# groupeLIAMG/ttcr

Hardware: AMD Instinct MI355X
Metric: Mnodes/s per sweep-iteration (512^3 fp32 grid, first-order FSM) (higher is better)
Workload: dtype f32

## Files before the change

include/ttcr_amd.h:

```cpp
#ifndef TTCR_AMD_H
#define TTCR_AMD_H

#include <stddef.h>
#include <stdint.h>

#ifdef __cplusplus
extern "C" {
#endif

typedef struct ttcr_fsm_grid ttcr_fsm_grid;

enum { TTCR_F32 = 0, TTCR_F64 = 1 };

enum {
    TTCR_OK = 0,
    TTCR_ERR_VALUE = 1,
    TTCR_ERR_RUNTIME = 2,
    TTCR_ERR_DEVICE = 3,
    TTCR_ERR_UNSUPPORTED = 4
};

int ttcr_fsm_device_count(void);

const char* ttcr_fsm_last_error(void);
// ... 97 lines not shown
int ttcr_fsm_adjoint_vjp_source(const ttcr_fsm_adjoint* t, const void* w, int w_on_device, const void* field_cot, int fc_on_device, void* grad,
                                int grad_on_device, void* gsrc, int gsrc_on_device, int schedule, int* passes);
int ttcr_fsm_adjoint_hold(ttcr_fsm_adjoint* t, const void* w, int w_on_device, const void* field_cot, int fc_on_device, void* grad,
                          int grad_on_device, int schedule, int* passes);
int ttcr_fsm_adjoint_release(ttcr_fsm_adjoint* t);
int ttcr_fsm_adjoint_hvp(ttcr_fsm_adjoint* t, const void* v, int v_on_device, void* out, int out_on_device, int schedule, int* passes_jvp,
                         int* passes_vjp);
int ttcr_fsm_adjoint_newton(ttcr_fsm_adjoint* t, const void* v, int v_on_device, const void* row_weight, int rw_on_device, void* out,
                            int out_on_device, int schedule, int* passes_jvp, int* passes_vjp);
int ttcr_fsm_adjoint_jvp_block(const ttcr_fsm_adjoint* t, int n_cols, const void* ds, int ds_on_device, void* dtt, int dtt_on_device,
                               void* dfields, int df_on_device, int schedule, int* passes);
int ttcr_fsm_adjoint_vjp_block(const ttcr_fsm_adjoint* t, int n_cols, const void* w, int w_on_device, void* grad, int grad_on_device,
                               int schedule, int* passes);
int ttcr_fsm_adjoint_gn_block(const ttcr_fsm_adjoint* t, int n_cols, const void* v, int v_on_device, const void* row_weight,
                              int rw_cols, int rw_on_device, void* out, int out_on_device, int schedule, int* passes_jvp, int* passes_vjp);
int ttcr_fsm_adjoint_block_release(ttcr_fsm_adjoint* t);
int ttcr_fsm_adjoint_free(ttcr_fsm_adjoint* t);

int ttcr_fsm_normal_tile_edge(int dtype);
int ttcr_fsm_normal_smooth(ttcr_fsm_adjoint* t, const void* v, int v_on_device, const double* weights, void* out, int out_on_device);
int ttcr_fsm_normal_dot(ttcr_fsm_adjoint* t, const void* a, int a_on_device, const void* b, int b_on_device, double* result);
int ttcr_fsm_normal_solve(ttcr_fsm_adjoint* t, const void* rhs, int rhs_on_device, const void* row_weight, int rw_on_device, double smooth,
                          const double* smooth_weights, double damp, const void* x0, int x0_on_device, int maxiter, double rtol,
                          int newton, int schedule, void* x, int x_on_device, int* status, int* iterations, double* rho, double* pq,
                          int* passes);
int ttcr_fsm_normal_release(ttcr_fsm_adjoint* t);

int ttcr_fsm_joint_jvp(const ttcr_fsm_adjoint* t, const void* ds, int ds_on_device, const void* dsrc, int dsrc_on_device, void* dtt,
                       int dtt_on_device, void* dfields, int df_on_device, int schedule, int* passes);
int ttcr_fsm_joint_gn(const ttcr_fsm_adjoint* t, const void* v, int v_on_device, const void* v_src, int vs_on_device, const void* row_weight,
                      int rw_on_device, const double* source_scale, void* out, int out_on_device, void* out_src, int os_on_device,
                      int schedule, int* passes_jvp, int* passes_vjp);
int ttcr_fsm_joint_solve(ttcr_fsm_adjoint* t, const void* rhs, int rhs_on_device, const void* rhs_src, int rs_on_device,
                         const void* row_weight, int rw_on_device, double smooth, const double* smooth_weights, double damp,
                         const double* source_damp, const double* source_scale, int maxiter, double rtol, int schedule, void* x,
                         int x_on_device, void* x_src, int xs_on_device, int* status, int* iterations, double* rho, double* pq, int* passes);
int ttcr_fsm_joint_release(ttcr_fsm_adjoint* t);

int ttcr_fsm_rcv_eval(const ttcr_fsm_adjoint* t, size_t n_pts, const void* pts, int pts_on_device, const int* event_of_pt, void* tt,
                              int tt_on_device, void* grad, int grad_on_device);
int ttcr_fsm_rcv_points(ttcr_fsm_adjoint* t, const int* set_point_of_row, size_t set_n_points, size_t* n_points, int* point_of_row,
                        int* differing_rows);
int ttcr_fsm_rcv_jvp(const ttcr_fsm_adjoint* t, const void* drcv, int drcv_on_device, void* dtt, int dtt_on_device);
int ttcr_fsm_rcv_vjp(const ttcr_fsm_adjoint* t, const void* w, int w_on_device, void* grcv, int grcv_on_device);
int ttcr_fsm_rjoint_jvp(const ttcr_fsm_adjoint* t, const void* ds, int ds_on_device, const void* drcv, int drcv_on_device, void* dtt,
                        int dtt_on_device, void* dfields, int df_on_device, int schedule, int* passes);
int ttcr_fsm_rjoint_gn(const ttcr_fsm_adjoint* t, const void* v, int v_on_device, const void* v_rcv, int vr_on_device, const void* row_weight,
                       int rw_on_device, const double* rcv_scale, void* out, int out_on_device, void* out_rcv, int or_on_device,
                       int schedule, int* passes_jvp, int* passes_vjp);
int ttcr_fsm_rjoint_solve(ttcr_fsm_adjoint* t, const void* rhs, int rhs_on_device, const void* rhs_rcv, int rr_on_device,
                          const void* row_weight, int rw_on_device, double smooth, const double* smooth_weights, double damp,
                          const double* rcv_damp, const double* rcv_scale, int maxiter, double rtol, int schedule, void* x,
                          int x_on_device, void* x_rcv, int xr_on_device, int* status, int* iterations, double* rho, double* pq, int* passes);
int ttcr_fsm_rcv_release(ttcr_fsm_adjoint* t);

int ttcr_fsm_loc_geometry(const ttcr_fsm_adjoint* t, int* nn, double* dx, double* origin);
int ttcr_fsm_loc_shape(const ttcr_fsm_adjoint* t, int* node_tile, int* hypo_chunk, int* staged);
int ttcr_fsm_loc_grid(const ttcr_fsm_adjoint* t, size_t n_hypo, const long long* hypo_off, const int* pick_field, const double* pick_time,
                      const double* pick_weight, const int* box, long long* node_out, double* t0_out, double* misfit_out,
                      void* volume_out, int volume_on_device);
int ttcr_fsm_loc_release(ttcr_fsm_adjoint* t);

int ttcr_fsm_raytrace_l(ttcr_fsm_grid* g, int slot, int n_tx, const void* tx, const void* t0, int n_rx,
                        const void* rx, void* tt_out, int with_rays);
int ttcr_fsm_slot_l_size(const ttcr_fsm_grid* g, int slot, size_t* n_rows, size_t* nnz);
int ttcr_fsm_get_slot_l(const ttcr_fsm_grid* g, int slot, long long* row_off, long long* cell, void* v);
int ttcr_fsm_raytrace_multi_l(ttcr_fsm_grid* g, int n_src, const int* tx_off, const void* tx, const void* t0, const int* rx_off,
                              const void* rx, void* tt_out, int with_rays);
int ttcr_fsm_multi_l_size(const ttcr_fsm_grid* g, size_t* n_rows, size_t* nnz);
int ttcr_fsm_get_multi_l(const ttcr_fsm_grid* g, long long* row_off, long long* cell, void* v);

typedef struct {
    double sweep_ms;
    double total_ms;
    long long kernel_launches;
    long long node_updates;
    long long evaluated_updates;
    int iterations;
    int n_sources;
} ttcr_fsm_timing;
int ttcr_fsm_last_timing(const ttcr_fsm_grid* g, ttcr_fsm_timing* out);
int ttcr_fsm_stopping_stats(const ttcr_fsm_grid* g, long long* reference_sums, long long* reference_sums_missed, long long* rounds);
int ttcr_fsm_prefill_swaps(const ttcr_fsm_grid* g, long long* swaps);
int ttcr_fsm_prefill_inline_fills(const ttcr_fsm_grid* g, long long* fills);
int ttcr_fsm_reference_change(ttcr_fsm_grid* g, const void* times, const void* field, int parallel, void* out);
int ttcr_fsm_last_kernel(const ttcr_fsm_grid* g, char* buf, size_t n);
int ttcr_fsm_unit_order(int dim, int dtype, int stage, int by_time, uint32_t nnx, uint32_t nny, uint32_t nnz, uint32_t* out,
                        size_t capacity, size_t* n_units);
int ttcr_fsm_prefill_slice(int dtype, uint64_t n_el, uint32_t n_tickets, uint32_t ticket, uint64_t* slice_len, uint64_t* begin, uint64_t* end);
const char* ttcr_fsm_build_id(void);

#ifdef __cplusplus
}
#endif
#endif
```

ttcr_amd/_lib.py:

```python
import ctypes as C
import os

HERE = os.path.dirname(os.path.abspath(__file__))
LIB_PATH = os.environ.get("TTCR_AMD_LIB") or os.path.join(HERE, "libttcr_amd.so")

TTCR_F32, TTCR_F64 = 0, 1
OK, ERR_VALUE, ERR_RUNTIME, ERR_DEVICE, ERR_UNSUPPORTED = 0, 1, 2, 3, 4

_P = C.c_void_p
_U32 = C.c_uint32
_D = C.c_double
_I = C.c_int


class Timing(C.Structure):
    _fields_ = [("sweep_ms", C.c_double), ("total_ms", C.c_double), ("kernel_launches", C.c_longlong),
                ("node_updates", C.c_longlong), ("evaluated_updates", C.c_longlong), ("iterations", C.c_int),
                ("n_sources", C.c_int)]


SYMBOLS = {
    "ttcr_fsm_device_count": (_I, []),
    "ttcr_fsm_last_error": (C.c_char_p, []),
    "ttcr_fsm3d_create": (_I, [C.POINTER(_P), _I, _I, _U32, _U32, _U32, _D, _D, _D, _D, _D, _I, _I, _I, _I, _I]),
    "ttcr_fsm2d_create": (_I, [C.POINTER(_P), _I, _I, _U32, _U32, _D, _D, _D, _D, _D, _I, _I, _I, _I, _I]),
    "ttcr_fsm3d_create_multi": (_I, [C.POINTER(_P), _I, _I, _U32, _U32, _U32, _D, _D, _D, _D, _D, _I, _I, _I, _I, C.POINTER(_I), _I]),
    "ttcr_fsm2d_create_multi": (_I, [C.POINTER(_P), _I, _I, _U32, _U32, _D, _D, _D, _D, _D, _I, _I, _I, _I, C.POINTER(_I), _I]),
    "ttcr_fsm_n_devices": (_I, [_P]),
    "ttcr_fsm_destroy": (None, [_P]),
    "ttcr_fsm_set_slowness": (_I, [_P, _P, C.c_size_t]),
    "ttcr_fsm_set_slowness_device": (_I, [_P, _P, C.c_size_t]),
    "ttcr_fsm_set_slowness_c_order": (_I, [_P, _P, C.c_size_t]),
    "ttcr_fsm_get_slowness": (_I, [_P, _P, C.c_size_t]),
    "ttcr_fsm_raytrace": (_I, [_P, _I, _I, _P, _P, _I, _P, _P]),
    "ttcr_fsm_raytrace_multi": (_I, [_P, _I, _P, _P, _P, _P, _P, _P]),
    "ttcr_fsm_get_tt": (_I, [_P, _I, _P, C.c_size_t]),
    "ttcr_fsm_get_tt_device": (_I, [_P, _I, C.POINTER(_P)]),
    "ttcr_fsm_get_tt_device_view": (_I, [_P, _I, C.POINTER(_P), C.POINTER(C.c_size_t)]),
    "ttcr_fsm_interp": (_I, [_P, _I, _I, _P, _P]),
    "ttcr_fsm_compute_slowness": (_I, [_P, _I, _P, _I, _P]),
    "ttcr_fsm_get_niter": (_I, [_P, _I, C.POINTER(_I), C.POINTER(_I)]),
    "ttcr_fsm_get_changes": (_I, [_P, _I, C.POINTER(_D), _I, C.POINTER(_D), _I]),
    "ttcr_fsm_get_reference_changes": (_I, [_P, _I, C.POINTER(_D), _I, C.POINTER(_D), _I]),
    "ttcr_fsm_n_slots": (_I, [_P]),
    "ttcr_fsm_n_nodes": (C.c_size_t, [_P]),
    "ttcr_fsm_n_cells": (C.c_size_t, [_P]),
    "ttcr_fsm_set_option": (_I, [_P, C.c_char_p, _D]),
    "ttcr_fsm_last_timing": (_I, [_P, C.POINTER(Timing)]),
    "ttcr_fsm_last_kernel": (_I, [_P, C.c_char_p, C.c_size_t]),
    "ttcr_fsm_build_id": (C.c_char_p, []),
    "ttcr_fsm_unit_order": (_I, [_I, _I, _I, _I, _U32, _U32, _U32, C.POINTER(_U32), C.c_size_t, C.POINTER(C.c_size_t)]),
    "ttcr_fsm_stopping_stats": (_I, [_P, C.POINTER(C.c_longlong), C.POINTER(C.c_longlong), C.POINTER(C.c_longlong)]),
    "ttcr_fsm_prefill_swaps": (_I, [_P, C.POINTER(C.c_longlong)]),
    "ttcr_fsm_prefill_inline_fills": (_I, [_P, C.POINTER(C.c_longlong)]),
    "ttcr_fsm_prefill_slice": (_I, [_I, C.c_uint64, _U32, _U32, C.POINTER(C.c_uint64), C.POINTER(C.c_uint64), C.POINTER(C.c_uint64)]),
    "ttcr_fsm_reference_change": (_I, [_P, C.c_void_p, C.c_void_p, C.c_int, C.c_void_p]),
    "ttcr_fsm_rays_size": (_I, [_P, C.POINTER(C.c_size_t), C.POINTER(C.c_size_t)]),
    "ttcr_fsm_get_rays": (_I, [_P, _P, _P]),
    "ttcr_fsm_raytrace_rays": (_I, [_P, _I, _I, _P, _P, _I, _P, _P]),
    "ttcr_fsm_slot_rays_size": (_I, [_P, _I, C.POINTER(C.c_size_t), C.POINTER(C.c_size_t)]),
    "ttcr_fsm_get_slot_rays": (_I, [_P, _I, _P, _P]),
    "ttcr_fsm_raytrace_m": (_I, [_P, _I, _I, _P, _P, _I, _P, _P]),
    "ttcr_fsm_raytrace_rm": (_I, [_P, _I, _I, _P, _P, _I, _P, _P]),
    "ttcr_fsm_raytrace_multi_m": (_I, [_P, _I, _P, _P, _P, _P, _P, _P, _I]),
    "ttcr_fsm_multi_m_size": (_I, [_P, C.POINTER(C.c_size_t), C.POINTER(C.c_size_t)]),
    "ttcr_fsm_get_multi_m": (_I, [_P, _P, _P, _P]),
    "ttcr_fsm_raytrace_multi_tape": (_I, [_P, _I, _P, _P, _P, _P, _P, _P, C.POINTER(_P)]),
    "ttcr_fsm_tape_size": (_I, [_P, C.POINTER(C.c_size_t), C.POINTER(C.c_size_t), C.POINTER(C.c_size_t)]),
    "ttcr_fsm_tape_bytes": (_I, [_P, C.POINTER(C.c_size_t)]),
    "ttcr_fsm_tape_device": (_I, [_P, C.POINTER(_I)]),
    "ttcr_fsm_tape_get_csr": (_I, [_P, _P, _P, _P]),
    "ttcr_fsm_tape_vjp": (_I, [_P, _P, _I, _P, _I]),
    "ttcr_fsm_tape_free": (_I, [_P]),
    "ttcr_fsm_raytrace_multi_adjoint": (_I, [_P, _I, _P, _P, _P, _P, _P, _P, C.POINTER(_P)]),
    "ttcr_fsm_raytrace_multi_adjoint_cells": (_I, [_P, _I, _P, _P, _P, _P, _P, _P, C.POINTER(_P)]),
    "ttcr_fsm_adjoint_model": (_I, [_P, C.POINTER(_I), C.POINTER(C.c_size_t), C.POINTER(C.c_size_t)]),
    "ttcr_fsm_adjoint_size": (_I, [_P, C.POINTER(C.c_size_t), C.POINTER(C.c_size_t), C.POINTER(C.c_size_t)]),
    "ttcr_fsm_adjoint_bytes": (_I, [_P, C.POINTER(C.c_size_t)]),
    "ttcr_fsm_adjoint_device": (_I, [_P, C.POINTER(_I)]),
    "ttcr_fsm_adjoint_get_field": (_I, [_P, C.c_size_t, _P]),
    "ttcr_fsm_adjoint_vjp": (_I, [_P, _P, _I, _P, _I, _P, _I, _I, C.POINTER(_I)]),
    "ttcr_fsm_adjoint_jvp": (_I, [_P, _P, _I, _P, _I, _P, _I, _I, C.POINTER(_I)]),
    "ttcr_fsm_adjoint_gn": (_I, [_P, _P, _I, _P, _I, _P, _I, _I, C.POINTER(_I), C.POINTER(_I)]),
    "ttcr_fsm_adjoint_points": (_I, [_P, C.POINTER(C.c_size_t), _P]),
    "ttcr_fsm_adjoint_jvp_source": (_I, [_P, _P, _I, _I, _P, _I, _P, _I, _I, C.POINTER(_I)]),
    "ttcr_fsm_adjoint_vjp_source": (_I, [_P, _P, _I, _P, _I, _P, _I, _P, _I, _I, C.POINTER(_I)]),
    "ttcr_fsm_adjoint_hold": (_I, [_P, _P, _I, _P, _I, _P, _I, _I, C.POINTER(_I)]),
    "ttcr_fsm_adjoint_release": (_I, [_P]),
    "ttcr_fsm_adjoint_hvp": (_I, [_P, _P, _I, _P, _I, _I, C.POINTER(_I), C.POINTER(_I)]),
    "ttcr_fsm_adjoint_newton": (_I, [_P, _P, _I, _P, _I, _P, _I, _I, C.POINTER(_I), C.POINTER(_I)]),
    "ttcr_fsm_adjoint_jvp_block": (_I, [_P, _I, _P, _I, _P, _I, _P, _I, _I, C.POINTER(_I)]),
    "ttcr_fsm_adjoint_vjp_block": (_I, [_P, _I, _P, _I, _P, _I, _I, C.POINTER(_I)]),
    "ttcr_fsm_adjoint_gn_block": (_I, [_P, _I, _P, _I, _P, _I, _I, _P, _I, _I, C.POINTER(_I), C.POINTER(_I)]),
    "ttcr_fsm_adjoint_block_release": (_I, [_P]),
    "ttcr_fsm_adjoint_free": (_I, [_P]),
    "ttcr_fsm_normal_tile_edge": (_I, [_I]),
    "ttcr_fsm_normal_smooth": (_I, [_P, _P, _I, C.POINTER(_D), _P, _I]),
    "ttcr_fsm_normal_dot": (_I, [_P, _P, _I, _P, _I, C.POINTER(_D)]),
    "ttcr_fsm_normal_solve": (_I, [_P, _P, _I, _P, _I, _D, C.POINTER(_D), _D, _P, _I, _I, _D, _I, _I, _P, _I, C.POINTER(_I),
                                   C.POINTER(_I), C.POINTER(_D), C.POINTER(_D), C.POINTER(_I)]),
    "ttcr_fsm_normal_release": (_I, [_P]),
    "ttcr_fsm_joint_jvp": (_I, [_P, _P, _I, _P, _I, _P, _I, _P, _I, _I, C.POINTER(_I)]),
    "ttcr_fsm_joint_gn": (_I, [_P, _P, _I, _P, _I, _P, _I, C.POINTER(_D), _P, _I, _P, _I, _I, C.POINTER(_I), C.POINTER(_I)]),
    "ttcr_fsm_joint_solve": (_I, [_P, _P, _I, _P, _I, _P, _I, _D, C.POINTER(_D), _D, C.POINTER(_D), C.POINTER(_D), _I, _D, _I, _P, _I, _P, _I,
                                  C.POINTER(_I), C.POINTER(_I), C.POINTER(_D), C.POINTER(_D), C.POINTER(_I)]),
    "ttcr_fsm_joint_release": (_I, [_P]),
    "ttcr_fsm_rcv_eval": (_I, [_P, C.c_size_t, _P, _I, C.POINTER(_I), _P, _I, _P, _I]),
    "ttcr_fsm_rcv_points": (_I, [_P, C.POINTER(_I), C.c_size_t, C.POINTER(C.c_size_t), C.POINTER(_I), C.POINTER(_I)]),
    "ttcr_fsm_rcv_jvp": (_I, [_P, _P, _I, _P, _I]),
    "ttcr_fsm_rcv_vjp": (_I, [_P, _P, _I, _P, _I]),
    "ttcr_fsm_rjoint_jvp": (_I, [_P, _P, _I, _P, _I, _P, _I, _P, _I, _I, C.POINTER(_I)]),
    "ttcr_fsm_rjoint_gn": (_I, [_P, _P, _I, _P, _I, _P, _I, C.POINTER(_D), _P, _I, _P, _I, _I, C.POINTER(_I), C.POINTER(_I)]),
    "ttcr_fsm_rjoint_solve": (_I, [_P, _P, _I, _P, _I, _P, _I, _D, C.POINTER(_D), _D, C.POINTER(_D), C.POINTER(_D), _I, _D, _I, _P, _I, _P, _I,
                                   C.POINTER(_I), C.POINTER(_I), C.POINTER(_D), C.POINTER(_D), C.POINTER(_I)]),
    "ttcr_fsm_rcv_release": (_I, [_P]),
    "ttcr_fsm_loc_geometry": (_I, [_P, C.POINTER(_I), C.POINTER(_D), C.POINTER(_D)]),
    "ttcr_fsm_loc_shape": (_I, [_P, C.POINTER(_I), C.POINTER(_I), C.POINTER(_I)]),
    "ttcr_fsm_loc_grid": (_I, [_P, C.c_size_t, C.POINTER(C.c_longlong), C.POINTER(_I), C.POINTER(_D), C.POINTER(_D), C.POINTER(_I),
                               C.POINTER(C.c_longlong), C.POINTER(_D), C.POINTER(_D), _P, _I]),
    "ttcr_fsm_loc_release": (_I, [_P]),
    "ttcr_fsm_raytrace_multi_l": (_I, [_P, _I, _P, _P, _P, _P, _P, _P, _I]),
    "ttcr_fsm_multi_l_size": (_I, [_P, C.POINTER(C.c_size_t), C.POINTER(C.c_size_t)]),
    "ttcr_fsm_get_multi_l": (_I, [_P, _P, _P, _P]),
    "ttcr_fsm_slot_m_size": (_I, [_P, _I, C.POINTER(C.c_size_t), C.POINTER(C.c_size_t)]),
    "ttcr_fsm_get_slot_m": (_I, [_P, _I, _P, _P, _P]),
    "ttcr_fsm_raytrace_l": (_I, [_P, _I, _I, _P, _P, _I, _P, _P, _I]),
    "ttcr_fsm_slot_l_size": (_I, [_P, _I, C.POINTER(C.c_size_t), C.POINTER(C.c_size_t)]),
    "ttcr_fsm_get_slot_l": (_I, [_P, _I, _P, _P, _P]),
}

_lib = None


def load():
# ... 50 lines not shown
```

ttcr_amd/build.py:

```python
import os
import shutil
import subprocess

HERE = os.path.dirname(os.path.abspath(__file__))
CSRC = os.path.join(HERE, "csrc")
OBJ = os.path.join(CSRC, "_obj")
LIB = os.path.join(HERE, "libttcr_amd.so")
INC = os.path.join("..", "..", "include", "ttcr_amd.h")
UNITS = {
    "fsm_capi.hip": ([], ["fsm_capi.hip", "fsm_kernels.h", "fsm_fast_api.h", "fsm_march_levels.inc", "fsm_fast.hip", "fsm_tape_api.h",
                          "fsm_tape.hip", "fsm_adjoint_api.h", "fsm_adjoint.hip", "fsm_normal.hip", "fsm_locate.hip", "fsm_unit_order.h", "fsm_prefill_slices.h", INC]),
    "fsm_fast.hip": ([], ["fsm_fast.hip", "fsm_fast_api.h", "fsm_kernels.h", "fsm_march_levels.inc", "fsm_prefill_slices.h"]),
    "fsm_tape.hip": ([], ["fsm_tape.hip", "fsm_tape_api.h"]),
    "fsm_adjoint.hip": ([], ["fsm_adjoint.hip", "fsm_adjoint_api.h", "fsm_kernels.h", "fsm_march_levels.inc", "fsm_prefill_slices.h"]),
    "fsm_normal.hip": ([], ["fsm_normal.hip", "fsm_adjoint_api.h"]),
    "fsm_locate.hip": ([], ["fsm_locate.hip", "fsm_adjoint_api.h"]),
}
SOURCES = list(UNITS)
DEPS = sorted({d for _, ds in UNITS.values() for d in ds})
FLAGS = ["--offload-arch=gfx950", "-O3", "-std=c++17", "-fPIC", "-ffp-contract=off",
         "-fno-fast-math", "-Wall", "-Wno-unused-result"]


def _hipcc():
    for c in (os.environ.get("HIPCC"), shutil.which("hipcc"), "/opt/rocm/bin/hipcc"):
        if c and os.path.exists(c):
            return c
    raise RuntimeError("hipcc not found")


def source_hash():
    import hashlib

    h = hashlib.sha256(" ".join(FLAGS).encode())
    for src in SOURCES:
        h.update(" ".join(UNITS[src][0]).encode())
    for d in DEPS:
        with open(os.path.join(CSRC, d), "rb") as f:
            h.update(f.read())
    return h.hexdigest()[:16]


def _obj(src):
    return os.path.join(OBJ, os.path.splitext(src)[0] + ".o")


def _stale(target, deps):
    if not os.path.exists(target):
        return True
    t = os.path.getmtime(target)
    return any(os.path.getmtime(os.path.join(CSRC, d)) > t for d in deps)


def needs_build():
    return _stale(LIB, DEPS)


def build(force=False, verbose=False):
    if not force and not needs_build():
        return LIB
    os.makedirs(OBJ, exist_ok=True)
    procs = []
    for src, (extra, deps) in UNITS.items():
        if force or _stale(_obj(src), deps):
            cmd = [_hipcc()] + FLAGS + extra + ['-DTTCR_BUILD_ID="%s"' % source_hash(), "-c", os.path.join(CSRC, src), "-o", _obj(src)]
            if verbose:
                print(" ".join(cmd), flush=True)
            procs.append((cmd, subprocess.Popen(cmd, cwd=CSRC)))
    for cmd, p in procs:
        if p.wait() != 0:
            raise subprocess.CalledProcessError(p.returncode, cmd)
    cmd = [_hipcc(), "--offload-arch=gfx950", "-shared", "-fPIC"] + [_obj(s) for s in SOURCES] + ["-o", LIB]
    if verbose:
        print(" ".join(cmd), flush=True)
    subprocess.check_call(cmd, cwd=CSRC)
    return LIB


if __name__ == "__main__":
    print(build(force=True, verbose=True))
```

ttcr_amd/csrc/fsm_capi.hip:

```cpp
#include <hip/hip_runtime.h>

#include <algorithm>
#include <atomic>
#include <chrono>
#include <condition_variable>
#include <cmath>
#include <cstdio>
#include <cstdlib>
#include <cstring>
#include <limits>
#include <map>
#include <memory>
#include <mutex>
#include <sstream>
#include <stdexcept>
#include <string>
#include <thread>
#include <vector>

#include "../../include/ttcr_amd.h"
#include "fsm_kernels.h"
#include "fsm_fast_api.h"
#include "fsm_tape_api.h"
#include "fsm_adjoint_api.h"
// ... 50 lines not shown
    ~DevBuf() { release(); }
};

struct Timing {
    double sweep_ms = 0, total_ms = 0;
    long long launches = 0, node_updates = 0, evaluated_updates = 0;
    int iterations = 0, n_sources = 0;
};

class GridBase {
   public:
    virtual ~GridBase() {}
    virtual void set_slowness(const void* s, size_t n, bool on_device, bool c_order = false) = 0;
    virtual void get_slowness(void* out, size_t n) = 0;
    virtual void raytrace_multi(int n_src, const int* tx_off, const void* tx, const void* t0, const int* rx_off,
                                const void* rx, void* tt_out, int forced_slot, const int* explicit_slots = nullptr,
                                bool force_rays = false) = 0;
    virtual void raytrace_rays(int slot, int n_tx, const void* tx, const void* t0, int n_rx, const void* rx, void* tt_out) = 0;
    virtual void slot_rays_size(int slot, size_t* n_rays, size_t* n_points) const = 0;
    virtual void get_slot_rays(int slot, long long* offsets, void* pts) const = 0;
    virtual void raytrace_m(int slot, int n_tx, const void* tx, const void* t0, int n_rx, const void* rx, void* tt_out, bool both) = 0;
    virtual void slot_m_size(int slot, size_t* n_rows, size_t* nnz) const = 0;
    virtual void get_slot_m(int slot, long long* row_off, long long* j, void* v) const = 0;
    virtual void raytrace_multi_m(int n_src, const int* tx_off, const void* tx, const void* t0, const int* rx_off, const void* rx,
                                  void* tt_out, bool both) = 0;
    virtual void multi_m_size(size_t* n_rows, size_t* nnz) const = 0;
    virtual void get_multi_m(long long* row_off, long long* j, void* v) const = 0;
    virtual void raytrace_multi_tape(int n_src, const int* tx_off, const void* tx, const void* t0, const int* rx_off, const void* rx,
                                     void* tt_out, TapeRows& out) = 0;
    virtual void raytrace_multi_adjoint(int n_src, const int* tx_off, const void* tx, const void* t0, const int* rx_off, const void* rx,
                                        void* tt_out, AdjSink& sink) = 0;
    virtual void adjoint_geometry(int* nn3, double* spacing, bool wrt_cells) const = 0;
    AdjSink* adj_sink = nullptr;
    std::vector<int> adj_src, adj_row;
    virtual void raytrace_l(int slot, int n_tx, const void* tx, const void* t0, int n_rx, const void* rx, void* tt_out, bool with_rays) = 0;
    virtual void slot_l_size(int slot, size_t* n_rows, size_t* nnz) const = 0;
    virtual void get_slot_l(int slot, long long* row_off, long long* cell, void* v) const = 0;
    virtual void raytrace_multi_l(int n_src, const int* tx_off, const void* tx, const void* t0, const int* rx_off, const void* rx,
                                  void* tt_out, bool with_rays) = 0;
    virtual void multi_l_size(size_t* n_rows, size_t* nnz) const = 0;
    virtual void get_multi_l(long long* row_off, long long* cell, void* v) const = 0;
    virtual void validate_points(int n_tx, const void* tx, int n_rx, const void* rx) = 0;
    struct Request {
        int slot, n_tx, n_rx;
        const void *tx, *t0, *rx;
        void* tt;
        int status = TTCR_OK;
        std::string err;
        bool done = false;
    };
    std::mutex q_mu;
    std::condition_variable q_cv;
    std::vector<Request*> queue;
    bool leader_active = false;
    bool had_company = false;
    std::atomic<int> combine_window_us{200};
    size_t elem_size = 4;
    virtual void get_tt(int slot, void* out, size_t n) = 0;
    virtual void* tt_device(int slot) = 0;
    virtual void* tt_device_view(int slot, size_t* stride) = 0;
    std::mutex mu;
    virtual void interp(int slot, int n, const void* pts, void* out) = 0;
    virtual void compute_slowness(int n, const void* pts, bool translated, void* out) = 0;
    virtual void rays_size(size_t* n_rays, size_t* n_points) const = 0;
    virtual void get_rays(long long* offsets, void* pts) const = 0;
    int dim = 3, dtype = 0, n_slots = 1, device = 0;
    size_t n_nodes = 0, n_cells = 0;
    std::vector<int> niter, niterw;
    std::vector<int> phys;
    int P(int slot) const { return phys.empty() ? slot : phys[slot]; }
    int stopping_shortcuts = 3;
    int stopping_rule = 1;
    long long reference_sums = 0, reference_sums_missed = 0;
    long long refsum_rounds = 0;
    virtual void stopping_stats(long long* sums, long long* missed, long long* rounds) const {
        if (sums) *sums = reference_sums;
        if (missed) *missed = reference_sums_missed;
        if (rounds) *rounds = refsum_rounds;
    }
    virtual void reference_change_host(const void* times, const void* field, bool parallel, void* out) = 0;
    int pair_by_distance = 1;
    virtual void set_pair_layout(int) {}
    virtual long long prefill_inline_count() const { return 0; }
    virtual long long prefill_swap_count() const { return 0; }
    int lone_chunk = 16;
    int arith = 0;
    int prefill = -1;
    int prefill_inline = -1;
    std::vector<std::vector<double>> change_hist, change_histw;
    std::vector<std::vector<double>> ref_hist, ref_histw;
    virtual void get_reference_changes(int slot, double* first, int n_first, double* wen, int n_weno) const {
        if (slot < 0 || slot >= n_slots) throw ValueError("Thread number is larger than number of threads");
        slot = P(slot);
        for (int q = 0; q < n_first; ++q) first[q] = (!ref_hist.empty() && q < (int)ref_hist[slot].size()) ? ref_hist[slot][q] : std::nan("");
        for (int q = 0; q < n_weno; ++q) wen[q] = (!ref_histw.empty() && q < (int)ref_histw[slot].size()) ? ref_histw[slot][q] : std::nan("");
    }
    virtual void get_changes(int slot, double* first, int n_first, double* wen, int n_weno) const {
        if (slot < 0 || slot >= n_slots) throw ValueError("Thread number is larger than number of threads");
        slot = P(slot);
        for (int q = 0; q < n_first; ++q) first[q] = (!change_hist.empty() && q < (int)change_hist[slot].size()) ? change_hist[slot][q] : 0.0;
        for (int q = 0; q < n_weno; ++q) wen[q] = (!change_histw.empty() && q < (int)change_histw[slot].size()) ? change_histw[slot][q] : 0.0;
    }
    bool weno = false;
    bool sweep45_strips = false;
    bool rotated = false;
    int ttrp = 0, interp_vel = 0;
    std::atomic<int> return_rays{0};
    int fixed_iters = 0, max_batch = 0, use_graph = 1;
    int skip = -1;
    int mode = 2;
    Timing timing;
    std::string last_kernel;
    virtual std::string kernel_name() const { return last_kernel; }
    long walk_step_limit = 1000000;
    long walk_records = 0;
    long walk_room(long extent) const { return std::min<long>(walk_step_limit, walk_records > 0 ? walk_records : extent); }
    virtual void apply_option(const std::string& k, double value) {
        if (k == "fixed_iters") fixed_iters = (int)value;
        else if (k == "max_batch") max_batch = (int)value;
        else if (k == "use_graph") use_graph = (int)value;
        else if (k == "combine_window_us") combine_window_us = (int)value;
        else if (k == "mode") mode = (int)value;
        else if (k == "skip") skip = (int)value;
        else if (k == "tt_from_rp") ttrp = value != 0;
        else if (k == "interp_vel") interp_vel = value != 0;
        else if (k == "return_rays") return_rays = value != 0;
        else if (k == "pair_sources") pair_by_distance = value != 0;
        else if (k == "pair_layout") {
            if (value != -1 && value != 0 && value != 1) throw ValueError("option 'pair_layout': -1 (default), 0 or 1");
            set_pair_layout((int)value);
        }
        else if (k == "stopping_rule") stopping_rule = (int)value;
        else if (k == "stopping_shortcuts") { if (value < 0 || value > 3 || value != (double)(int)value) throw ValueError("option stopping_shortcuts: 0 ... 3"); stopping_shortcuts = (int)value; }
        else if (k == "prefill") {
            if (value != -1 && value != 0 && value != 1) throw ValueError("option 'prefill': -1 (default), 0 or 1");
            prefill = (int)value;
        } else if (k == "prefill_inline") {
            if (value != -1 && value != 0 && value != 1) throw ValueError("option 'prefill_inline': -1 (default), 0 or 1");
            prefill_inline = (int)value;
        } else if (k == "lone_chunk") {
            if (value != 8 && value != 16) throw ValueError("option 'lone_chunk': 8 or 16");
            lone_chunk = (int)value;
        }
        else if (k == "arith") {
            if (value != 0 && value != 1 && value != 2)
                throw ValueError("option 'arith': 0 (the reference's arithmetic), 1 (tolerance-grade fp32 where it stays within 1e-5 s RMS) or 2 (the WENO stage as well)");
            arith = (int)value;
        }
        else if (k == "walk_records") {
            if (value != 0 && !(value >= 1 && value <= (double)walk_step_limit && value == (double)(long)value))
                throw ValueError("option 'walk_records': 0 (default) or a whole number from 1 to the step limit of a walk");
            walk_records = (long)value;
        }
        else throw ValueError("unknown option '" + k + "'");
    }
    virtual void get_niter(int slot, int* it, int* itw) const {
        if (slot < 0 || slot >= n_slots) throw ValueError("Thread number is larger than number of threads");
        if (it) *it = niter[P(slot)];
        if (itw) *itw = niterw[P(slot)];
    }
};

template <typename T, int DIM> struct TileCfg;
#ifndef FSM_PJ3
#define FSM_PJ3 16
#endif
#ifndef FSM_PK3
#define FSM_PK3 16
#endif
template <> struct TileCfg<float, 3> { static constexpr int PJ = FSM_PJ3, PK = FSM_PK3, BL = 16; };
template <> struct TileCfg<double, 3> { static constexpr int PJ = 16, PK = 8, BL = 16; };
#ifndef FSM_PJ2
#define FSM_PJ2 64
#endif
#ifndef FSM_CHUNK2
#define FSM_CHUNK2 16
#endif
template <> struct TileCfg<float, 2> { static constexpr int PJ = FSM_PJ2, PK = 1, BL = 32; };
template <> struct TileCfg<double, 2> { static constexpr int PJ = FSM_PJ2, PK = 1, BL = 32; };
template <typename T, int DIM> struct ChunkCfg { static constexpr int C = DIM == 3 ? FSM_CHUNK3 : FSM_CHUNK2; };

template <typename T>
class GridT : public GridBase {
   public:
    uint32_t ncx, ncy, ncz;
    T dx, dz, xmin, ymin, zmin, xmax, ymax, zmax, ox = 0, oy = 0, oz = 0;
    T epsilon;
    int nitermax;
    bool cell, translate;
    bool have_slowness = false;

    hipStream_t stream = nullptr;
    hipEvent_t ev0 = nullptr, ev1 = nullptr;
    DevBuf<T> d_s, d_cells, d_tt, d_rx, d_out;
    DevBuf<T> d_tt_alt;
    bool alt_filled = false;
    hipStream_t fill_stream = nullptr;
    hipEvent_t ev_fill = nullptr;
    long long prefill_swaps = 0;
    long long prefill_swap_count() const override { return prefill_swaps; }
    long long prefill_inline_fills = 0;
    long long prefill_inline_count() const override { return prefill_inline_fills; }
    void set_pair_layout(int v) override { pair_layout = v; }
    DevBuf<int> d_rslot;
    DevBuf<RaySrc> d_rdesc;
    int weno_ch4_min = 8;
    int weno_c16_below = 3;
    int f64_c16_below = 5;
    int pre_min = 2;
    size_t xs_lds_bytes = 40000;
    int xs_lds_below = 2;
    size_t xs_dyn_lds(int batch) const { return (dim == 3 && stage == 0 && batch < xs_lds_below) ? xs_lds_bytes : 0; }
    int time_order_below = 1 << 30;
    DevBuf<T> d_gather;
    DevBuf<T> d_rsrc, d_rt0;
    DevBuf<int> d_rstat;
    DevBuf<T> d_ssh;
    size_t ssh_stride = 0;
    DevBuf<uint32_t> d_mask;
    DevBuf<int> d_bbox, d_slots, d_lmask;
    int* h_lmask = nullptr;
    DevBuf<uint32_t> d_tiles;
    std::vector<int> tile_off, tile_cnt;
    DevBuf<double> d_change;
    DevBuf<unsigned long long> d_prof;
    size_t prof_words = 0;
    DevBuf<uint32_t> d_order;
    DevBuf<uint32_t> d_order_xs[2][2];
    DevBuf<int> d_sync;
    int n_patches = 0;
    int* h_abort = nullptr;
    DevBuf<int> d_stamp;
    DevBuf<unsigned long long> d_cmap;
    int cmap_words = 1;
    DevBuf<unsigned long long> d_sw;
    int sw_sweeps = 0;
    DevBuf<int> d_iter;
    DevBuf<unsigned long long> d_evals;
    int* h_iter = nullptr;
    unsigned launch_epoch = 1;
    bool sync_clean = true;
    size_t sync_words = 0;
    unsigned long long* h_evals = nullptr;
    int nbf = 0, nbj = 0, nbk = 0;
    size_t n_bricks = 0;
    DevBuf<InitPoint<T>> d_pts;
    double* h_change = nullptr;
    int* h_slots = nullptr;
    size_t mask_words = 0;
    SweepGeom geom;
    int n_launch = 0;
    hipGraph_t graphs[2] = {nullptr, nullptr};
    hipGraphExec_t graph_execs[2] = {nullptr, nullptr};
    int graph_batches[2] = {0, 0}, graph_modes[2] = {-1, -1};

    GridT(int dim_, bool cell_, uint32_t nx, uint32_t ny, uint32_t nz, double ddx, double ddz, double minx,
          double miny, double minz, double eps, int maxit, int nslots, bool translate_, int dev, bool weno_) {
        dim = dim_;
        weno = weno_;
        dtype = sizeof(T) == 4 ? TTCR_F32 : TTCR_F64;
        elem_size = sizeof(T);
        cell = cell_;
        translate = translate_;
        ncx = nx; ncy = ny; ncz = nz;
        dx = (T)ddx;
        dz = (T)ddz;
        xmin = (T)minx; ymin = (T)miny; zmin = (T)minz;
        xmax = xmin + (T)nx * dx;
        if (dim == 3) {
            ymax = ymin + (T)ny * dx;
            zmax = zmin + (T)nz * dx;
        } else {
            ymax = ymin;
            zmax = zmin + (T)nz * dz;
        }
        if (translate) {
            ox = xmin; oy = ymin; oz = zmin;
            xmax -= xmin; ymax -= ymin; zmax -= zmin;
            xmin = 0; ymin = 0; zmin = 0;
        }
        n_nodes = dim == 3 ? (size_t)(nx + 1) * (ny + 1) * (nz + 1) : (size_t)(nx + 1) * (nz + 1);
        n_cells = dim == 3 ? (size_t)nx * ny * nz : (size_t)nx * nz;
        if (n_nodes >= (1ull << 32)) throw ValueError("grid too large: node index must fit uint32 (reference T2)");
        epsilon = (T)eps;
        epsilon *= (T)n_nodes;
        nitermax = maxit;
        n_slots = nslots;
        niter.assign(n_slots, 0);
        niterw.assign(n_slots, 0);
        phys.resize(n_slots);
        for (int q = 0; q < n_slots; ++q) phys[q] = q;
        max_batch = n_slots;
        device = dev;
        HIP_CHECK(hipSetDevice(device));
        {
            int cus = 0;
            HIP_CHECK(hipDeviceGetAttribute(&cus, hipDeviceAttributeMultiprocessorCount, device));
            persist_wgs = 8 * std::max(cus, 1);
        }
        HIP_CHECK(hipStreamCreateWithFlags(&stream, hipStreamNonBlocking));
        HIP_CHECK(hipEventCreate(&ev0));
        HIP_CHECK(hipEventCreate(&ev1));
        d_s.reserve(n_nodes, 64);
        {
            long long pair_units_min = 6144;
            if (const char* e = std::getenv("TTCR_FSM_PAIR_UNITS")) pair_units_min = std::atoll(e);
            const long long patches = dim == 3 ? (long long)((ny + 1 + TileCfg<T, 3>::PJ - 1) / TileCfg<T, 3>::PJ) * ((nz + 1 + TileCfg<T, 3>::PK - 1) / TileCfg<T, 3>::PK) : 0;
            NS = (n_slots >= 2 && dim == 3 && !weno && (long long)n_slots * patches > pair_units_min) ? 2 : 1;
            ns_window = NS == 2 && (long long)n_slots * patches <= (5 * pair_units_min) / 2;
        }
        if (const char* e = std::getenv("TTCR_FSM_PAIR")) { NS = (std::atoi(e) != 0 && n_slots >= 2) ? 2 : 1; ns_window = false; }
        if (const char* e = std::getenv("TTCR_FSM_LAYOUT_LO")) layout_lo = std::atof(e);
        if (const char* e = std::getenv("TTCR_FSM_LAYOUT_HI")) layout_hi = std::atof(e);
        d_tt.reserve(n_nodes * tt_fields(), 64);
        mask_words = (n_nodes + 31) / 32;
        d_mask.reserve(mask_words * (size_t)n_slots);
        d_bbox.reserve(6 * (size_t)n_slots);
        d_slots.reserve(n_slots);
        d_lmask.reserve(n_slots);
        HIP_CHECK(hipHostMalloc((void**)&h_lmask, sizeof(int) * n_slots));
        d_change.reserve(n_slots);
        if (std::getenv("TTCR_FSM_PROF")) {
            prof_words = 8 + 4 * (size_t)(1 << 20);
            d_prof.reserve(prof_words);
            HIP_CHECK(hipMemset(d_prof.p, 0, prof_words * sizeof(unsigned long long)));
        }
        HIP_CHECK(hipHostMalloc((void**)&h_change, sizeof(double) * n_slots));
        HIP_CHECK(hipHostMalloc((void**)&h_slots, sizeof(int) * n_slots));
        HIP_CHECK(hipHostMalloc((void**)&h_abort, sizeof(int)));
        *h_abort = 0;
        HIP_CHECK(hipHostMalloc((void**)&h_iter, 2 * sizeof(int)));
        HIP_CHECK(hipHostMalloc((void**)&h_evals, sizeof(unsigned long long) * n_slots));
        HIP_CHECK(hipMemsetAsync(d_tt.p, 0, n_nodes * tt_fields() * sizeof(T), stream));

        if (dim == 3) {
            using C = TileCfg<T, 3>;
            geom.NF = nx + 1; geom.NJ = ny + 1; geom.NK = nz + 1;
            geom.npj = (geom.NJ + C::PJ - 1) / C::PJ;
            geom.npk = (geom.NK + C::PK - 1) / C::PK;
            n_launch = count_launches(C::BL);
        } else {
            using C = TileCfg<T, 2>;
            geom.NF = nz + 1; geom.NJ = nx + 1; geom.NK = 1;
            geom.npj = (geom.NJ + C::PJ - 1) / C::PJ;
            geom.npk = 1;
            n_launch = count_launches(C::BL);
        }
        geom.n_nodes = (uint32_t)n_nodes;
        geom.M = (std::max(geom.NF, geom.NJ) + 1) & ~1;
        geom.MP = geom.M + FSM_XPAD;
        geom.SR = dim == 3 ? ((geom.NJ + 15) / 16) * 32 : 0;
        ssh_stride = (size_t)geom.NK * shear_plane(geom);
        if ((double)(dim == 3 ? 16 : 1) * (double)shear_plane(geom) * sizeof(T) >= 4294967296.0)
            throw ValueError("grid too large for the slowness offsets of the sweep kernel (16 planes of max(nx, ny) x ny nodes must stay below 4 GiB)");
        d_ssh.reserve(ssh_stride * (dim == 3 ? 4 : 2));
        HIP_CHECK(hipMemsetAsync(d_ssh.p, 0, ssh_stride * (dim == 3 ? 4 : 2) * sizeof(T), stream));
        if (dim == 3) build_tile_lists(TileCfg<T, 3>::PJ, TileCfg<T, 3>::PK, TileCfg<T, 3>::BL);
        else build_tile_lists(TileCfg<T, 2>::PJ, TileCfg<T, 2>::PK, TileCfg<T, 2>::BL);
        build_persistent_lists();
        nbf = (geom.NF + FSM_BRICK - 1) / FSM_BRICK;
        nbj = (geom.NJ + FSM_BRICK - 1) / FSM_BRICK;
        nbk = (geom.NK + FSM_BRICK - 1) / FSM_BRICK;
        n_bricks = (size_t)nbf * nbj * nbk;
        d_stamp.reserve(n_bricks * n_slots);
        {
            const int PJ = dim == 3 ? TileCfg<T, 3>::PJ : TileCfg<T, 2>::PJ, PK = dim == 3 ? TileCfg<T, 3>::PK : 1;
            const int max_chunks = (geom.NF + 2 * (PJ + PK)) / 4 + 4;
            cmap_words = max_chunks / 32 + 1;
            d_cmap.reserve((size_t)n_patches * n_slots * (dim == 3 ? 8 : 4) * 2 * cmap_words);
            HIP_CHECK(hipMemset(d_cmap.p, 0, (size_t)n_patches * n_slots * (dim == 3 ? 8 : 4) * 2 * cmap_words * sizeof(unsigned long long)));
            sw_sweeps = (dim == 3 ? 8 : 4) * (2 * std::min(nitermax, 256) + 2);
            d_sw.reserve((size_t)sw_sweeps * n_slots);
        }
        d_iter.reserve(2);
        d_evals.reserve(n_slots);
        if (dim == 2)
            HIP_CHECK(hipFuncSetAttribute(reinterpret_cast<const void*>(&fsm_sweep45_rows<T>),
                                          hipFuncAttributeMaxDynamicSharedMemorySize, 156 * 1024));
        if (const char* e = std::getenv("TTCR_FSM_SWEEP45")) sweep45_strips = std::string(e) == "strips";
        if (const char* e = std::getenv("TTCR_FSM_WENO_CH4_MIN")) weno_ch4_min = std::atoi(e);
        if (const char* e = std::getenv("TTCR_FSM_WENO_C16_BELOW")) weno_c16_below = std::atoi(e);
        if (const char* e = std::getenv("TTCR_FSM_F64_C16_BELOW")) f64_c16_below = std::atoi(e);
        if (const char* e = std::getenv("TTCR_FSM_TIME_ORDER_BELOW")) time_order_below = std::atoi(e);
        if (const char* e = std::getenv("TTCR_FSM_PRE_MIN")) pre_min = std::atoi(e);
        if (const char* e = std::getenv("TTCR_FSM_SKIP")) skip = std::atoi(e);
        if (const char* e = std::getenv("TTCR_FSM_SKIP_UNITS")) skip_units_min = std::atoi(e);
        if (const char* e = std::getenv("TTCR_FSM_SKIP_PROBE_UNITS")) skip_probe_min = std::atoi(e);
        if (const char* e = std::getenv("TTCR_FSM_RS_FIELDS")) rs_fields_max = (size_t)std::max(0, std::atoi(e));
        if (const char* e = std::getenv("TTCR_FSM_WGS")) persist_wgs = std::atoi(e);
        if (const char* e = std::getenv("TTCR_FSM_XS_LDS")) xs_lds_bytes = (size_t)std::atol(e);
        if (const char* e = std::getenv("TTCR_FSM_XS_LDS_BELOW")) xs_lds_below = std::atoi(e);
        if (const char* e = std::getenv("TTCR_FSM_MODE")) mode = std::atoi(e);
        if (const char* e = std::getenv("TTCR_FSM_PREFILL")) prefill = std::atoi(e);
        if (const char* e = std::getenv("TTCR_FSM_LONE_CHUNK")) lone_chunk = std::atoi(e) == 8 ? 8 : 16;
        if (const char* e = std::getenv("TTCR_FSM_ARITH")) arith = std::max(0, std::min(2, std::atoi(e)));
    }

    void build_persistent_lists() {
        const std::vector<uint32_t> order = fsm_diag_order(geom.npj, geom.npk);
        n_patches = (int)order.size();
        d_order.reserve(order.size());
        HIP_CHECK(hipMemcpy(d_order.p, order.data(), order.size() * sizeof(uint32_t), hipMemcpyHostToDevice));
        sync_words = 8 + (size_t)n_patches * n_slots * (dim == 3 ? 8 : 4);
        d_sync.reserve(sync_words);
        HIP_CHECK(hipMemset(d_sync.p, 0, sync_words * sizeof(int)));
        if (geom.npj >= (1 << 14) || geom.npk >= (1 << 14)) throw ValueError("grid too large for the patch index of the sweep kernel");
        for (int st = 0; st < 2; ++st)
            for (int tm = 0; tm < 2; ++tm) {
                const std::vector<uint32_t> xs = xs_order(order, tm != 0, st == 0 ? 1 : 2);
                d_order_xs[st][tm].reserve(xs.size());
                HIP_CHECK(hipMemcpy(d_order_xs[st][tm].p, xs.data(), xs.size() * sizeof(uint32_t), hipMemcpyHostToDevice));
            }
    }

    std::vector<uint32_t> xs_order(const std::vector<uint32_t>& diag_order, bool by_time, int H) const {
        const int PJ = dim == 3 ? TileCfg<T, 3>::PJ : TileCfg<T, 2>::PJ, PK = dim == 3 ? TileCfg<T, 3>::PK : 1;
        const int C = dim == 3 ? ChunkCfg<T, 3>::C : ChunkCfg<T, 2>::C;
        return fsm_xs_order(dim, geom.NF, geom.NJ, geom.NK, PJ, PK, C, H, by_time, diag_order);
    }

    template <int DIM, int H>
    void launch_sweeps_persistent(int batch) {
        constexpr int C0 = ChunkCfg<T, DIM>::C;
        if constexpr (DIM == 3 && C0 == 8) {
            const int below = H == 2 ? weno_c16_below : sizeof(T) == 4 ? std::numeric_limits<int>::max() : f64_c16_below;
            if (NS == 1 && mode == 2 && (lone_chunk == 16 || fast_now<H>()) && batch < below) {
                launch_sweeps_persistent_ns<DIM, H, 1, 16, true>(batch);
                return;
            }
        }
        if (H == 2 && DIM == 3 && NS == 2 && batch >= weno_ch4_min && C0 == 8) {
            if (NS == 2) launch_sweeps_persistent_ns<DIM, H, 2, (H == 2 && DIM == 3) ? 4 : C0>(batch);
            else launch_sweeps_persistent_ns<DIM, H, 1, (H == 2 && DIM == 3) ? 4 : C0>(batch);
        } else {
            if (NS == 2) launch_sweeps_persistent_ns<DIM, H, 2, C0>(batch); else launch_sweeps_persistent_ns<DIM, H, 1, C0>(batch);
        }
    }

    template <int DIM, int H, int NSV, int CH, bool XS_ONLY = false>
    void launch_sweeps_persistent_ns(int batch) {
        using C = TileCfg<T, DIM>;
        PersistArgs<T> pa;
        SweepArgs<T>& a = pa.s;
        constexpr bool NO_PRE = CH == 16 && H == 1 && DIM == 3;
        const size_t dyn_lds = NO_PRE ? 0 : xs_dyn_lds(batch);
        a.tt = d_tt.p;
        a.ts = NS;
        a.lmask = d_lmask.p;
        a.frozen = d_mask.p;
        a.bbox = d_bbox.p;
        a.change = d_change.p;
        a.slots = d_slots.p;
        a.tiles = nullptr;
        a.g = geom;
        a.prof = d_prof.p;
        a.mask_words = (uint32_t)mask_words;
        a.dx = dx;
        a.dz = dz;
        a.w = 0;
        a.variant = DIM == 3 ? 0 : (dx == dz ? 1 : 2);
        pa.order = d_order.p;
        pa.sync = d_sync.p;
        pa.n_patches = n_patches;
        pa.batch = batch;
        pa.timeout_ticks = 300000000ull;
        pa.stamp = d_stamp.p;
        pa.iter_ptr = d_iter.p;
        pa.evals = d_evals.p;
        pa.nbf = nbf; pa.nbj = nbj; pa.nbk = nbk;
        pa.ndir = DIM == 3 ? 8 : 4;
        pa.skip = skip_now(batch) ? (std::getenv("TTCR_FSM_SKIP_ALL_DIRTY") ? 2 : 1) : 0;
        pa.cmap = d_cmap.p;
        pa.cw = cmap_words;
        pa.sw = std::getenv("TTCR_FSM_NO_SW") ? nullptr : d_sw.p;
        pa.n_sw_groups = n_groups();
        pa.n_sw_sweeps = sw_sweeps;
        pa.fill_dst = nullptr;
        pa.fill_slice = 0;
        pa.fill_n = 0;

        const size_t wg_cap = (fsm_looped(DIM == 3, H) && persist_wgs > 0) ? (size_t)persist_wgs : ~(size_t)0;
        const dim3 block(C::PJ * C::PK), grid((unsigned)std::min<size_t>((size_t)n_patches * batch, wg_cap));
        const int ndir = DIM == 3 ? 8 : 4;
        {
            const bool pre_ = mode == 2 && !NO_PRE && (DIM == 2 || batch >= pre_min || dyn_lds > 0);
            char nm[160];
            std::snprintf(nm, sizeof nm, "fsm_sweep_persistent<%s,%d,%d,%d,%s,%s,%d,%d,%s,%s>", sizeof(T) == 4 ? "float" : "double", C::PJ, C::PK, CH,
                          DIM == 3 ? "true" : "false", skip_now(batch) ? "true" : "false", H, NSV, mode == 2 ? "true" : "false", pre_ ? "true" : "false");
            last_kernel = nm;
        }
        if (mode == 2) {
            pa.ssh = d_ssh.p;
            pa.ssh_stride = ssh_stride;
            pa.dir = 0;
            a.rf = a.rj = a.rk = a.rev = 0;
            a.s_sheared = nullptr;
            pa.timeout_ticks = 1000000000ull;
            const dim3 gridx((unsigned)std::min<size_t>((size_t)n_patches * batch * ndir, wg_cap));
            pa.order = d_order_xs[H == 2 ? 1 : 0][batch < time_order_below ? 1 : 0].p;
            const bool pre = DIM == 2 || batch >= pre_min || dyn_lds > 0;
            if (fill_arm) {
                pa.fill_dst = d_tt_alt.p;
                pa.fill_n = n_nodes * tt_fields();
                pa.fill_slice = fsm_fill_slice_len(pa.fill_n, (size_t)n_patches * batch * ndir, 16 / sizeof(T));
                fill_arm = false;
                fill_in_flight = true;
            }
            if constexpr (std::is_same<T, float>::value) {
                if (fast_now<H>() && (H == 1 || NSV == 1)) {
                    const FastCfg fc{H, DIM, NSV, CH, skip_now(batch), NO_PRE ? false : pre};
                    last_kernel.insert(last_kernel.size() - 1, ",1");
                    const hipError_t e = fsm_fast_launch(pa, fc, gridx.x, dyn_lds, stream);
                    if (e == hipErrorInvalidValue) throw std::logic_error("arith = 1: no such kernel (" + last_kernel + ")");
                    HIP_CHECK(e);
                    return;
                }
            }
            if constexpr (NO_PRE) {
                (void)pre;
                if (skip_now(batch))
                    fsm_sweep_persistent<T, C::PJ, C::PK, CH, DIM == 3, true, H, NSV, true><<<gridx, block, dyn_lds, stream>>>(pa);
                else
                    fsm_sweep_persistent<T, C::PJ, C::PK, CH, DIM == 3, false, H, NSV, true><<<gridx, block, dyn_lds, stream>>>(pa);
            } else {
                if (skip_now(batch) && pre)
                    fsm_sweep_persistent<T, C::PJ, C::PK, CH, DIM == 3, true, H, NSV, true, true><<<gridx, block, dyn_lds, stream>>>(pa);
                else if (skip_now(batch))
                    fsm_sweep_persistent<T, C::PJ, C::PK, CH, DIM == 3, true, H, NSV, true><<<gridx, block, dyn_lds, stream>>>(pa);
                else if (pre)
                    fsm_sweep_persistent<T, C::PJ, C::PK, CH, DIM == 3, false, H, NSV, true, true><<<gridx, block, dyn_lds, stream>>>(pa);
                else
                    fsm_sweep_persistent<T, C::PJ, C::PK, CH, DIM == 3, false, H, NSV, true><<<gridx, block, dyn_lds, stream>>>(pa);
            }
            HIP_CHECK(hipGetLastError());
            return;
        }
        if (fast_now<H>() && H == 1) throw ValueError("option 'arith' = 1 needs whole-iteration launches (option 'mode' = 2)");
        if constexpr (XS_ONLY) throw std::logic_error("launch_sweeps_persistent_ns: whole-iteration launches only");
        else {
        pa.ssh = nullptr;
        pa.ssh_stride = 0;
        static const int RX2[4] = {0, 1, 1, 0}, RZ2[4] = {0, 0, 1, 1};
        for (int d = 0; d < ndir; ++d) {
            int fam;
            if (DIM == 3) {
                a.rf = d & 1; a.rj = (d >> 1) & 1; a.rk = (d >> 2) & 1;
                a.rev = a.rk;
                fam = (a.rf ^ a.rk) | ((a.rj ^ a.rk) << 1);
            } else {
                a.rj = RX2[d]; a.rf = RZ2[d]; a.rk = 0;
                a.rev = a.rj;
                fam = a.rf ^ a.rj;
            }
            a.s_sheared = d_ssh.p + (size_t)fam * ssh_stride;
            pa.dir = d;
            if (skip_now(batch))
                fsm_sweep_persistent<T, C::PJ, C::PK, CH, DIM == 3, true, H, NSV, false><<<grid, block, 0, stream>>>(pa);
            else
                fsm_sweep_persistent<T, C::PJ, C::PK, CH, DIM == 3, false, H, NSV, false><<<grid, block, 0, stream>>>(pa);
        }
        HIP_CHECK(hipGetLastError());
        }
    }

    void build_tile_lists(int PJ, int PK, int BL) {
        std::vector<uint32_t> all;
        tile_off.assign(n_launch, 0);
        tile_cnt.assign(n_launch, 0);
        for (int w = 0; w < n_launch; ++w) {
            tile_off[w] = (int)all.size();
            for (int m = 0; m <= geom.npj + geom.npk - 2; ++m) {
                const int L0 = BL * w - m * (BL - 1);
                for (int TK = std::max(0, m - geom.npj + 1); TK <= std::min(m, geom.npk - 1); ++TK) {
                    const int TJ = m - TK;
                    const int j0 = TJ * PJ, k0 = TK * PK;
                    const int jmaxp = std::min(j0 + PJ, geom.NJ) - 1, kmaxp = std::min(k0 + PK, geom.NK) - 1;
                    if (L0 + BL - 1 < j0 + k0 || L0 > jmaxp + kmaxp + geom.NF - 1) continue;
                    all.push_back((uint32_t)TJ | ((uint32_t)TK << 16));
                }
            }
            tile_cnt[w] = (int)all.size() - tile_off[w];
        }
        d_tiles.reserve(std::max<size_t>(all.size(), 1));
        HIP_CHECK(hipMemcpy(d_tiles.p, all.data(), all.size() * sizeof(uint32_t), hipMemcpyHostToDevice));
    }

    ~GridT() override {
        (void)hipSetDevice(device);
        for (int i = 0; i < 2; ++i) {
            if (graph_execs[i]) (void)hipGraphExecDestroy(graph_execs[i]);
            if (graphs[i]) (void)hipGraphDestroy(graphs[i]);
        }
        if (h_change) (void)hipHostFree(h_change);
        if (h_slots) (void)hipHostFree(h_slots);
        if (h_lmask) (void)hipHostFree(h_lmask);
        if (h_abort) (void)hipHostFree(h_abort);
        if (h_iter) (void)hipHostFree(h_iter);
// ... 200 lines not shown
        a.dz = dz;
        a.variant = DIM == 3 ? 0 : (dx == dz ? 1 : 2);
        const dim3 block(C::PJ * C::PK);
        const int ndir = DIM == 3 ? 8 : 4;
        static const int RX2[4] = {0, 1, 1, 0}, RZ2[4] = {0, 0, 1, 1};
        for (int d = 0; d < ndir; ++d) {
            int fam;
            if (DIM == 3) {
                a.rf = d & 1; a.rj = (d >> 1) & 1; a.rk = (d >> 2) & 1;
                a.rev = a.rk;
                fam = (a.rf ^ a.rk) | ((a.rj ^ a.rk) << 1);
            } else {
                a.rj = RX2[d]; a.rf = RZ2[d]; a.rk = 0;
                a.rev = a.rj;
                fam = a.rf ^ a.rj;
            }
            a.s_sheared = d_ssh.p + (size_t)fam * ssh_stride;
            for (int w = 0; w < n_launch; ++w) {
                if (tile_cnt[w] == 0) continue;
                a.w = w;
                a.tiles = d_tiles.p + tile_off[w];
                const dim3 grid(tile_cnt[w], 1, batch);
                fsm_sweep_tile<T, C::PJ, C::PK, C::BL, DIM == 3><<<grid, block, 0, stream>>>(a);
            }
        }
        last_kernel = std::string("fsm_sweep_tile<") + (sizeof(T) == 4 ? "float" : "double") + "," + std::to_string(C::PJ) + "," + std::to_string(C::PK) + "," + std::to_string(C::BL) + "," + (DIM == 3 ? "true" : "false") + ">";
        HIP_CHECK(hipGetLastError());
    }

    int NS = 1;
    bool ns_window = false;
    int pair_layout = -1;
    double last_eval_frac = -1;
    double layout_lo = 0.55, layout_hi = 0.70;
    void choose_layout() {
        if (!ns_window) return;
        int want = NS;
        if (pair_layout >= 0) want = pair_layout ? 2 : 1;
        else if (last_eval_frac >= 0) want = NS == 2 ? (last_eval_frac < layout_lo ? 1 : 2) : (last_eval_frac > layout_hi ? 2 : 1);
        if (want == NS) return;
        NS = want;
        graph_batches[0] = graph_batches[1] = -1;
        for (int q = 0; q < n_slots; ++q) phys[q] = q;
    }
    int n_groups() const { return (n_slots + NS - 1) / NS; }
    size_t tt_fields() const { return (size_t)n_slots + ((ns_window || NS == 2) ? (size_t)(n_slots & 1) : 0); }
    T* tt_ptr(int slot) const { return d_tt.p + (size_t)(slot / NS) * n_nodes * NS + slot % NS; }
    template <int H>
    bool fast_now() const { return sizeof(T) == 4 && (arith == 2 || (arith == 1 && !weno)); }
    bool prefill_on() const {
        if (prefill >= 0) return prefill != 0;
        const size_t bytes = n_nodes * tt_fields() * sizeof(T);
        if (bytes < ((size_t)64 << 20)) return false;
        size_t free_b = 0, total_b = 0;
        if (hipMemGetInfo(&free_b, &total_b) != hipSuccess) return false;
        return d_tt_alt.p || (2 * bytes <= total_b / 2 && bytes + ((size_t)1 << 30) <= free_b);
    }
    bool fill_arm = false;
    bool fill_in_flight = false;
    bool inline_fill_now(int entries) const {
        if (prefill_inline == 0 || !d_tt_alt.p || d_tt_alt.n < n_nodes * tt_fields()) return false;
        if (mode != 2 || stage != 0 || use_graph >= 2) return false;
        if (prefill_inline == 1) return true;
        return dim == 3 && !fast_now<1>() && (long long)n_patches * entries >= skip_units_min;
    }

    int stage = 0;
    int skip_units_min = 2048;
    int skip_probe_min = 1024;
    bool probe_skip = true;
    int probe_off_calls = 0;
    int persist_wgs = 2048;
    bool in_probe_window(int entries) const {
        const long long u = (long long)n_patches * entries;
        return dim == 3 && sizeof(T) == 4 && u >= skip_probe_min && u < skip_units_min;
    }
    int skip_default(int entries) const {
        if (dim != 3) return 1;
        if (stage == 1) return 1;
        if (in_probe_window(entries)) return probe_skip ? 1 : 0;
        return (long long)n_patches * entries >= skip_units_min ? 1 : 0;
    }
    bool persistent_now() const { return mode >= 1 || stage == 1; }
    bool skip_now(int entries) const {
        const int on = skip < 0 ? skip_default(entries) : skip;
        const bool fits = (long long)geom.NF + geom.NJ + geom.NK < (1ll << 22) && nbf <= 32 * FSM_SLAB_WORDS;
        return on != 0 && fits && !(dim == 2 && rotated && !weno && dx == dz);
    }

    void launch_sweep45(int batch) {
        Sweep45Args<T> a;
        a.tt = d_tt.p;
        a.s = d_s.p;
        a.frozen = d_mask.p;
        a.change = d_change.p;
        a.slots = d_slots.p;
        a.lmask = d_lmask.p;
        a.ts = NS;
        a.by_group = persistent_now() ? 1 : 0;
        a.nnx = (int)ncx + 1;
        a.nnz = (int)ncz + 1;
        a.n_nodes = n_nodes;
        a.mask_words = (uint32_t)mask_words;
        a.dx = dx;
        const int blocks = a.by_group ? batch * NS : batch;
        const size_t smem = 4 * ((size_t)a.nnz + 2) * sizeof(T);
        if (smem <= 156 * 1024 && !sweep45_strips) {
            const int threads = (int)std::min<size_t>(1024, (((size_t)a.nnz + 63) / 64) * 64);
            fsm_sweep45_rows<T><<<blocks, threads, smem, stream>>>(a);
        } else {
            constexpr int NTMAX = sizeof(T) == 4 ? 1024 : 512;
            if (a.nnx + 2 <= 256) fsm_sweep45<T, 256><<<blocks, 256, 0, stream>>>(a);
            else fsm_sweep45<T, NTMAX><<<blocks, NTMAX, 0, stream>>>(a);
        }
        HIP_CHECK(hipGetLastError());
    }

    void issue_sweeps(int batch) {
        issue_sweeps_axis(batch);
        if (dim == 2 && rotated && !weno && dx == dz) launch_sweep45(batch);
    }

    void issue_sweeps_axis(int batch) {
        if (stage == 1) {
            if (dim == 3) launch_sweeps_persistent<3, 2>(batch); else launch_sweeps_persistent<2, 2>(batch);
        } else if (mode >= 1) {
            if (dim == 3) launch_sweeps_persistent<3, 1>(batch); else launch_sweeps_persistent<2, 1>(batch);
        } else {
            if (dim == 3) launch_sweeps<3>(batch); else launch_sweeps<2>(batch);
        }
    }

    void run_iteration(int batch) {
        const int ndir = dim == 3 ? 8 : 4;
        if (use_graph >= 2 || (use_graph == 1 && !persistent_now())) {
            hipGraph_t& graph = graphs[stage];
            hipGraphExec_t& graph_exec = graph_execs[stage];
            const int key = mode * 2 + (skip_now(batch) ? 1 : 0);
            if (!graph_exec || graph_batches[stage] != batch || graph_modes[stage] != key) {
                if (graph_exec) { (void)hipGraphExecDestroy(graph_exec); graph_exec = nullptr; }
                if (graph) { (void)hipGraphDestroy(graph); graph = nullptr; }
                HIP_CHECK(hipStreamBeginCapture(stream, hipStreamCaptureModeThreadLocal));
                try {
                    issue_sweeps(batch);
                } catch (...) {
                    hipGraph_t junk = nullptr;
                    (void)hipStreamEndCapture(stream, &junk);
                    if (junk) (void)hipGraphDestroy(junk);
                    throw;
                }
                HIP_CHECK(hipStreamEndCapture(stream, &graph));
                HIP_CHECK(hipGraphInstantiate(&graph_exec, graph, nullptr, nullptr, 0));
                graph_batches[stage] = batch;
                graph_modes[stage] = key;
            }
            HIP_CHECK(hipGraphLaunch(graph_exec, stream));
        } else {
            issue_sweeps(batch);
        }
        timing.launches += mode == 2 ? 1 : persistent_now() ? (long long)ndir : (long long)ndir * n_launch;
    }

    std::map<int, DevBuf<T>> snap;
    std::vector<int> snap_iter;
    std::vector<double> prev_change;
    std::vector<double> prev2_change;
    bool snap_always = false;
    std::vector<int> snap_T;
    bool stamps_ok = false;
    int iter_T = 0;
    bool stamps_live_for(int entries) const { return (stopping_shortcuts & 1) && dim == 3 && !weno && persistent_now() && skip_now(entries) && n_nodes * (size_t)NS < ((size_t)1 << 31); }
    void terms_pass(int gi, T* x0, T* x1, unsigned* c0, unsigned* c1, int since_T) {
        RefTermsArgs<T> ta;
        ta.cur = d_tt.p + (size_t)gi * n_nodes * NS;
        ta.old = snap[gi].p;
        ta.x[0] = x0; ta.x[1] = x1;
        ta.cnt[0] = c0; ta.cnt[1] = c1;
        ta.n_nodes = (uint32_t)n_nodes;
        ta.ns = NS;
        constexpr int V = 16 / (int)sizeof(T);
        const size_t n_el = n_nodes * (size_t)NS;
        const bool vec = n_el % V == 0 && ((uintptr_t)ta.cur | (uintptr_t)ta.old) % 16 == 0;
        const int nodes_per_vec = vec ? std::max(1, V / NS) : 1;
        const bool bricks = since_T >= 0 && geom.NF % nodes_per_vec == 0;
        ta.stamp = bricks ? d_stamp.p + (size_t)gi * n_bricks : nullptr;
        ta.thr = (dim == 3 ? 8 : 4) * since_T + 1;
        ta.NF = geom.NF; ta.NJ = geom.NJ; ta.nbf = nbf; ta.nbj = nbj;
        const unsigned nblk = (unsigned)((n_nodes + FSM_REFSUM_CB - 1) / FSM_REFSUM_CB);
        const unsigned blocks = std::min(nblk, 8192u);
        if (vec) fsm_refsum_terms<T, V><<<blocks, 256, 0, stream>>>(ta);
        else fsm_refsum_terms<T, 1><<<blocks, 256, 0, stream>>>(ta);
        HIP_CHECK(hipGetLastError());
    }
    DevBuf<size_t> d_ref_off;
    DevBuf<T> d_ref_out;
    double window_lo() const { return sizeof(T) == 4 ? 0.5 : 1.0 - 1e-6; }
    double window_hi() const { return sizeof(T) == 4 ? 16.0 : 1.0 + 1e-6; }
    void snapshots_before_iteration(const std::vector<int>& active, int it_next) {
        if (!stopping_rule || fixed_iters > 0) return;
        if ((int)snap_iter.size() != n_groups()) snap_iter.assign(n_groups(), 0);
        const bool cheap = n_nodes * (size_t)NS <= ((size_t)1 << 24);
        std::vector<char> done(n_groups(), 0);
        for (int s2 : active) {
            const int gi = s2 / NS;
            if (done[gi]) continue;
            bool may = prev_change[s2] < 1e3 * window_hi() * (double)epsilon;
            if (may && (int)prev2_change.size() == n_slots && std::isfinite(prev2_change[s2]) && prev2_change[s2] > 0) {
                const double r = std::min(1.0, prev_change[s2] / prev2_change[s2]);
                may = prev_change[s2] * r / 8.0 <= window_hi() * (double)epsilon;
            }
            if (!(cheap || (stage == 1 && it_next == 1) || may || snap_always)) continue;
            if (it_next == 1 && stage == 0) continue;
            done[gi] = 1;
            if (snap_iter[gi] == it_next) continue;
            DevBuf<T>& b = snap[gi];
            b.reserve(n_nodes * (size_t)NS);
            if ((int)snap_T.size() != n_groups()) snap_T.assign(n_groups(), -1);
            if (stamps_ok && snap_T[gi] >= 0 && n_nodes * (size_t)NS < ((size_t)1 << 32)) terms_pass(gi, nullptr, nullptr, nullptr, nullptr, snap_T[gi]);
            else HIP_CHECK(hipMemcpyAsync(b.p, d_tt.p + (size_t)gi * n_nodes * NS, n_nodes * (size_t)NS * sizeof(T), hipMemcpyDeviceToDevice, stream));
            snap_iter[gi] = it_next;
            snap_T[gi] = iter_T;
// ... 172 lines not shown
                    const int gi = active[ask[a]] / NS;
                    if (a > a0 && active[ask[a - 1]] / NS == gi) continue;
                    T* xp[2] = {nullptr, nullptr};
                    unsigned* cp[2] = {nullptr, nullptr};
                    for (size_t b = a; b < a1 && active[ask[b]] / NS == gi; ++b) {
                        xp[active[ask[b]] % NS] = d_rs_x.p + (b - a0) * pitch;
                        cp[active[ask[b]] % NS] = d_rs_cnt.p + (b - a0) * (size_t)nblk;
                    }
                    const bool bricks = stamps_ok && (int)snap_T.size() == n_groups() && snap_T[gi] == iter_T;
                    terms_pass(gi, xp[0], xp[1], cp[0], cp[1], bricks ? iter_T : -1);
                    snap_iter[gi] = it + 1;
                    if ((int)snap_T.size() != n_groups()) snap_T.assign(n_groups(), -1);
                    snap_T[gi] = iter_T + 1;
                }
                const dim3 cgrid(std::min(nblk, 4096u), (unsigned)nf);
                fsm_refsum_scan<0><<<(unsigned)nf, 1024, 0, stream>>>(d_rs_cnt.p, d_rs_off.p, nblk, d_rs_n.p);
                HIP_CHECK(hipGetLastError());
                std::vector<unsigned long long> h_m(nf);
                HIP_CHECK(hipMemcpyAsync(h_m.data(), d_rs_n.p, nf * sizeof(unsigned long long), hipMemcpyDeviceToHost, stream));
                HIP_CHECK(hipStreamSynchronize(stream));
                std::vector<size_t> need;
                for (size_t f = 0; f < nf; ++f) {
                    const double u = 0.5 * (double)std::numeric_limits<T>::epsilon(), mu = (double)h_m[f] * u;
                    const double c = h_change[active[ask[a0 + f]]], e = (double)epsilon;
                    if (host_prof) std::fprintf(stderr, "[host]   ask: slot %d iteration %d  fp64 change / (eps N) %.4f  non-zero terms %llu (M u = %.4f)\n", active[ask[a0 + f]], it, c / e, h_m[f], mu);
                    if (h_m[f] == 0ull) { res[a0 + f] = (T)0; res_known[a0 + f] = 1; continue; }
                    if ((stopping_shortcuts & 2) && stage == 0 && mu < 0.25) {
                        const double g = mu / (1.0 - mu), m = 2.0 * (double)(geom.NF + geom.NJ + geom.NK + 64) * u + 1e-6;
                        if (c * (1.0 - m) * (1.0 - g) >= e) { res_go[a0 + f] = 1; continue; }
                        if (c * (1.0 + m) * (1.0 + g) < e) { res_go[a0 + f] = 0; continue; }
                    }
                    need.push_back(f);
                }
                if (!need.empty()) {
                    fsm_refsum_compact<T><<<cgrid, 256, 0, stream>>>(d_rs_x.p, d_rs_xc.p, pitch, n_nodes, d_rs_cnt.p, d_rs_off.p, nblk);
                    HIP_CHECK(hipGetLastError());
                    std::vector<const T*> c2(need.size()), o2(need.size(), nullptr);
                    std::vector<unsigned long long> m2(need.size());
                    for (size_t q = 0; q < need.size(); ++q) { c2[q] = curs[need[q]]; m2[q] = h_m[need[q]]; }
                    d_rs_n2.reserve(std::max<size_t>(need.size(), 64));
                    HIP_CHECK(hipMemcpyAsync(d_rs_n2.p, m2.data(), need.size() * sizeof(unsigned long long), hipMemcpyHostToDevice, stream));
                    const std::vector<T> r = reference_changes(c2, o2, 1, false, epsilon, d_rs_n2.p, &m2);
                    for (size_t q = 0; q < need.size(); ++q) { res[a0 + need[q]] = r[q]; res_known[a0 + need[q]] = 1; }
                }
                a0 = a1;
            }
        }
        for (size_t a = 0; a < ask.size(); ++a) {
            go[ask[a]] = res_known[a] ? res[a] >= epsilon : res_go[a] != 0;
            if (res_known[a]) ref_change_last[active[ask[a]]] = (double)res[a];
            ++reference_sums;
        }
        return go;
    }
    std::vector<double> ref_change_last;

    bool host_prof = std::getenv("TTCR_FSM_HOST_PROF") != nullptr;
    std::chrono::steady_clock::time_point hp_t = std::chrono::steady_clock::now();
    void hp_mark(const char* what) {
        if (!host_prof) return;
        const auto now = std::chrono::steady_clock::now();
        std::fprintf(stderr, "[host] %-28s %8.3f ms\n", what, std::chrono::duration<double, std::milli>(now - hp_t).count());
        hp_t = now;
    }
    void solve_batch(const std::vector<int>& slot_ids, const std::vector<int>& src_ids, const int* tx_off,
                     const T* tx, const T* t0) {
        const int nb = (int)slot_ids.size();
        hp_mark("(before solve_batch)");
        const int nc = ncoord();
        const long long node_updates_before = timing.node_updates;
        size_t tot_pts = 0;
        for (int b = 0; b < nb; ++b) tot_pts += tx_off[src_ids[b] + 1] - tx_off[src_ids[b]];
        std::vector<InitPoint<T>> pts;
        pts.reserve(tot_pts);
        std::vector<size_t> first(nb);
        for (int b = 0; b < nb; ++b) {
            first[b] = pts.size();
            for (int n = tx_off[src_ids[b]]; n < tx_off[src_ids[b] + 1]; ++n) pts.push_back(locate(tx + (size_t)nc * n, t0[n]));
        }
        d_pts.reserve(std::max<size_t>(tot_pts, 1));
        HIP_CHECK(hipMemcpyAsync(d_pts.p, pts.data(), pts.size() * sizeof(InitPoint<T>), hipMemcpyHostToDevice, stream));
        for (int b = 0; b < nb; ++b)
            HIP_CHECK(hipMemsetAsync(d_stamp.p + (size_t)(slot_ids[b] / NS) * n_bricks, 0xFF, n_bricks * sizeof(int), stream));
        std::vector<char> group_filled(n_groups(), 0);
        const bool all_slots = nb == n_slots && prefill_on();
        fill_arm = fill_in_flight = false;
        bool inline_filled = false;
        if (all_slots && alt_filled) {
            HIP_CHECK(hipStreamWaitEvent(stream, ev_fill, 0));
            std::swap(d_tt.p, d_tt_alt.p);
            std::swap(d_tt.n, d_tt_alt.n);
            std::swap(d_tt.guard, d_tt_alt.guard);
            alt_filled = false;
            ++prefill_swaps;
            graph_batches[0] = graph_batches[1] = -1;
            std::fill(group_filled.begin(), group_filled.end(), 1);
        }
        if (NS > 1) {
            std::vector<int> cnt(n_groups(), 0);
            for (int b = 0; b < nb; ++b) cnt[slot_ids[b] / NS] += 1;
            for (int gi = 0; gi < n_groups(); ++gi) {
                if (cnt[gi] != NS || group_filled[gi]) continue;
                const size_t n_el = n_nodes * (size_t)NS;
                const int blocks = (int)std::min<size_t>((n_el + 255) / 256, 16384);
                fsm_fill<T><<<blocks, 256, 0, stream>>>(d_tt.p + (size_t)gi * n_el, n_el, real_traits<T>::max(), 1);
                group_filled[gi] = 1;
            }
        }
        for (int b = 0; b < nb; ++b) {
            const int slot = slot_ids[b];
            T* tt = tt_ptr(slot);
            const int blocks = (int)std::min<size_t>((n_nodes + 255) / 256, 8192);
            if (!group_filled[slot / NS]) fsm_fill<T><<<blocks, 256, 0, stream>>>(tt, n_nodes, real_traits<T>::max(), NS);
            HIP_CHECK(hipMemsetAsync(d_mask.p + (size_t)slot * mask_words, 0, mask_words * sizeof(uint32_t), stream));
            InitArgs<T> ia;
            ia.tt = tt;
            ia.ts = NS;
            ia.slowness = d_s.p;
            ia.frozen = d_mask.p + (size_t)slot * mask_words;
            ia.bbox = d_bbox.p + 6 * (size_t)slot;
            ia.pts = d_pts.p + first[b];
            ia.n_pts = tx_off[src_ids[b] + 1] - tx_off[src_ids[b]];
            ia.npts = weno ? 2 : 1;
            ia.nnx = ncx + 1;
            ia.nny = dim == 3 ? ncy + 1 : 1;
            ia.nnz = ncz + 1;
            ia.dx = dx; ia.dz = dz; ia.xmin = xmin; ia.ymin = ymin; ia.zmin = zmin;
            ia.dim = dim;
            ia.stamp = d_stamp.p + (size_t)(slot / NS) * n_bricks;
            ia.nbf = nbf; ia.nbj = nbj; ia.nbk = nbk;
            fsm_init_source<T><<<1, 128, 0, stream>>>(ia);
            niter[slot] = 0;
            niterw[slot] = 0;
            if (change_hist.empty()) { change_hist.resize(n_slots); change_histw.resize(n_slots); }
            if (ref_hist.empty()) { ref_hist.resize(n_slots); ref_histw.resize(n_slots); }
            change_hist[slot].clear();
            change_histw[slot].clear();
            ref_hist[slot].clear();
            ref_histw[slot].clear();
        }
        HIP_CHECK(hipGetLastError());
        hp_mark("reinit + initFSM issued");
        HIP_CHECK(hipStreamSynchronize(stream));
        hp_mark("reinit + initFSM done");

        const int maxit = fixed_iters > 0 ? fixed_iters : nitermax;
        const int ndir = dim == 3 ? 8 : 4;
        if (!sync_clean || launch_epoch > 0xfffff000u) {
            HIP_CHECK(hipMemsetAsync(d_sync.p, 0, sync_words * sizeof(int), stream));
            HIP_CHECK(hipMemsetAsync(d_cmap.p, 0, (size_t)n_patches * n_slots * ndir * 2 * cmap_words * sizeof(unsigned long long), stream));
            HIP_CHECK(hipStreamSynchronize(stream));
            launch_epoch = 1;
        }
        sync_clean = false;
        snap_always = false;
        if (persistent_now() || weno) HIP_CHECK(hipMemsetAsync(d_sync.p + 8, 0, (sync_words - 8) * sizeof(int), stream));
        if (persistent_now() || weno) HIP_CHECK(hipMemsetAsync(d_sync.p + 4, 0, sizeof(int), stream));
        HIP_CHECK(hipMemsetAsync(d_evals.p, 0, sizeof(unsigned long long) * n_slots, stream));
        HIP_CHECK(hipMemsetAsync(d_sw.p, 0, sizeof(unsigned long long) * (size_t)sw_sweeps * n_groups(), stream));
        HIP_CHECK(hipEventRecord(ev0, stream));
        int it_total = 0;
        for (stage = 0; stage < (weno ? 2 : 1); ++stage) {
            std::vector<int> active(slot_ids);
            int it = 0;
            prev_change.assign(n_slots, std::numeric_limits<double>::infinity());
            prev2_change.assign(n_slots, std::numeric_limits<double>::infinity());
            snap_iter.assign(n_groups(), 0);
            snap_T.assign(n_groups(), -1);
            stamps_ok = false;
            if ((int)ref_change_last.size() != n_slots) ref_change_last.assign(n_slots, std::nan(""));
            std::vector<int> groups;
            for (int s2 : slot_ids)
                if (groups.empty() || groups.back() != s2 / NS) groups.push_back(s2 / NS);
            while (!active.empty() && it < maxit) {
                int n_entries;
                if (persistent_now()) {
                    n_entries = (int)groups.size();
                    for (int b = 0; b < n_entries; ++b) {
                        int m2 = 0;
                        for (int s2 : active)
                            if (s2 / NS == groups[b]) m2 |= 1 << (s2 % NS);
                        h_slots[b] = m2 ? groups[b] : -1;
                        h_lmask[b] = m2;
                    }
                } else {
                    n_entries = nb;
                    for (int b = 0; b < nb; ++b) { h_slots[b] = b < (int)active.size() ? active[b] : -1; h_lmask[b] = 1; }
                }
                HIP_CHECK(hipMemcpyAsync(d_slots.p, h_slots, sizeof(int) * n_entries, hipMemcpyHostToDevice, stream));
                HIP_CHECK(hipMemcpyAsync(d_lmask.p, h_lmask, sizeof(int) * n_entries, hipMemcpyHostToDevice, stream));
                HIP_CHECK(hipMemsetAsync(d_change.p, 0, sizeof(double) * n_slots, stream));
                iter_T = it_total;
                snapshots_before_iteration(active, it + 1);
                if (host_prof) { HIP_CHECK(hipStreamSynchronize(stream)); hp_mark("snapshots"); }
                stamps_ok = (it == 0 ? true : stamps_ok) && stamps_live_for(n_entries);
                h_iter[0] = it_total;
                h_iter[1] = (int)launch_epoch;
                launch_epoch += (persistent_now() && mode == 2) ? 1u : (unsigned)ndir;
                HIP_CHECK(hipMemcpyAsync(d_iter.p, h_iter, 2 * sizeof(int), hipMemcpyHostToDevice, stream));
                fill_arm = it_total == 0 && all_slots && !alt_filled && inline_fill_now(n_entries);
                run_iteration(n_entries);
                fill_arm = false;
                HIP_CHECK(hipMemcpyAsync(h_change, d_change.p, sizeof(double) * n_slots, hipMemcpyDeviceToHost, stream));
                if (persistent_now()) HIP_CHECK(hipMemcpyAsync(h_abort, d_sync.p + 4, sizeof(int), hipMemcpyDeviceToHost, stream));
                HIP_CHECK(hipStreamSynchronize(stream));
                hp_mark("sweep-iteration");
                if (persistent_now() && *h_abort) {
                    HIP_CHECK(hipMemsetAsync(d_sync.p + 4, 0, sizeof(int), stream));
                    stage = 0;
                    throw DeviceError("persistent sweep kernel: a patch timed out waiting for its upwind neighbour");
                }
                if (fill_in_flight) { inline_filled = true; fill_in_flight = false; }
                ++it;
                ++it_total;
                std::vector<int> next;
                if (fixed_iters > 0) ref_change_last.assign(n_slots, std::nan(""));
                const std::vector<char> go = fixed_iters > 0 ? std::vector<char>(active.size(), 1) : decide_go_on(active, it);
                hp_mark("stopping rule");
                for (size_t q = 0; q < active.size(); ++q) {
                    const int s2 = active[q];
                    (stage == 0 ? niter : niterw)[s2] = it;
                    (stage == 0 ? change_hist : change_histw)[s2].push_back(h_change[s2]);
                    (stage == 0 ? ref_hist : ref_histw)[s2].push_back((int)ref_change_last.size() == n_slots ? ref_change_last[s2] : std::nan(""));
                    timing.node_updates += (long long)n_nodes * ndir;
                    prev2_change[s2] = prev_change[s2];
                    prev_change[s2] = h_change[s2];
                    if (go[q]) next.push_back(s2);
                }
                active.swap(next);
            }
            timing.iterations = std::max(timing.iterations, it_total);
            if (stage == 0 && weno) {
                HIP_CHECK(hipMemsetAsync(d_sw.p, 0, sizeof(unsigned long long) * (size_t)sw_sweeps * n_groups(), stream));
                for (int s2 : slot_ids)
                    HIP_CHECK(hipMemsetD32Async((hipDeviceptr_t)(d_stamp.p + (size_t)(s2 / NS) * n_bricks), it_total * (dim == 3 ? 8 : 4),
                                                n_bricks, stream));
            }
        }
        if (std::getenv("TTCR_FSM_DEBUG_SW")) {
            std::vector<unsigned long long> h((size_t)std::min(sw_sweeps, 40) * n_groups());
            HIP_CHECK(hipMemcpy(h.data(), d_sw.p, h.size() * sizeof(unsigned long long), hipMemcpyDeviceToHost));
            for (size_t q = 0; q < h.size(); ++q) std::fprintf(stderr, "%s%u/%u", q % n_groups() == 0 ? "\n[sw] " : " ", (unsigned)h[q], (unsigned)(h[q] >> 32));
            std::fprintf(stderr, "\n");
        }
        const bool was_persistent = mode >= 1 || weno;
        stage = 0;
        sync_clean = true;
        HIP_CHECK(hipEventRecord(ev1, stream));
        if (all_slots && inline_filled) {
            alt_filled = true;
            ++prefill_inline_fills;
        } else if (all_slots) {
            const size_t n_el = n_nodes * tt_fields();
            if (!fill_stream) {
                int lo = 0, hi = 0;
                HIP_CHECK(hipDeviceGetStreamPriorityRange(&lo, &hi));
                HIP_CHECK(hipStreamCreateWithPriority(&fill_stream, hipStreamNonBlocking, lo));
                HIP_CHECK(hipEventCreateWithFlags(&ev_fill, hipEventDisableTiming));
            }
            bool have_alt = true;
            try {
                d_tt_alt.reserve(n_el, 64);
            } catch (const DeviceError&) {
                (void)hipGetLastError();
                have_alt = false;
                prefill = 0;
            }
            if (have_alt) {
            HIP_CHECK(hipStreamWaitEvent(fill_stream, ev1, 0));
            const int blocks = (int)std::min<size_t>((n_el + 255) / 256, 16384);
            fsm_fill<T><<<blocks, 256, 0, fill_stream>>>(d_tt_alt.p, n_el, real_traits<T>::max(), 1);
            HIP_CHECK(hipEventRecord(ev_fill, fill_stream));
            alt_filled = true;
            }
        }
        HIP_CHECK(hipEventSynchronize(ev1));
        if (d_prof.p) {
            unsigned long long h[8];
            HIP_CHECK(hipMemcpy(h, d_prof.p, sizeof(h), hipMemcpyDeviceToHost));
            if (const char* tp = std::getenv("TTCR_FSM_PROF_TRACE")) {
                std::vector<unsigned long long> tr(prof_words);
                HIP_CHECK(hipMemcpy(tr.data(), d_prof.p, prof_words * sizeof(unsigned long long), hipMemcpyDeviceToHost));
                if (FILE* f = std::fopen(tp, "wb")) { std::fwrite(tr.data() + 8, sizeof(unsigned long long), prof_words - 8, f); std::fclose(f); }
            }
            HIP_CHECK(hipMemset(d_prof.p, 0, sizeof(h)));
            if (mode >= 1) {
                const double nb_ = (double)std::max<unsigned long long>(h[7], 1), nu_ = (double)std::max<unsigned long long>(h[6], 1);
                std::fprintf(stderr, "[ttcr_amd prof] units %llu chunks %llu  per unit (us): start %.2f total %.2f | per chunk (us): top %.3f  wait %.3f  stage %.3f  march %.3f  writeback %.3f\n",
                             h[6], h[7], h[5] * 0.01 / nu_, (h[0] + h[1] + h[2] + h[3] + h[4] + h[5]) * 0.01 / nu_, h[0] * 0.01 / nb_,
                             h[1] * 0.01 / nb_, h[2] * 0.01 / nb_, h[3] * 0.01 / nb_, h[4] * 0.01 / nb_);
            } else {
                const double nb_ = (double)std::max<unsigned long long>(h[4], 1);
                std::fprintf(stderr, "[ttcr_amd prof] tiles %llu  per tile (us): setup %.2f  stage %.2f  march %.2f  writeback %.2f\n",
                             h[4], h[0] * 0.01 / nb_, h[1] * 0.01 / nb_, h[2] * 0.01 / nb_, h[3] * 0.01 / nb_);
            }
        }
        hp_mark("after the iterations");
        float ms = 0;
        HIP_CHECK(hipEventElapsedTime(&ms, ev0, ev1));
        timing.sweep_ms += ms;
        const long long evaluated_before = timing.evaluated_updates;
        if (was_persistent) {
            HIP_CHECK(hipMemcpy(h_evals, d_evals.p, sizeof(unsigned long long) * n_slots, hipMemcpyDeviceToHost));
            for (int s2 : slot_ids) timing.evaluated_updates += (long long)h_evals[s2];
        } else {
            timing.evaluated_updates += timing.node_updates - node_updates_before;
        }
        const bool skipped_now = skip_now(n_groups());
        if (nb == n_slots && timing.node_updates > node_updates_before && skipped_now)
            last_eval_frac = (double)(timing.evaluated_updates - evaluated_before) / (double)(timing.node_updates - node_updates_before);
        if (skip < 0 && !weno && in_probe_window((nb + NS - 1) / NS) && timing.node_updates > node_updates_before) {
            if (skipped_now) {
                probe_skip = (double)(timing.evaluated_updates - evaluated_before) / (double)(timing.node_updates - node_updates_before) < 0.6;
                probe_off_calls = 0;
            } else if (++probe_off_calls >= 8) {
                probe_skip = true;
                probe_off_calls = 0;
            }
        }
    }

    void interp(int slot, int n, const void* pts, void* out) override {
        HIP_CHECK(hipSetDevice(device));
        check_slot(slot);
        if (n <= 0) return;
        const int nc = ncoord();
        std::vector<T> p((const T*)pts, (const T*)pts + (size_t)nc * n);
        if (translate)
            for (int m = 0; m < n; ++m) { p[3 * m] -= ox; p[3 * m + 1] -= oy; p[3 * m + 2] -= oz; }
        check_pts(p.data(), n);
        interp_grid_coords(P(slot), n, p.data(), (T*)out);
    }

    void compute_slowness(int n, const void* pts, bool translated, void* out) override {
        HIP_CHECK(hipSetDevice(device));
        if (!have_slowness) throw std::runtime_error("Error: slowness has not been assigned.");
        if (n <= 0) return;
        const int nc = ncoord();
        std::vector<T> p((const T*)pts, (const T*)pts + (size_t)nc * n);
        if (translate && !translated)
            for (int m = 0; m < n; ++m) { p[3 * m] -= ox; p[3 * m + 1] -= oy; p[3 * m + 2] -= oz; }
        check_pts(p.data(), n);
        d_rx.reserve((size_t)nc * n);
        d_out.reserve(n);
        HIP_CHECK(hipMemcpyAsync(d_rx.p, p.data(), sizeof(T) * nc * n, hipMemcpyHostToDevice, stream));
        const int blocks = (n + 63) / 64;
        if (dim == 3) {
            RayGeom<T> rg;
            rg.nnx = ncx + 1; rg.nny = ncy + 1; rg.nnz = ncz + 1;
            rg.dx = dx; rg.xmin = xmin; rg.ymin = ymin; rg.zmin = zmin; rg.xmax = xmax; rg.ymax = ymax; rg.zmax = zmax;
            rg.interp_vel = interp_vel;
            fsm_compute_slowness3d<T><<<blocks, 64, 0, stream>>>(rg, d_s.p, d_rx.p, n, d_out.p);
        } else {
            RayGeom2<T> rg2;
            rg2.nnx = ncx + 1; rg2.nnz = ncz + 1;
            rg2.dx = dx; rg2.dz = dz; rg2.xmin = xmin; rg2.zmin = zmin; rg2.xmax = xmax; rg2.zmax = zmax;
            fsm_compute_slowness2d<T><<<blocks, 64, 0, stream>>>(rg2, d_s.p, d_rx.p, n, d_out.p);
        }
        HIP_CHECK(hipGetLastError());
        HIP_CHECK(hipMemcpyAsync(out, d_out.p, sizeof(T) * n, hipMemcpyDeviceToHost, stream));
        HIP_CHECK(hipStreamSynchronize(stream));
    }

    void interp_grid_coords(int slot, int n, const T* p, T* out) {
        if (n <= 0) return;
        const int nc = ncoord();
        d_rx.reserve((size_t)nc * n);
        d_out.reserve(n);
        HIP_CHECK(hipMemcpyAsync(d_rx.p, p, sizeof(T) * nc * n, hipMemcpyHostToDevice, stream));
        const T* tt = tt_ptr(slot);
        const int blocks = (n + 127) / 128;
        if (dim == 3)
            fsm_interp3d<T><<<blocks, 128, 0, stream>>>(tt, NS, d_rx.p, d_out.p, n, (int)ncx + 1, (int)ncy + 1, (int)ncz + 1, dx, xmin, ymin, zmin);
        else
            fsm_interp2d<T><<<blocks, 128, 0, stream>>>(tt, NS, d_rx.p, d_out.p, n, (int)ncx + 1, (int)ncz + 1, dx, dz, xmin, zmin);
        HIP_CHECK(hipGetLastError());
        HIP_CHECK(hipMemcpyAsync(out, d_out.p, sizeof(T) * n, hipMemcpyDeviceToHost, stream));
        HIP_CHECK(hipStreamSynchronize(stream));
    }

    void interp_batch(const std::vector<int>& sl, const std::vector<int>& sr, const int* rx_off, const T* rx, T* tt_out) {
        const int nc = ncoord();
        size_t n = 0;
        for (int s2 : sr) n += (size_t)(rx_off[s2 + 1] - rx_off[s2]);
        if (n == 0) return;
        std::vector<T> p(nc * n), o(n);
        std::vector<int> so(n);
        size_t k = 0;
        for (size_t b = 0; b < sl.size(); ++b) {
            const int m = rx_off[sr[b] + 1] - rx_off[sr[b]];
            std::memcpy(p.data() + nc * k, rx + (size_t)nc * rx_off[sr[b]], sizeof(T) * nc * m);
// ... 2557 lines not shown
}
int ttcr_fsm_slot_rays_size(const ttcr_fsm_grid* g, int slot, size_t* n_rays, size_t* n_points) {
    return guarded_on(g, [&] {
        if (!n_rays || !n_points) throw ValueError("null output pointer");
        g->impl->slot_rays_size(slot, n_rays, n_points);
    });
}
int ttcr_fsm_get_slot_rays(const ttcr_fsm_grid* g, int slot, long long* offsets, void* pts) {
    return guarded_on(g, [&] { g->impl->get_slot_rays(slot, offsets, pts); });
}

int ttcr_fsm_raytrace_multi(ttcr_fsm_grid* g, int n_src, const int* tx_off, const void* tx, const void* t0,
                            const int* rx_off, const void* rx, void* tt_out) {
    return guarded_on(g, [&] { g->impl->raytrace_multi(n_src, tx_off, tx, t0, rx_off, rx, tt_out, -1); });
}

int ttcr_fsm_get_tt(ttcr_fsm_grid* g, int slot, void* out, size_t n) {
    return guarded_on(g, [&] { g->impl->get_tt(slot, out, n); });
}
int ttcr_fsm_get_tt_device(ttcr_fsm_grid* g, int slot, void** d_ptr) {
    return guarded_on(g, [&] {
        if (!d_ptr) throw ValueError("null output pointer");
        *d_ptr = g->impl->tt_device(slot);
    });
}
int ttcr_fsm_get_tt_device_view(ttcr_fsm_grid* g, int slot, void** d_ptr, size_t* stride) {
    return guarded_on(g, [&] {
        if (!d_ptr || !stride) throw ValueError("null output pointer");
        *d_ptr = g->impl->tt_device_view(slot, stride);
    });
}
int ttcr_fsm_interp(ttcr_fsm_grid* g, int slot, int n_pts, const void* pts, void* tt_out) {
    return guarded_on(g, [&] { g->impl->interp(slot, n_pts, pts, tt_out); });
}
int ttcr_fsm_compute_slowness(ttcr_fsm_grid* g, int n_pts, const void* pts, int translated, void* out) {
    return guarded_on(g, [&] { g->impl->compute_slowness(n_pts, pts, translated != 0, out); });
}
int ttcr_fsm_get_niter(ttcr_fsm_grid* g, int slot, int* niter, int* niterw) {
    return guarded_on(g, [&] { g->impl->get_niter(slot, niter, niterw); });
}
int ttcr_fsm_get_changes(ttcr_fsm_grid* g, int slot, double* first_order, int n_first, double* weno, int n_weno) {
    return guarded_on(g, [&] {
        if ((n_first > 0 && !first_order) || (n_weno > 0 && !weno) || n_first < 0 || n_weno < 0) throw ValueError("bad output buffers");
        g->impl->get_changes(slot, first_order, n_first, weno, n_weno);
    });
}
int ttcr_fsm_get_reference_changes(ttcr_fsm_grid* g, int slot, double* first_order, int n_first, double* weno, int n_weno) {
    return guarded_on(g, [&] {
        if ((n_first > 0 && !first_order) || (n_weno > 0 && !weno) || n_first < 0 || n_weno < 0) throw ValueError("bad output buffers");
        g->impl->get_reference_changes(slot, first_order, n_first, weno, n_weno);
    });
}
int ttcr_fsm_n_slots(const ttcr_fsm_grid* g) { return g->impl->n_slots; }
size_t ttcr_fsm_n_nodes(const ttcr_fsm_grid* g) { return g->impl->n_nodes; }
size_t ttcr_fsm_n_cells(const ttcr_fsm_grid* g) { return g->impl->n_cells; }

int ttcr_fsm_set_option(ttcr_fsm_grid* g, const char* key, double value) {
    return guarded_on(g, [&] { g->impl->apply_option(std::string(key ? key : ""), value); });
}

int ttcr_fsm_rays_size(const ttcr_fsm_grid* g, size_t* n_rays, size_t* n_points) {
    return guarded_on(g, [&] { g->impl->rays_size(n_rays, n_points); });
}
int ttcr_fsm_get_rays(const ttcr_fsm_grid* g, long long* offsets, void* pts) {
    return guarded_on(g, [&] { g->impl->get_rays(offsets, pts); });
}

int ttcr_fsm_last_timing(const ttcr_fsm_grid* g, ttcr_fsm_timing* out) {
    return guarded_on(g, [&] {
        const Timing& t = g->impl->timing;
        out->sweep_ms = t.sweep_ms;
        out->total_ms = t.total_ms;
        out->kernel_launches = t.launches;
        out->node_updates = t.node_updates;
        out->evaluated_updates = t.evaluated_updates;
        out->iterations = t.iterations;
        out->n_sources = t.n_sources;
    });
}

int ttcr_fsm_stopping_stats(const ttcr_fsm_grid* g, long long* reference_sums, long long* reference_sums_missed, long long* rounds) {
    return guarded_on(g, [&] { g->impl->stopping_stats(reference_sums, reference_sums_missed, rounds); });
}
int ttcr_fsm_prefill_swaps(const ttcr_fsm_grid* g, long long* swaps) {
    return guarded_on(g, [&] { if (swaps) *swaps = g->impl->prefill_swap_count(); });
}
int ttcr_fsm_prefill_inline_fills(const ttcr_fsm_grid* g, long long* fills) {
    return guarded_on(g, [&] { if (fills) *fills = g->impl->prefill_inline_count(); });
}
int ttcr_fsm_reference_change(ttcr_fsm_grid* g, const void* times, const void* field, int parallel, void* out) {
    return guarded_on(g, [&] {
        if (!times || !field || !out) throw ValueError("ttcr_fsm_reference_change: null argument");
        g->impl->reference_change_host(times, field, parallel != 0, out);
    });
}

int ttcr_fsm_last_kernel(const ttcr_fsm_grid* g, char* buf, size_t n) {
    return guarded_on(g, [&] {
        if (!buf || n == 0) throw ValueError("ttcr_fsm_last_kernel: no buffer");
        const std::string k = g->impl->kernel_name();
        std::snprintf(buf, n, "%s", k.c_str());
    });
}

#ifndef TTCR_BUILD_ID
#define TTCR_BUILD_ID "unknown"
#endif
int ttcr_fsm_unit_order(int dim, int dtype, int stage, int by_time, uint32_t nnx, uint32_t nny, uint32_t nnz, uint32_t* out,
                        size_t capacity, size_t* n_units) {
    return guarded([&] {
        if (dim != 2 && dim != 3) throw ValueError("dim must be 2 or 3");
        if (dtype != TTCR_F32 && dtype != TTCR_F64) throw ValueError("dtype must be TTCR_F32 or TTCR_F64");
        if (stage != 0 && stage != 1) throw ValueError("stage must be 0 (first order) or 1 (WENO)");
        if (nnx < 2 || nnz < 2 || (dim == 3 && nny < 2)) throw ValueError("grid needs at least two nodes per axis");
        if (!n_units) throw ValueError("null unit count");
        const uint32_t NF = dim == 3 ? nnx : nnz, NJ = dim == 3 ? nny : nnx, NK = dim == 3 ? nnz : 1;
        int PJ, PK, C;
        if (dtype == TTCR_F32) {
            PJ = dim == 3 ? TileCfg<float, 3>::PJ : TileCfg<float, 2>::PJ; PK = dim == 3 ? TileCfg<float, 3>::PK : 1;
            C = dim == 3 ? ChunkCfg<float, 3>::C : ChunkCfg<float, 2>::C;
        } else {
            PJ = dim == 3 ? TileCfg<double, 3>::PJ : TileCfg<double, 2>::PJ; PK = dim == 3 ? TileCfg<double, 3>::PK : 1;
            C = dim == 3 ? ChunkCfg<double, 3>::C : ChunkCfg<double, 2>::C;
        }
        const uint64_t npj = ((uint64_t)NJ + PJ - 1) / PJ, npk = ((uint64_t)NK + PK - 1) / PK;
        if (NF >= (1u << 30) || npj >= (1u << 14) || npk >= (1u << 14)) throw ValueError("grid too large for the patch index of the sweep kernel");
        *n_units = (size_t)(npj * npk) * (dim == 3 ? 8 : 4);
        if (!out) return;
        if (capacity < *n_units) throw ValueError("output buffer too small for the units of the launch");
        const std::vector<uint32_t> xs = fsm_xs_order(dim, (int)NF, (int)NJ, (int)NK, PJ, PK, C, stage == 0 ? 1 : 2, by_time != 0,
                                                      fsm_diag_order((int)npj, (int)npk));
        std::copy(xs.begin(), xs.end(), out);
    });
}

int ttcr_fsm_prefill_slice(int dtype, uint64_t n_el, uint32_t n_tickets, uint32_t ticket, uint64_t* slice_len, uint64_t* begin, uint64_t* end) {
    return guarded([&] {
        if (dtype != TTCR_F32 && dtype != TTCR_F64) throw ValueError("dtype must be TTCR_F32 or TTCR_F64");
        if (n_tickets == 0) throw ValueError("a launch has at least one ticket");
        const size_t slice = fsm_fill_slice_len((size_t)n_el, n_tickets, dtype == TTCR_F32 ? 4 : 2);
        size_t b = 0, e = 0;
        fsm_fill_slice_range((size_t)n_el, slice, ticket, &b, &e);
        if (slice_len) *slice_len = slice;
        if (begin) *begin = b;
        if (end) *end = e;
    });
}

const char* ttcr_fsm_build_id(void) { return TTCR_BUILD_ID; }

}
```

ttcr_amd/csrc/fsm_kernels.h:

```cpp
#pragma once
#include <hip/hip_runtime.h>
#include <stdint.h>
#include <type_traits>

#include "fsm_prefill_slices.h"

namespace ttcr_amd {

constexpr int FSM_BRICK = 16;

template <typename T> struct real_traits;
template <> struct real_traits<float> {
    static __host__ __device__ constexpr float max() { return 3.402823466e+38f; }
    static __device__ __forceinline__ float inf() { return __builtin_huge_valf(); }
};
template <> struct real_traits<double> {
    static __host__ __device__ constexpr double max() { return 1.7976931348623157e+308; }
    static __device__ __forceinline__ double inf() { return __builtin_huge_val(); }
};

__device__ __forceinline__ uint32_t idx_u32(double v) { return v < 0 ? 0u : (v >= 4294967295.0 ? 4294967295u : (uint32_t)v); }

__device__ __forceinline__ float rmin(float a, float b) { return a < b ? a : b; }
__device__ __forceinline__ double rmin(double a, double b) { return a < b ? a : b; }
__device__ __forceinline__ float rmax(float a, float b) { return a < b ? b : a; }
__device__ __forceinline__ double rmax(double a, double b) { return a < b ? b : a; }

__device__ __forceinline__ bool wave_any(bool p) { return __builtin_amdgcn_ballot_w64(p) != 0ull; }
__device__ __forceinline__ unsigned long long lanes_gt(float a, float b) { return __builtin_amdgcn_fcmpf(a, b, 2); }
__device__ __forceinline__ unsigned long long lanes_gt(double a, double b) { return __builtin_amdgcn_fcmp(a, b, 2); }

__device__ __forceinline__ double sqrt_disc(double x) {
    double y = __builtin_amdgcn_rsq(x);
    double g = x * y;
    double h = 0.5 * y;
    double e = __builtin_fma(-h, g, 0.5);
    g = __builtin_fma(g, e, g);
    h = __builtin_fma(h, e, h);
    double d = __builtin_fma(-g, g, x);
    g = __builtin_fma(d, h, g);
    d = __builtin_fma(-g, g, x);
    g = __builtin_fma(d, h, g);
    return x == 0.0 ? x : g;
}
__device__ __forceinline__ double sqrt_disc_pos(double x) {
    double y = __builtin_amdgcn_rsq(x);
    double g = x * y;
    double h = 0.5 * y;
    double e = __builtin_fma(-h, g, 0.5);
    g = __builtin_fma(g, e, g);
    h = __builtin_fma(h, e, h);
    double d = __builtin_fma(-g, g, x);
    g = __builtin_fma(d, h, g);
    d = __builtin_fma(-g, g, x);
    return __builtin_fma(d, h, g);
}

__device__ __forceinline__ float update3(float ax, float ay, float az, float s, float dx, unsigned long long live_lanes) {
    const float a1 = __builtin_fminf(__builtin_fminf(ax, ay), az);
    const float a3 = __builtin_fmaxf(__builtin_fmaxf(ax, ay), az);
    const float a2 = __builtin_amdgcn_fmed3f(ax, ay, az);
    const float fh = s * dx;
    const float t1 = a1 + fh;
    float t = t1;
    const unsigned long long beyond1d = lanes_gt(t1, a2) & live_lanes;
    if (beyond1d != 0ull) {
        const double d1 = a1, d2 = a2, d3 = a3, dfh = fh;
        double r = -d1 * d1;
        r = __builtin_fma(d1, d2, r);
        r = __builtin_fma(-d2, d2, r);
        r = __builtin_fma(d1, d3, r);
        r = __builtin_fma(d2, d3, r);
        r = __builtin_fma(-d3, d3, r);
        r = __builtin_fma(r, 2.0, (3.0 * dfh) * dfh);
        const float s12 = a1 + a2;
        const float s123 = s12 + a3;
        const float t3 = (float)((1. / 3.) * ((double)s123 + sqrt_disc_pos(r)));
        const float u = a3 - a1, v = a3 - a2;
        const float fh2 = fh * fh;
        const float slack = fh2 - (u * u + v * v);
        const float thr = __builtin_fmaf(4e-6f * fh, __builtin_fabsf(a1) + __builtin_fabsf(a3), __builtin_fmaf(4e-6f, fh2, 0x1p-120f));
        if ((beyond1d & ~lanes_gt(slack, thr)) != 0ull) {
            const float df = a1 - a2;
            const float df2 = df * df;
            const double disc2 = __builtin_fma(dfh * dfh, 2.0, -(double)df2);
            const float t2 = (float)(0.5 * ((double)s12 + sqrt_disc_pos(disc2)));
            t = t1 > a2 ? (t2 > a3 ? t3 : t2) : t1;
        } else {
// ... 278 lines not shown
    bool changed = false;

    __syncthreads();
    FSM_PROF_MARK(1)

    T own[NQ];
#pragma unroll
    for (int q = 0; q < NQ; ++q) own[q] = Tt[row * RS + q];

#pragma unroll
    for (int q = 1; q <= BL; ++q) {
        bool active = (q >= qa) & (q <= qb);
        if (near_src && active) {
            const int ip = L0 - 1 + q - jp - kp;
            const uint32_t n = colbase + (rf ? NF - 1 - ip : ip);
            active = !((Fz[n >> 5] >> (n & 31)) & 1u);
        }
        const T c = own[q];
        const T af = vmin(own[q - 1], own[q + 1]);
        const T aj = vmin(Tt[(row - 1) * RS + q - 1], Tt[(row + 1) * RS + q + 1]);
        const T s = sv[q - 1];
        T t;
        if (IS3D) {
            const T ak = vmin(Tt[(row - RJ) * RS + q - 1], Tt[(row + RJ) * RS + q + 1]);
            t = update3(ak, aj, af, s, dx, __builtin_amdgcn_ballot_w64(active));
        } else {
            t = variant == 1 ? update2(aj, af, s, dx) : update2_xz(aj, af, s, dx, dz);
        }
        const bool acc = active & (t < c);
        const T nv = acc ? t : c;
        dec += acc ? c - t : (T)0;
        changed |= acc;
        own[q] = nv;
        Tt[row * RS + q] = nv;
        __syncthreads();
    }

    FSM_PROF_MARK(2)
    if (FSM_ENABLE_PROF && a.prof && tid == 0) atomicAdd(a.prof + 4, 1ull);
    if (__syncthreads_or(changed)) {
        for (int f = tid; f < NT * BL; f += NT) {
            const int c = f / BL, q = f - c * BL;
            const int cj = c % PJ, ck = c / PJ;
            const int jq = j0 + cj, kq = k0 + ck;
            const int ip = L0 + q - jq - kq;
            if (jq < NJ && kq < NK && ip >= 0 && ip < NF) {
                const int i = rf ? NF - 1 - ip : ip;
                const int j = rj ? NJ - 1 - jq : jq;
                const int k = rk ? NK - 1 - kq : kq;
                const int r2 = IS3D ? (ck + 1) * RJ + cj + 1 : cj + 1;
                Tg[(size_t)(((uint32_t)k * NJ + j) * NF + i) * ts] = Tt[r2 * RS + q + 1];
            }
        }
        double accd = (double)dec;
#pragma unroll
        for (int off = 32; off > 0; off >>= 1) accd += __shfl_down(accd, off, 64);
        if ((tid & 63) == 0 && accd != 0.0) atomicAdd(a.change + slot, accd);
        FSM_PROF_MARK(3)
    }
}

template <typename T>
struct PersistArgs {
    SweepArgs<T> s;
    const uint32_t* order;
    int* sync;
    int n_patches, batch;
    unsigned long long timeout_ticks;
    int* stamp;
    const int* iter_ptr;
    unsigned long long* evals;
    int nbf, nbj, nbk;
    int dir, ndir;
    int skip;
    unsigned long long* cmap;
    int cw;
    unsigned long long* sw;
    int n_sw_groups, n_sw_sweeps;
    const T* ssh;
    size_t ssh_stride;
    T* fill_dst;
    size_t fill_slice;
    size_t fill_n;
};



__device__ __forceinline__ float ld_sc1(const float* p) {
    return __uint_as_float(__hip_atomic_load((const unsigned int*)p, __ATOMIC_RELAXED, __HIP_MEMORY_SCOPE_AGENT));
}
__device__ __forceinline__ double ld_sc1(const double* p) {
    return __longlong_as_double(__hip_atomic_load((const long long*)p, __ATOMIC_RELAXED, __HIP_MEMORY_SCOPE_AGENT));
}
__device__ __forceinline__ void st_sc1(float* p, float v) {
    __hip_atomic_store((unsigned int*)p, __float_as_uint(v), __ATOMIC_RELAXED, __HIP_MEMORY_SCOPE_AGENT);
}
__device__ __forceinline__ void st_sc1(double* p, double v) {
    __hip_atomic_store((long long*)p, __double_as_longlong(v), __ATOMIC_RELAXED, __HIP_MEMORY_SCOPE_AGENT);
}

__device__ __forceinline__ double div_h2(double x, double h2, double r2) {
    const double q0 = x * r2;
    return __builtin_fma(__builtin_fma(-q0, h2, x), r2, q0);
}

__device__ __forceinline__ float weno_fwd(float v1, float v2, float v3, float v4, float h, double r2) {
    const float eps = 1.1920928955078125e-07f;
    const float num = (float)(((double)v4 - 2.0 * (double)v3) + (double)v2);
    const float den = (float)(((double)v3 - 2.0 * (double)v2) + (double)v1);
    const float r = (eps + num * num) / (eps + den * den);
    const float w = (float)(1.0 / (1.0 + (2.0 * (double)r) * (double)r));
    const float d31 = v3 - v1;
    const double h2 = 2.0 * (double)h;
    const double ap = div_h2((1.0 - (double)w) * (double)d31, h2, r2) +
                      div_h2((double)w * ((-(double)v4 + 4.0 * (double)v3) - 3.0 * (double)v2), h2, r2);
    return v2 + h * (float)ap;
}
__device__ __forceinline__ float weno_bwd(float v0, float v1, float v2, float v3, float h, double r2) {
    const float eps = 1.1920928955078125e-07f;
    const float num = (float)(((double)v2 - 2.0 * (double)v1) + (double)v0);
    const float den = (float)(((double)v3 - 2.0 * (double)v2) + (double)v1);
    const float r = (eps + num * num) / (eps + den * den);
    const float w = (float)(1.0 / (1.0 + (2.0 * (double)r) * (double)r));
    const float d31 = v3 - v1;
    const double h2 = 2.0 * (double)h;
    const double am = div_h2((1.0 - (double)w) * (double)d31, h2, r2) +
                      div_h2((double)w * ((3.0 * (double)v2 - 4.0 * (double)v1) + (double)v0), h2, r2);
    return v2 - h * (float)am;
}
__device__ __forceinline__ double weno_fwd(double v1, double v2, double v3, double v4, double h, double) {
    const double eps = 2.220446049250313e-16;
    const double num = (v4 - 2.0 * v3 + v2);
    const double den = (v3 - 2.0 * v2 + v1);
    const double r = (eps + num * num) / (eps + den * den);
    const double w = 1.0 / (1.0 + 2.0 * r * r);
    const double ap = (1.0 - w) * (v3 - v1) / (2.0 * h) + w * (-v4 + 4.0 * v3 - 3.0 * v2) / (2.0 * h);
    return v2 + h * ap;
}
__device__ __forceinline__ double weno_bwd(double v0, double v1, double v2, double v3, double h, double) {
    const double eps = 2.220446049250313e-16;
    const double num = (v2 - 2.0 * v1 + v0);
    const double den = (v3 - 2.0 * v2 + v1);
    const double r = (eps + num * num) / (eps + den * den);
    const double w = 1.0 / (1.0 + 2.0 * r * r);
    const double am = (1.0 - w) * (v3 - v1) / (2.0 * h) + w * (3.0 * v2 - 4.0 * v1 + v0) / (2.0 * h);
    return v2 - h * am;
}

template <typename T>
__device__ __forceinline__ T weno_axis(T m2, T m1, T c, T p1, T p2, int idx, int n, T h, double r2) {
    const bool c0 = idx == 0;
    const bool c1 = !c0 && idx == 1;
    const bool cn = !c0 && !c1 && idx == n;
    const bool cm = !c0 && !c1 && !cn && idx == n - 1;
    const T F = weno_fwd(m1, c, p1, p2, h, r2);
    const T B = weno_bwd(m2, m1, c, p1, h, r2);
    T a = cm ? B : F;
    const T t = c1 ? m1 : (cm ? p1 : B);
    a = a < t ? a : t;
    return c0 ? p1 : (cn ? m1 : a);
}

#ifndef FSM_WENO_PLAIN
#define FSM_WENO_PLAIN 0
#endif
__device__ __forceinline__ float weno_quot_tame(float A, float B, float y) {
// ... 96 lines not shown

__device__ __forceinline__ float solve3_literal(float a1, float a2, float a3, float fh) {
    if (a1 > a2) { const float w = a1; a1 = a2; a2 = w; }
    if (a1 > a3) { const float w = a1; a1 = a3; a3 = w; }
    if (a2 > a3) { const float w = a2; a2 = a3; a3 = w; }
    float t = a1 + fh;
    if (t > a2) {
        const double d1 = a1, d2 = a2, dfh = fh;
        const float df = a1 - a2;
        const float df2 = df * df;
        t = (float)(0.5 * ((double)(a1 + a2) + __builtin_sqrt(__builtin_fma(dfh * dfh, 2.0, -(double)df2))));
        if (t > a3) {
            const double d3 = a3;
            double r = (-2.0 * d1) * d1;
            r = __builtin_fma(2.0 * d1, d2, r);
            r = __builtin_fma(-2.0 * d2, d2, r);
            r = __builtin_fma(2.0 * d1, d3, r);
            r = __builtin_fma(2.0 * d2, d3, r);
            r = __builtin_fma(-2.0 * d3, d3, r);
            r = __builtin_fma(3.0 * dfh, dfh, r);
            t = (float)((1. / 3.) * ((double)((a1 + a2) + a3) + __builtin_sqrt(r)));
        }
    }
    return t;
}
__device__ __forceinline__ double solve3_literal(double a1, double a2, double a3, double fh) {
    if (a1 > a2) { const double w = a1; a1 = a2; a2 = w; }
    if (a1 > a3) { const double w = a1; a1 = a3; a3 = w; }
    if (a2 > a3) { const double w = a2; a2 = a3; a3 = w; }
    double t = a1 + fh;
    if (t > a2) {
        t = 0.5 * (a1 + a2 + __builtin_sqrt(2. * fh * fh - (a1 - a2) * (a1 - a2)));
        if (t > a3) {
            t = 1. / 3. * ((a1 + a2 + a3) + __builtin_sqrt(-2. * a1 * a1 + 2. * a1 * a2 - 2. * a2 * a2 + 2. * a1 * a3 +
                                                            2. * a2 * a3 - 2. * a3 * a3 + 3. * fh * fh));
        }
    }
    return t;
}

__device__ __forceinline__ float weno_axis_fast(float m2, float m1, float c, float p1, float p2, int idx, int n) {
    const float eps = 1.1920928955078125e-07f;
    const float d0 = c - m1, d1 = p1 - c, d2 = p2 - p1, dm = m1 - m2;
    const float den = d1 - d0, nF = d2 - d1, nB = d0 - dm;
    const float y = __builtin_amdgcn_rcpf(__builtin_fmaf(den, den, eps));
    const float rF = __builtin_fmaf(nF, nF, eps) * y, rB = __builtin_fmaf(nB, nB, eps) * y;
    const float wF = __builtin_amdgcn_rcpf(__builtin_fmaf(2.0f * rF, rF, 1.0f));
    const float wB = __builtin_amdgcn_rcpf(__builtin_fmaf(2.0f * rB, rB, 1.0f));
    const float d31 = p1 - m1;
    const float F = __builtin_fmaf(0.5f, __builtin_fmaf(wF, __builtin_fmaf(3.0f, d1, -d2) - d31, d31), c);
    const float B = __builtin_fmaf(-0.5f, __builtin_fmaf(wB, __builtin_fmaf(3.0f, d0, -dm) - d31, d31), c);
    const bool c0 = idx == 0;
    const bool c1 = !c0 && idx == 1;
    const bool cn = !c0 && !c1 && idx == n;
    const bool cm = !c0 && !c1 && !cn && idx == n - 1;
    float a = cm ? B : F;
    const float t = c1 ? m1 : (cm ? p1 : B);
    a = a < t ? a : t;
    return c0 ? p1 : (cn ? m1 : a);
}
__device__ __forceinline__ float solve3_literal_fast(float a1, float a2, float a3, float fh) {
    if (a1 > a2) { const float w = a1; a1 = a2; a2 = w; }
    if (a1 > a3) { const float w = a1; a1 = a3; a3 = w; }
    if (a2 > a3) { const float w = a2; a2 = a3; a3 = w; }
    const float t1 = a1 + fh;
    const float df = a1 - a2, d3 = a3 - a1;
    const float df2 = df * df;
    const float t2 = 0.5f * ((a1 + a2) + __builtin_amdgcn_sqrtf(__builtin_fmaf(2.0f * fh, fh, -df2)));
    const float e = d3 + df;
    const float disc3 = __builtin_fmaf(3.0f * fh, fh, -(df2 + __builtin_fmaf(d3, d3, e * e)));
    const float t3 = __builtin_fmaf(1.0f / 3.0f, (d3 - df) + __builtin_amdgcn_sqrtf(disc3), a1);
    return t1 > a2 ? (t2 > a3 ? t3 : t2) : t1;
}

#ifndef FSM_POLL_SLEEP
#define FSM_POLL_SLEEP 2
#endif
#ifndef FSM_MINW
#define FSM_MINW 1
#endif
#ifndef FSM_SLAB_WORDS
#define FSM_SLAB_WORDS 32
#endif
#define FSM_FIN 0x3ffffff0
#ifndef FSM_SKIP_ABL
#define FSM_SKIP_ABL 0
#endif
#ifndef FSM_EARLY_PUB
#define FSM_EARLY_PUB 0
#endif
__device__ __forceinline__ float lane_below(float x, float edge) {
    return __uint_as_float((unsigned)__builtin_amdgcn_update_dpp((int)__float_as_uint(edge), (int)__float_as_uint(x), 0x138, 0xf, 0xf, false));
}
__device__ __forceinline__ float lane_above(float x, float edge) {
    return __uint_as_float((unsigned)__builtin_amdgcn_update_dpp((int)__float_as_uint(edge), (int)__float_as_uint(x), 0x130, 0xf, 0xf, false));
}
__device__ __forceinline__ double lane_below(double x, double edge) {
    const unsigned long long u = (unsigned long long)__double_as_longlong(x), e = (unsigned long long)__double_as_longlong(edge);
    const unsigned lo = (unsigned)__builtin_amdgcn_update_dpp((int)(unsigned)e, (int)(unsigned)u, 0x138, 0xf, 0xf, false);
    const unsigned hi = (unsigned)__builtin_amdgcn_update_dpp((int)(unsigned)(e >> 32), (int)(unsigned)(u >> 32), 0x138, 0xf, 0xf, false);
    return __longlong_as_double((long long)(((unsigned long long)hi << 32) | lo));
}
__device__ __forceinline__ double lane_above(double x, double edge) {
    const unsigned long long u = (unsigned long long)__double_as_longlong(x), e = (unsigned long long)__double_as_longlong(edge);
    const unsigned lo = (unsigned)__builtin_amdgcn_update_dpp((int)(unsigned)e, (int)(unsigned)u, 0x130, 0xf, 0xf, false);
    const unsigned hi = (unsigned)__builtin_amdgcn_update_dpp((int)(unsigned)(e >> 32), (int)(unsigned)(u >> 32), 0x130, 0xf, 0xf, false);
    return __longlong_as_double((long long)(((unsigned long long)hi << 32) | lo));
}

template <typename T, int NS> struct Pack;
template <typename T> struct Pack<T, 1> { T v[1]; };
template <typename T> struct alignas(2 * sizeof(T)) Pack<T, 2> { T v[2]; };

template <typename T, int NS>
__device__ __forceinline__ Pack<T, NS> pack_fill(T x) {
    Pack<T, NS> p;
#pragma unroll
    for (int l = 0; l < NS; ++l) p.v[l] = x;
    return p;
}
__device__ __forceinline__ Pack<float, 1> ld_sc1(const Pack<float, 1>* p) { Pack<float, 1> r; r.v[0] = ld_sc1(&p->v[0]); return r; }
__device__ __forceinline__ Pack<double, 1> ld_sc1(const Pack<double, 1>* p) { Pack<double, 1> r; r.v[0] = ld_sc1(&p->v[0]); return r; }
__device__ __forceinline__ Pack<float, 2> ld_sc1(const Pack<float, 2>* p) {
    const unsigned long long u = __hip_atomic_load((const unsigned long long*)p, __ATOMIC_RELAXED, __HIP_MEMORY_SCOPE_AGENT);
    Pack<float, 2> r;
    r.v[0] = __uint_as_float((unsigned)u);
    r.v[1] = __uint_as_float((unsigned)(u >> 32));
    return r;
}
__device__ __forceinline__ Pack<double, 2> ld_sc1(const Pack<double, 2>* p) {
    Pack<double, 2> r;
    r.v[0] = ld_sc1(&p->v[0]);
    r.v[1] = ld_sc1(&p->v[1]);
    return r;
}
__device__ __forceinline__ void st_sc1(Pack<float, 1>* p, Pack<float, 1> x) { st_sc1(&p->v[0], x.v[0]); }
__device__ __forceinline__ void st_sc1(Pack<double, 1>* p, Pack<double, 1> x) { st_sc1(&p->v[0], x.v[0]); }
__device__ __forceinline__ void st_sc1(Pack<float, 2>* p, Pack<float, 2> x) {
    const unsigned long long u = (unsigned long long)__float_as_uint(x.v[0]) | ((unsigned long long)__float_as_uint(x.v[1]) << 32);
    __hip_atomic_store((unsigned long long*)p, u, __ATOMIC_RELAXED, __HIP_MEMORY_SCOPE_AGENT);
}
__device__ __forceinline__ void st_sc1(Pack<double, 2>* p, Pack<double, 2> x) {
    st_sc1(&p->v[0], x.v[0]);
    st_sc1(&p->v[1], x.v[1]);
}

__host__ __device__ constexpr bool fsm_looped(bool is3d, int h) { return is3d && h == 1; }

__device__ __forceinline__ int kmaxp_of(int k0, int NK, int PK) { return (k0 + PK < NK ? k0 + PK : NK) - 1; }
template <typename T, int PJ, int PK, int C, bool IS3D, bool SKIP, int H, int NS, bool XS, bool PRE, int AR = 0>
__device__ __forceinline__ bool fsm_sweep_unit(const PersistArgs<T>& pa) {
    static_assert(AR == 0 || std::is_same<T, float>::value, "tolerance-grade arithmetic: fp32 kernels");
    constexpr bool LOOPED = fsm_looped(IS3D, H);
    using P = Pack<T, NS>;
    constexpr int NT = PJ * PK;
    constexpr int RJ = PJ + 2 * H;
    constexpr int NROWS = IS3D ? RJ * (PK + 2 * H) : RJ;
    constexpr int NQ = C + 2 * H;
    constexpr int RS = NQ | 1;
    constexpr int NUP = IS3D ? H * (PJ + PK) : H;
    constexpr int NDH = IS3D ? H * (PJ + PK) : H;
    constexpr int RPI = NT / C;
    constexpr int NOWN = C;
    constexpr int NHI = (NDH + RPI - 1) / RPI;
    constexpr int NUPI = (NUP + RPI - 1) / RPI;
    static_assert(NT % C == 0 && (IS3D || PK == 1) && C <= FSM_BRICK && (H == 1 || H == 2), "tile shape");
    static_assert(C - 1 <= FSM_XPAD, "the rows of a chunk are read from the sheared copies without a wrap");
    static_assert(!(SKIP && FSM_EARLY_PUB > 0), "FSM_EARLY_PUB is a tuning option of the kernels without exact skipping");
    const SweepArgs<T>& a = pa.s;
    const unsigned epoch = (unsigned)pa.iter_ptr[1] + (XS ? 0u : (unsigned)pa.dir);
    const int e2 = (int)(epoch % 3u) + 1;
    auto dec_prog = [&](int raw_) -> int { return (int)((unsigned)raw_ >> 30) == e2 ? (raw_ & 0x3fffffff) : 0; };
    auto ld_raw = [&](const int* p_) -> int { return __hip_atomic_load(p_, __ATOMIC_RELAXED, __HIP_MEMORY_SCOPE_AGENT); };
    auto ld_prog = [&](const int* p_) -> int { return dec_prog(ld_raw(p_)); };
    auto st_prog = [&](int* p_, int v_) {
        __hip_atomic_store(p_, (int)(((unsigned)e2 << 30) | (unsigned)v_), __ATOMIC_RELAXED, __HIP_MEMORY_SCOPE_AGENT);
    };
    auto ld_cmap = [&](const unsigned long long* p_) -> unsigned {
        const unsigned long long v_ = __hip_atomic_load(p_, __ATOMIC_RELAXED, __HIP_MEMORY_SCOPE_AGENT);
        return (unsigned)(v_ >> 32) == epoch ? (unsigned)v_ : 0u;
    };
    auto st_cmap = [&](unsigned long long* p_, unsigned v_) {
        __hip_atomic_store(p_, ((unsigned long long)epoch << 32) | v_, __ATOMIC_RELAXED, __HIP_MEMORY_SCOPE_AGENT);
    };

    __shared__ P Tt[NROWS * RS];
    __shared__ int s_ticket, s_abort;
    __shared__ int s_anychg;
    constexpr int SLABW = SKIP ? FSM_SLAB_WORDS : 1;
    __shared__ unsigned s_stamped[SKIP ? 9 : 1][SLABW];
    __shared__ unsigned s_slab[SLABW];
    __shared__ int s_next, s_act;
    __shared__ int s_cwi[2], s_cwl[2];
    __shared__ unsigned s_cwv[2];
    __shared__ int s_mywi;
    __shared__ unsigned s_mywv[2];
    enum { U_THR, U_RSJLO, U_RSKLO, U_RSNJ, U_RSNK, U_LCF, U_UPLCF0, U_UPLCF1, U_HIST, U_EVER, U_UCHG, U_PENDV, U_LCHG, U_N };
    __shared__ int s_u[U_N];

    int tid = threadIdx.x;
    if constexpr (LOOPED) asm volatile("" : "+v"(tid));
    unsigned long long prof_t = (FSM_ENABLE_PROF && a.prof) ? wall_clock64() : 0ull;
    unsigned long long pacc[6] = {0, 0, 0, 0, 0, 0};
    unsigned pchunks = 0;
    unsigned long long twait = 0;
    constexpr int FSM_TRACE_UNITS = FSM_ENABLE_PROF == 2 ? (1 << 20) : 65536;
    const unsigned long long trace_t0 = prof_t;
    unsigned long long* prec = nullptr;
    __shared__ unsigned long long s_pacc[FSM_ENABLE_PROF == 2 ? 8 : 1];
    if constexpr (FSM_ENABLE_PROF == 2) {
        if (tid == 0) {
            for (int q = 0; q < 6; ++q) s_pacc[q] = 0;
            s_pacc[6] = prof_t;
        }
    }
#define FSM_PMARK(slot_)                                                          \
    if constexpr (FSM_ENABLE_PROF == 2) {                                         \
        if (a.prof && tid == 0) {                                                 \
            const unsigned long long now_ = wall_clock64();                       \
            s_pacc[slot_] += now_ - s_pacc[6];                                    \
            s_pacc[6] = now_;                                                     \
        }                                                                         \
    }                                                                             \
    if (FSM_ENABLE_PROF == 1 && a.prof && tid == 0) {                             \
        const unsigned long long now_ = wall_clock64();                           \
        pacc[slot_] += now_ - prof_t;                                             \
        prof_t = now_;                                                            \
         \
        if ((slot_) < 5 && prec && pchunks < 80u) prec[pchunks * 5u + (slot_)] = now_; \
    }
    const int NF = a.g.NF, NJ = a.g.NJ, NK = a.g.NK;
    const int npj = a.g.npj;
    auto prev_sweep_counter = [&](int d, int TJ_, int TK_, int z_, int lane) -> const int* {
        const int pd = d - 1;
        int crj, crk, prj, prk;
        if (IS3D) { crj = (d >> 1) & 1; crk = (d >> 2) & 1; prj = (pd >> 1) & 1; prk = (pd >> 2) & 1; }
        else { crj = (d == 1) | (d == 2); crk = 0; prj = (pd == 1) | (pd == 2); prk = 0; }
        const int j0_ = TJ_ * PJ, k0_ = TK_ * PK;
        const int jm_ = (j0_ + PJ < NJ ? j0_ + PJ : NJ) - 1, km_ = (k0_ + PK < NK ? k0_ + PK : NK) - 1;
        int ja = j0_ - 2 * H, jb = jm_ + 2 * H, ka = k0_ - 2 * H, kb = km_ + 2 * H;
        ja = ja < 0 ? 0 : ja; jb = jb > NJ - 1 ? NJ - 1 : jb;
        ka = ka < 0 ? 0 : ka; kb = kb > NK - 1 ? NK - 1 : kb;
        const int ja2 = (crj != prj) ? NJ - 1 - jb : ja, jb2 = (crj != prj) ? NJ - 1 - ja : jb;
        const int ka2 = (crk != prk) ? NK - 1 - kb : ka, kb2 = (crk != prk) ? NK - 1 - ka : kb;
        const int tja = ja2 / PJ, ntj = jb2 / PJ - tja + 1;
        const int tka = IS3D ? ka2 / PK : 0, ntk = IS3D ? kb2 / PK - tka + 1 : 1;
        const int ia = lane & 3, ib = lane >> 2;
        if (ia >= ntj || ib >= ntk) return nullptr;
        return pa.sync + 8 + ((size_t)pd * pa.batch + z_) * pa.n_patches + ((tka + ib) * npj + tja + ia);
    };
    if constexpr (LOOPED) __syncthreads();
    if (tid == 0) {
        const int t_ = atomicAdd(pa.sync + (epoch & 3u), 1);
        if (t_ == 0) __hip_atomic_store(pa.sync + ((epoch + 2u) & 3u), 0, __ATOMIC_RELAXED, __HIP_MEMORY_SCOPE_AGENT);
        s_ticket = t_;
    }
    if (LOOPED && tid == 1) s_abort = __hip_atomic_load(pa.sync + 4, __ATOMIC_RELAXED, __HIP_MEMORY_SCOPE_AGENT);
    __syncthreads();
    if (LOOPED && s_abort) return false;
    const int ticket = __builtin_amdgcn_readfirstlane(s_ticket);
    if (pa.fill_slice) {
        constexpr int VE = 16 / (int)sizeof(T);
        typedef T FillV __attribute__((ext_vector_type(VE)));
        size_t fb, fe;
        fsm_fill_slice_range(pa.fill_n, pa.fill_slice, (size_t)(unsigned)ticket, &fb, &fe);
        T* __restrict__ fdst = pa.fill_dst;
        T fmax = real_traits<T>::max();
        asm volatile("" : "+v"(fmax));
        FillV fv;
#pragma unroll
        for (int q = 0; q < VE; ++q) fv[q] = fmax;
        for (size_t i = fb + (size_t)tid * VE; i + VE <= fe; i += (size_t)NT * VE) *reinterpret_cast<FillV*>(fdst + i) = fv;
        const size_t rem = (fe - fb) % VE;
        if ((size_t)tid < rem) fdst[fe - rem + tid] = fmax;
    }
    const int oidx = ticket / pa.batch, z = ticket - oidx * pa.batch;
    if (oidx >= (XS ? pa.n_patches * pa.ndir : pa.n_patches)) return false;
    if (FSM_ENABLE_PROF == 1 && a.prof && ticket < 8192) prec = a.prof + 8 + 4 * 65536 + (size_t)ticket * 400;
    const uint32_t tile = pa.order[oidx];
    const int dir = XS ? (int)(tile >> 28) : pa.dir;
    const int TJ = XS ? (int)(tile & 0x3fffu) : (int)(tile & 0xffffu), TK = XS ? (int)((tile >> 14) & 0x3fffu) : (int)(tile >> 16);
// ... 235 lines not shown
                    if (q & 1) rowp += SRB;
                }
            } else {
#pragma unroll
                for (int q = 0; q < C; ++q) {
                    if (!(q & 1)) { sv[q] = ld_row(1); rowp += SRB; } else sv[q] = ld_row(0);
                }
            }
        } else {
#pragma unroll
            for (int q = 0; q < C; ++q) {
                sv[q] = ld_row(0);
                rowp += SRB;
            }
        }
        x = rev ? x - C : x + C;
        if (x < 0 || x >= M) { x %= M; x = x < 0 ? x + M : x; }
        xs_next = x;
        xs_level = L + C;
        const int sL = sf * L;
#pragma unroll
        for (int it = 0; it < NOWN + NHI; ++it) {
            P v = PFILL;
            if ((unsigned)(L + ipb[it]) < (unsigned)NF) v = XS ? ld_sc1(Tg + (abase[it] + sL)) : Tg[abase[it] + sL];
            tv[it] = v;
        }
    };

    unsigned long long nevals = 0;

    T dec[NS];
#pragma unroll
    for (int l = 0; l < NS; ++l) dec[l] = 0;
    P carry[2 * H];
#pragma unroll
    for (int q = 0; q < 2 * H; ++q) carry[q] = PFILL;
    bool have_prev = false;
    int pref_for = -(1 << 30);
    int pending = 0;
    int n_done = 0;
    int pre_j = -1, pre_k = -1;
    int smp_j = 0, smp_k = 0;
    P uvn[NUPI];
    int uvn_for = -(1 << 30);
    int near_lo[NS], near_hi[NS];
    {
        const int jlo = rj ? NJ - 1 - jmaxp : j0, jhi = rj ? NJ - 1 - j0 : jmaxp;
        const int klo = rk ? NK - 1 - kmaxp : k0, khi = rk ? NK - 1 - k0 : kmaxp;
#pragma unroll
        for (int l = 0; l < NS; ++l) {
            const int* b6 = bb + 6 * l;
            const int b0 = rf ? NF - 1 - b6[1] : b6[0], b1 = rf ? NF - 1 - b6[0] : b6[1];
            const bool jk = !(jhi < b6[2] || jlo > b6[3] || khi < b6[4] || klo > b6[5]) && b0 <= NF - 1 && b1 >= 0;
            near_lo[l] = jk ? b0 - (C - 1) + j0 + k0 : 1;
            near_hi[l] = jk ? b1 + jmaxp + kmaxp : 0;
        }
    }
    if (!FSM_EXP_NOWAIT && XS && dir > 0 && !chase) {
        if (tid < 16) {
            const int* pp = prev_sweep_counter(dir, TJ, TK, z, tid);
            if (pp) {
                const unsigned long long t0 = wall_clock64();
                int spins = 0;
                while (ld_prog(pp) < (SKIP ? FSM_FIN : 0x3fffffff)) {
                    if ((++spins & 63) == 0) {
                        if (__hip_atomic_load(pa.sync + 4, __ATOMIC_RELAXED, __HIP_MEMORY_SCOPE_AGENT)) break;
                        if (wall_clock64() - t0 > pa.timeout_ticks) {
                            __hip_atomic_store(pa.sync + 4, 1, __ATOMIC_RELAXED, __HIP_MEMORY_SCOPE_AGENT);
                            break;
                        }
                    }
                    __builtin_amdgcn_s_sleep(8);
                }
            }
        }
        __syncthreads();
    }
    if (CHASE_OK && chase) chase_wait(Lc - C, -1, false);
    if (!SKIP) { issue_static(Lc); pref_for = Lc; }
    if constexpr (SKIP) {
        const int nsw = (pa.nbf + 31) >> 5;
        for (int w = tid; w < nsw; w += NT) s_slab[w] = 0u;
        for (int w = tid; w < 9 * SLABW; w += NT) s_stamped[w / SLABW][w % SLABW] = 0u;
        if (tid == 0) {
            s_cwi[0] = -1; s_cwi[1] = -1; s_mywi = -1;
            const int ja = j0 - H < 0 ? 0 : j0 - H, jb = jmaxp + H > NJ - 1 ? NJ - 1 : jmaxp + H;
            const int ka = k0 - H < 0 ? 0 : k0 - H, kb = kmaxp + H > NK - 1 ? NK - 1 : kmaxp + H;
            const int jlo = (rj ? NJ - 1 - jb : ja) / FSM_BRICK, jhi = (rj ? NJ - 1 - ja : jb) / FSM_BRICK;
            const int klo = (rk ? NK - 1 - kb : ka) / FSM_BRICK, khi = (rk ? NK - 1 - ka : kb) / FSM_BRICK;
            s_u[U_RSJLO] = jlo; s_u[U_RSNJ] = jhi - jlo + 1;
            s_u[U_RSKLO] = klo; s_u[U_RSNK] = khi - klo + 1;
            const int sg = pa.ndir * pa.iter_ptr[0] + dir + 1;
            s_u[U_THR] = pa.skip == 2 ? -(1 << 30) : (sg - 1 > 0 ? sg - 1 : 0);
            s_u[U_LCF] = Lc;
            const int lsj = Ls - PJ, lsk = Ls - PK, mu = TJ + TK - 1;
            s_u[U_UPLCF0] = lsj - (((lsj - mu) % C + C) % C);
            s_u[U_UPLCF1] = lsk - (((lsk - mu) % C + C) % C);
            s_u[U_HIST] = 0; s_u[U_EVER] = 0; s_u[U_UCHG] = 0; s_u[U_PENDV] = 0; s_u[U_LCHG] = 0;
        }
        __syncthreads();
        {
            const int jlo = s_u[U_RSJLO], nj = s_u[U_RSNJ], klo = s_u[U_RSKLO], nk = s_u[U_RSNK], thr = s_u[U_THR];
            const int* __restrict__ stamp = pa.stamp + (size_t)grp * pa.nbf * pa.nbj * pa.nbk;
            const int total = pa.nbf * nj * nk;
            for (int b = tid; b < total; b += NT) {
                const int bf = b % pa.nbf, jk = b / pa.nbf;
                const int bj = jlo + jk % nj, bk = klo + jk / nj;
                const int v = __hip_atomic_load(stamp + ((size_t)bk * pa.nbj + bj) * pa.nbf + bf, __ATOMIC_RELAXED, __HIP_MEMORY_SCOPE_AGENT);
                if (v >= thr) atomicOr(&s_slab[bf >> 5], 1u << (bf & 31));
            }
        }
        __syncthreads();
    }
    FSM_PMARK(5)
    const unsigned long long trace_t1 = (FSM_ENABLE_PROF && a.prof) ? wall_clock64() : 0ull;
    auto cmap_of = [&](int pidx, int e) -> unsigned long long* {
        return pa.cmap + ((((size_t)(XS ? dir : 0) * pa.batch + z) * pa.n_patches + (size_t)pidx) * 2 + e) * pa.cw;
    };
    auto slab_any = [&](int flo, int fhi) -> bool {
        const int b0 = flo / FSM_BRICK, b1 = fhi / FSM_BRICK;
        for (int w = b0 >> 5; w <= (b1 >> 5); ++w) {
            const int lo = w == (b0 >> 5) ? (b0 & 31) : 0, hi = w == (b1 >> 5) ? (b1 & 31) : 31;
            const unsigned msk = (hi == 31 ? 0xffffffffu : ((2u << hi) - 1u)) & ~((1u << lo) - 1u);
            if (s_slab[w] & msk) return true;
        }
        return false;
    };
    auto chunk_frange = [&](int L, int ext, int& flo, int& fhi) {
        int ia = L - ext - jmaxp - kmaxp, ib = L + C - 1 + ext - j0 - k0;
        ia = ia < 0 ? 0 : ia;
        ib = ib > NF - 1 ? NF - 1 : ib;
        flo = rf ? NF - 1 - ib : ia;
        fhi = rf ? NF - 1 - ia : ib;
    };
    auto up_dirty = [&](int v, int need, int e) -> bool {
        if (v >= FSM_FIN && !((v >> e) & 1)) return false;
        for (int p2 = 0; p2 < H; ++p2) {
            const int nd = need - p2 * C;
            const int ulcf = s_u[U_UPLCF0 + e];
            const int ciu = (nd - C - ulcf) / C;
            if (nd - C - ulcf < 0) continue;
            int bit;
            const int d = v >= FSM_FIN ? 4 : ((v >> 8) - nd) / C;
            if (d < 4) {
                bit = (v >> (2 * d + e)) & 1;
            } else {
                const int w = ciu >> 5;
                if (w >= pa.cw) continue;
                if (s_cwi[e] != w || s_cwl[e] < nd) {
                    s_cwl[e] = v >= FSM_FIN ? 0x7fffffff : (v >> 8);
                    const unsigned long long* um = cmap_of(e == 0 ? TK * npj + TJ - 1 : (TK - 1) * npj + TJ, e);
                    s_cwv[e] = ld_cmap(um + w);
                    s_cwi[e] = w;
                }
                bit = (s_cwv[e] >> (ciu & 31)) & 1u;
            }
            if (bit) return true;
        }
        return false;
    };
    auto poll_until = [&](const int* ptr, int want, bool& ok) -> int {
        unsigned long long t0 = 0;
        int spins = 0;
        for (;;) {
            const int v = ld_prog(ptr);
            if (v >= want) {
                if (FSM_ENABLE_PROF == 2 && spins) twait += wall_clock64() - t0;
                return v;
            }
            if (spins == 0) t0 = wall_clock64();
            if ((++spins & 63) == 0) {
                if (__hip_atomic_load(pa.sync + 4, __ATOMIC_RELAXED, __HIP_MEMORY_SCOPE_AGENT)) { ok = false; return v; }
                if (wall_clock64() - t0 > pa.timeout_ticks) {
                    __hip_atomic_store(pa.sync + 4, 1, __ATOMIC_RELAXED, __HIP_MEMORY_SCOPE_AGENT);
                    ok = false;
                    return v;
                }
            }
            __builtin_amdgcn_s_sleep(FSM_POLL_SLEEP);
        }
    };
    for (; Lc <= Le; Lc += C) {
        if constexpr (PRE) {
            pre_j = dec_prog(smp_j);
            pre_k = dec_prog(smp_k);
        }
        if constexpr (SKIP) {
            FSM_PMARK(0)
            if (tid == 0) {
                int L = Lc, act = 1, h = s_u[U_HIST];
                const int lcf = s_u[U_LCF];
                const bool follow = s_u[U_LCHG] != 0 && L <= Le;
                s_u[U_LCHG] = 0;
                for (;;) {
                    if (L > Le) { act = 0; break; }
                    if (follow) {
                        const int need8 = (L + C - 1) << 8;
                        bool ok = true;
                        if (up_j && pre_j < need8) pre_j = poll_until(up_j, need8, ok);
                        if (up_k && ok && pre_k < need8) pre_k = poll_until(up_k, need8, ok);
                        if (!ok) act = 0;
                        break;
                    }
                    const int need = L + C - 1, need8 = need << 8;
                    int vj = FSM_FIN, vk = FSM_FIN;
                    bool ok = true;
                    if (up_j) { vj = pre_j >= need8 ? pre_j : poll_until(up_j, need8, ok); pre_j = vj; }
                    if (up_k && ok) { vk = pre_k >= need8 ? pre_k : poll_until(up_k, need8, ok); pre_k = vk; }
                    if (!ok) { act = 0; break; }
                    if (L == lcf && vj >= FSM_FIN && !(vj & 1) && vk >= FSM_FIN && !(vk & 2)) {
                        bool any = false;
                        for (int w = 0; w < ((pa.nbf + 31) >> 5); ++w) any |= s_slab[w] != 0u;
                        if (!any) {
                            st_prog(my_prog, FSM_FIN);
                            L = Le + 1;
                            act = 0;
                            break;
                        }
                    }
                    int flo, fhi;
                    chunk_frange(L, H, flo, fhi);
                    bool dirty = slab_any(flo, fhi);
                    if (!dirty && up_j) dirty = up_dirty(vj, need, 0);
                    if (!dirty && up_k) dirty = up_dirty(vk, need, 1);
                    if (dirty) break;
                    if (pending) { act = 2; break; }
                    L += C;
                    h = (h << 2) & 0xff;
                    if (L > Le && s_u[U_UCHG]) {
                        s_u[U_PENDV] = FSM_FIN | s_u[U_EVER];
                    } else {
                        st_prog(my_prog, L > Le ? (FSM_FIN | s_u[U_EVER]) : ((L << 8) | h));
                    }
                }
                s_u[U_HIST] = h;
                s_next = L;
                s_act = act;
            }
            __syncthreads();
            const int act = __builtin_amdgcn_readfirstlane(s_act), Ln = __builtin_amdgcn_readfirstlane(s_next);
            if (Ln != Lc) {
                have_prev = false;
                Lc = Ln;
            }
            if (act == 2) {
                asm volatile("s_waitcnt vmcnt(0)" ::: "memory");
                __syncthreads();
                if (tid == 0) st_prog(my_prog, s_u[U_PENDV]);
                pending = 0;
                Lc -= C;
                continue;
            }
            if (act == 0) break;
        }
        const int L0 = Lc;
        const int eoff = jp + kp - L0;
        const int ea = col_ok ? (eoff > 0 ? eoff : 0) : C;
        const int eb = eoff + NF - 1 < C - 1 ? eoff + NF - 1 : C - 1;
        if constexpr (!SKIP) { FSM_PMARK(0) }

        if constexpr (!SKIP) {
        if (CHASE_OK && chase) {
            chase_wait(L0, pre_j, true);
        } else if (tid == 0 && (up_j || up_k) && !((up_j ? pre_j : 0x3fffffff) >= L0 + C - 1 && (up_k ? pre_k : 0x3fffffff) >= L0 + C - 1)) {
            const int need = L0 + C - 1;
            unsigned long long t0 = 0;
            int spins = 0;
            for (;;) {
                const int vj = up_j ? ld_prog(up_j) : need;
                const int vk = up_k ? ld_prog(up_k) : need;
                if (vj >= need && vk >= need) break;
                if (spins == 0) t0 = wall_clock64();
                if ((++spins & 63) == 0) {
                    if (__hip_atomic_load(pa.sync + 4, __ATOMIC_RELAXED, __HIP_MEMORY_SCOPE_AGENT)) break;
                    if (wall_clock64() - t0 > pa.timeout_ticks) {
                        __hip_atomic_store(pa.sync + 4, 1, __ATOMIC_RELAXED, __HIP_MEMORY_SCOPE_AGENT);
                        break;
                    }
                }
                __builtin_amdgcn_s_sleep(FSM_POLL_SLEEP);
            }
        }
        __syncthreads();
        }
        if (tid == 0) s_anychg = 0;
        FSM_PMARK(1)
        if (pref_for != L0) issue_static(L0);
        nevals += (eb >= ea) ? (unsigned)(eb - ea + 1) : 0u;

        P uv[NUPI];
        if (PRE && uvn_for == L0) {
#pragma unroll
            for (int it = 0; it < NUPI; ++it) uv[it] = uvn[it];
        } else {
#pragma unroll
            for (int it = 0; it < NUPI; ++it) {
                P v = PFILL;
                if ((unsigned)(L0 + uipb[it]) < (unsigned)NF) v = ld_sc1(Tg + (uabase[it] + sf * L0));
                uv[it] = v;
            }
        }
        P xv = PFILL;
        if (H == 2 && (unsigned)(L0 + xipb) < (unsigned)NF) {
            const P* src = Tg + (xabase + sf * L0);
            if (x_up || XS) xv = ld_sc1(src); else xv = *src;
// ... 41 lines not shown
        if (PRE && (tid & 63) == 0 && Lc + C <= Le) {
            if (up_j) smp_j = ld_raw(up_j);
            if (up_k) smp_k = ld_raw(up_k);
        }
        if (PRE && CHASE_OK && chase_ptr && Lc + C <= Le)
            smp_j = ld_raw(chase_ptr);

        bool near_src[NS];
#pragma unroll
        for (int l = 0; l < NS; ++l) near_src[l] = L0 >= near_lo[l] && L0 <= near_hi[l];

        P own[NQ];
#pragma unroll
        for (int q = 0; q < 2 * H; ++q) own[q] = carry[q];
#pragma unroll
        for (int q = 2 * H; q < NQ; ++q) own[q] = Tt[row * RS + q];
        T sc[C];
#pragma unroll
        for (int q = 0; q < C; ++q) sc[q] = rev ? sv[C - 1 - q] : sv[q];
        FSM_PMARK(2)

        if (Lc + C <= Le) { issue_static(Lc + C); pref_for = Lc + C; }

        constexpr bool WAVE2D = !IS3D && NT == 64 && H == 1;
        P hup[WAVE2D ? C : 1], hdn[WAVE2D ? C : 1];
        if (WAVE2D) {
#pragma unroll
            for (int ee = 0; ee < C; ++ee) {
                hup[ee] = Tt[(H - 1) * RS + ee + H - 1];
                hdn[ee] = Tt[(PJ + H) * RS + ee + H + 1];
            }
        }
        bool changed = false;
        constexpr bool DUP = H == 1 && !IS3D;
        if constexpr (!DUP) {
#define FSM_SIMPLE false
#define FSM_VAR 0
#include "fsm_march_levels.inc"
#undef FSM_SIMPLE
#undef FSM_VAR
        } else {
            bool near_any = false;
#pragma unroll
            for (int l = 0; l < NS; ++l) near_any |= near_src[l];
            const bool full_wave = !near_any && __builtin_amdgcn_ballot_w64(ea == 0 && eb == C - 1) == ~0ull;
            if (!full_wave) {
#define FSM_SIMPLE false
#define FSM_VAR 0
#include "fsm_march_levels.inc"
#undef FSM_SIMPLE
#undef FSM_VAR
            } else if (variant == 1) {
#define FSM_SIMPLE true
#define FSM_VAR 1
#include "fsm_march_levels.inc"
#undef FSM_SIMPLE
#undef FSM_VAR
            } else {
#define FSM_SIMPLE true
#define FSM_VAR 2
#include "fsm_march_levels.inc"
#undef FSM_SIMPLE
#undef FSM_VAR
            }
        }
#pragma unroll
        for (int q = 0; q < 2 * H; ++q) carry[q] = own[C + q];
        FSM_PMARK(3)
        if (FSM_ENABLE_PROF) ++pchunks;

        if constexpr (SKIP) {
            const bool ej = changed && jp + H > jmaxp, ek = IS3D && changed && kp + H > kmaxp;
            const int f = (wave_any(changed) ? 1 : 0) | (wave_any(ej) ? 2 : 0) | (wave_any(ek) ? 4 : 0);
            if (f && (tid & 63) == 0) atomicOr(&s_anychg, f);
            if (!(FSM_SKIP_ABL & 2) && changed) {
                const int ip0 = L0 - jp - kp;
                const int ia = ip0 + ea, ib = ip0 + eb;
                const int ba = (rf ? NF - 1 - ib : ia) / FSM_BRICK, bb2 = (rf ? NF - 1 - ia : ib) / FSM_BRICK;
                const int my_bj = (rj ? NJ - 1 - jp : jp) / FSM_BRICK - s_u[U_RSJLO], my_bk = (rk ? NK - 1 - kp : kp) / FSM_BRICK - s_u[U_RSKLO];
                const int jk = my_bk * s_u[U_RSNJ] + my_bj;
                atomicOr(&s_stamped[jk][ba >> 5], 1u << (ba & 31));
                if (bb2 != ba) atomicOr(&s_stamped[jk][bb2 >> 5], 1u << (bb2 & 31));
            }
        } else {
            if (wave_any(changed) && (tid & 63) == 0) s_anychg = 1;
        }
        __syncthreads();
        const int chg_flags = SKIP ? __builtin_amdgcn_readfirstlane(s_anychg) : s_anychg;
        const bool any_changed = chg_flags != 0;
        if (any_changed) {
#pragma unroll
            for (int it = 0; it < NOWN; ++it) {
                const int ipm = L0 + ipb[it] - H;
                if ((unsigned)ipm < (unsigned)NF) {
                    const int rid = rsub + RPI * it;
                    const int cj = rid % PJ, ck = rid / PJ;
                    P* dst = Tg + (abase[it] + sf * (L0 - H));
                    const P v = Tt[lrow[it] - H];
                    if (XS || cj >= PJ - H || (IS3D && ck >= PK - H)) st_sc1(dst, v); else *dst = v;
                }
            }
        }
        if constexpr (SKIP) {
            if (!(FSM_SKIP_ABL & 4) && tid == 0) {
                if (any_changed) {
                    int flo, fhi;
                    chunk_frange(L0, 0, flo, fhi);
                    for (int b = flo / FSM_BRICK; b <= fhi / FSM_BRICK; ++b) s_slab[b >> 5] |= 1u << (b & 31);
                    const int ci = (L0 - s_u[U_LCF]) / C, w = ci >> 5;
                    if ((chg_flags & 6) && w < pa.cw) {
                        if (s_mywi != w) { s_mywi = w; s_mywv[0] = 0u; s_mywv[1] = 0u; }
                        for (int e2 = 0; e2 < 2; ++e2)
                            if (chg_flags & (2 << e2)) {
                                s_mywv[e2] |= 1u << (ci & 31);
                                st_cmap(cmap_of(TK * npj + TJ, e2) + w, s_mywv[e2]);
                            }
                    }
                    s_u[U_UCHG] = 1;
                    s_u[U_LCHG] = 1;
                }
                const int h2 = ((s_u[U_HIST] << 2) | (chg_flags >> 1)) & 0xff, ev2 = s_u[U_EVER] | (chg_flags >> 1);
                s_u[U_HIST] = h2;
                s_u[U_EVER] = ev2;
                s_u[U_PENDV] = Lc + C > Le ? (FSM_FIN | ev2) : (((Lc + C) << 8) | h2);
            }
        }
        if constexpr (SKIP) pending = 1;
        else pending = Lc + C > Le ? 0x3fffffff : Lc + C;
        if (FSM_EARLY_PUB > 0 && n_done < FSM_EARLY_PUB) {
            asm volatile("s_waitcnt vmcnt(0)" ::: "memory");
            __syncthreads();
            if (tid == 0) st_prog(my_prog, SKIP ? s_u[U_PENDV] : pending);
            pending = 0;
        }
        ++n_done;
        FSM_PMARK(4)
    }
    if constexpr (SKIP) {
        __syncthreads();
        if (s_u[U_UCHG]) {
            const int nsw = (pa.nbf + 31) >> 5;
            const int rs_jlo = s_u[U_RSJLO], rs_nj = s_u[U_RSNJ], rs_klo = s_u[U_RSKLO], njk = rs_nj * s_u[U_RSNK];
            int* __restrict__ stamp = pa.stamp + (size_t)grp * pa.nbf * pa.nbj * pa.nbk;
            const int sigma = pa.ndir * pa.iter_ptr[0] + dir + 1;
            for (int q = tid; q < njk * nsw * 32; q += NT) {
                const int jk = q / (nsw * 32), bf = q % (nsw * 32);
                if (bf < pa.nbf && ((s_stamped[jk][bf >> 5] >> (bf & 31)) & 1u))
                    atomicMax(stamp + ((size_t)(rs_klo + jk / rs_nj) * pa.nbj + rs_jlo + jk % rs_nj) * pa.nbf + bf, sigma);
            }
            pending = 1;
        }
    }
    if (pending) {
        asm volatile("s_waitcnt vmcnt(0)" ::: "memory");
        __syncthreads();
        if (tid == 0) st_prog(my_prog, SKIP ? s_u[U_PENDV] : pending);
    }
    if constexpr (SKIP) {
        const int sigma0 = pa.ndir * pa.iter_ptr[0] + dir;
        if (tid == 0 && pa.sw && sigma0 < pa.n_sw_sweeps)
            atomicAdd(pa.sw + (size_t)sigma0 * pa.n_sw_groups + grp, 1ull | (s_u[U_UCHG] ? (1ull << 32) : 0ull));
    }

    if (FSM_ENABLE_PROF && a.prof && tid == 0) {
        if constexpr (FSM_ENABLE_PROF == 2) {
            for (int q = 0; q < 6; ++q) atomicAdd(a.prof + q, s_pacc[q]);
            atomicAdd(a.prof + 6, 1ull);
            atomicAdd(a.prof + 7, (unsigned long long)pchunks);
        }
        if (FSM_ENABLE_PROF == 1) {
#pragma unroll
            for (int q = 0; q < 6; ++q) atomicAdd(a.prof + q, pacc[q]);
            atomicAdd(a.prof + 6, 1ull);
            atomicAdd(a.prof + 7, (unsigned long long)pchunks);
        }
        if (ticket < FSM_TRACE_UNITS) {
            unsigned long long* tr = a.prof + 8 + 4 * (size_t)ticket;
            tr[0] = trace_t0; tr[1] = FSM_ENABLE_PROF == 2 ? ((trace_t1 - trace_t0) & 0xffffffffull) | (twait << 32) : trace_t1; tr[2] = wall_clock64();
            tr[3] = (unsigned long long)TJ | ((unsigned long long)TK << 16) | ((unsigned long long)dir << 32) | ((unsigned long long)z << 40) |
                    ((unsigned long long)pchunks << 48);
        }
    }
#undef FSM_PMARK
#pragma unroll
    for (int off = 32; off > 0; off >>= 1) nevals += __shfl_down(nevals, off, 64);
#pragma unroll
    for (int l = 0; l < NS; ++l) {
        double accd = (double)dec[l];
#pragma unroll
        for (int off = 32; off > 0; off >>= 1) accd += __shfl_down(accd, off, 64);
        if ((tid & 63) == 0 && accd != 0.0) atomicAdd(a.change + grp * NS + l, accd);
        if ((tid & 63) == 0 && nevals && ((lm >> l) & 1)) atomicAdd(pa.evals + grp * NS + l, nevals);
    }
    return true;
}

template <typename T, int PJ, int PK, int C, bool IS3D, bool SKIP, int H, int NS, bool XS, bool PRE = false, int AR = 0>
#ifndef FSM_WENO_MINW
#define FSM_WENO_MINW FSM_MINW
#endif
__global__ __launch_bounds__(PJ* PK, (SKIP && IS3D && H == 1 && NS == 2 && sizeof(T) == 4) ? 3
                                     : (IS3D && H == 2 && NS == 1 && sizeof(T) == 4) ? FSM_WENO_MINW : FSM_MINW) void fsm_sweep_persistent(const PersistArgs<T> pa) {
    if constexpr (fsm_looped(IS3D, H)) {
        (void)pa;
        for (;;) {
            auto kp = __builtin_amdgcn_kernarg_segment_ptr();
            asm volatile("" : "+s"(kp));
            if (!fsm_sweep_unit<T, PJ, PK, C, IS3D, SKIP, H, NS, XS, PRE, AR>(*(const PersistArgs<T>*)kp)) break;
        }
    } else {
        fsm_sweep_unit<T, PJ, PK, C, IS3D, SKIP, H, NS, XS, PRE, AR>(pa);
    }
}

template <typename T>
struct Sweep45Args {
    T* tt;
    const T* s;
    const uint32_t* frozen;
    double* change;
    const int* slots;
    const int* lmask;
    int ts, by_group;
    int nnx, nnz;
    size_t n_nodes;
    uint32_t mask_words;
    T dx;
};

template <typename T, int NT>
__global__ __launch_bounds__(NT) void fsm_sweep45(const Sweep45Args<T> a) {
    constexpr int W = 16, C = 8;
    __shared__ T ring[NT * W];
    int slot;
    if (a.by_group) {
        const int z = blockIdx.x / a.ts, l = blockIdx.x % a.ts;
        const int grp = a.slots[z];
        if (grp < 0 || !((a.lmask[z] >> l) & 1)) return;
        slot = grp * a.ts + l;
    } else {
        slot = a.slots[blockIdx.x];
        if (slot < 0) return;
    }
    T* __restrict__ Tg = a.tt + ((size_t)(slot / a.ts) * a.n_nodes * a.ts + slot % a.ts);
    const uint32_t* __restrict__ Fz = a.frozen + (size_t)slot * a.mask_words;
    const int nnx = a.nnx, nnz = a.nnz, ts = a.ts;
    const T TMAX = real_traits<T>::max();
    const int r = threadIdx.x;
    constexpr int S = NT - 2;
    double dec = 0;
    for (int dir = 0; dir < 4; ++dir) {
        const int ri = (dir == 1) | (dir == 2), rj = dir >> 1;
        for (int x0 = 0; x0 < nnx; x0 += S) {
            const int ncol = nnx - x0 < S ? nnx - x0 : S;
            const int nlev = 2 * (ncol - 1) + nnz;
            const int xp = x0 + r - 1;
            const bool col_in = xp >= 0 && xp < nnx && r <= ncol + 1;
            const bool own = r >= 1 && r <= ncol;
            const int i = ri ? nnx - 1 - xp : xp;
            const uint32_t rowbase = (uint32_t)(col_in ? i : 0) * nnz;
            auto load_levels = [&](int lo, T* v) {
#pragma unroll
                for (int e = 0; e < C; ++e) {
                    const int zp = lo + e - 2 * (r - 1);
                    const bool ok = col_in && zp >= 0 && zp < nnz;
                    const uint32_t n = rowbase + (rj ? nnz - 1 - zp : zp);
                    v[e] = ok ? ld_sc1(Tg + (size_t)n * ts) : TMAX;
                }
            };
            auto load_static = [&](int lo, T* sv, unsigned& fz) {
                fz = 0;
#pragma unroll
                for (int e = 0; e < C; ++e) {
                    const int zp = lo + e - 2 * (r - 1);
                    const bool ok = own && zp >= 0 && zp < nnz;
                    const uint32_t n = rowbase + (rj ? nnz - 1 - zp : zp);
                    sv[e] = ok ? a.s[n] : (T)0;
                    const bool frozen = ok ? ((Fz[n >> 5] >> (n & 31)) & 1u) : true;
                    fz |= (frozen ? 1u : 0u) << e;
                }
            };
            auto to_ring = [&](int lo, const T* v) {
#pragma unroll
                for (int e = 0; e < C; ++e) ring[r * W + ((lo + e) & (W - 1))] = v[e];
            };
            T vn[C], svn[C];
            unsigned fzn;
            load_levels(-4, vn);
            to_ring(-4, vn);
            load_levels(4, vn);
            load_static(0, svn, fzn);
            for (int L0 = 0; L0 < nlev; L0 += C) {
                T sv[C];
#pragma unroll
// ... 1694 lines not shown
```

ttcr_amd/rgrid.py:

```python
import collections
import ctypes as C
import math

import numpy as np

from . import _lib

_verbose = 0


def set_verbose(v):
    global _verbose
    _verbose = int(v)


def _ptr(a):
    return a.ctypes.data_as(C.c_void_p)


def _row_groups(a):
    key = np.ascontiguousarray(a, dtype=np.float64) + 0.0
    n = key.shape[0]
    if n == 0:
        return np.zeros(0, dtype=np.intp), np.zeros(1, dtype=np.intp), key
# ... 15 lines not shown
def _first_rows(a):
    order, bounds, _ = _row_groups(a)
    return np.sort(order[bounds[:-1]])


def _device_arg(device):
    if isinstance(device, (list, tuple, np.ndarray)):
        devs = tuple(int(d) for d in device)
        if not devs:
            raise ValueError("device list is empty")
        return devs if len(devs) > 1 else devs[0]
    return int(device)


class _GridBase:

    _dtype = np.float64
    _ndim = 3

    def __init__(self):
        self._h = C.c_void_p()
        self._lib = None

    def __del__(self):
        try:
            if self._lib is not None and self._h:
                self._lib.ttcr_fsm_destroy(self._h)
                self._h = C.c_void_p()
        except Exception:
            pass

    @property
    def n_threads(self):
        return self._n_threads

    @property
    def n_devices(self):
        return int(self._lib.ttcr_fsm_n_devices(self._h))

    def set_use_thread_pool(self, use_thread_pool):
        self._use_pool = bool(use_thread_pool)

    def set_traveltime_from_raypath(self, traveltime_from_raypath):
        self.set_option("tt_from_rp", 1 if traveltime_from_raypath else 0)
        self.tt_from_rp = bool(traveltime_from_raypath)

    def set_option(self, key, value):
        _lib.check(self._lib.ttcr_fsm_set_option(self._h, key.encode(), float(value)))

    def set_slowness_device(self, device_ptr, n):
        _lib.check(self._lib.ttcr_fsm_set_slowness_device(self._h, C.c_void_p(int(device_ptr)), int(n)))

    def get_niter(self, thread_no=0):
        a, b = C.c_int(), C.c_int()
        _lib.check(self._lib.ttcr_fsm_get_niter(self._h, int(thread_no), C.byref(a), C.byref(b)))
        return a.value

    def get_niterw(self, thread_no=0):
        a, b = C.c_int(), C.c_int()
        _lib.check(self._lib.ttcr_fsm_get_niter(self._h, int(thread_no), C.byref(a), C.byref(b)))
        return b.value

    def get_changes(self, thread_no=0):
        n1, n2 = self.get_niter(thread_no), self.get_niterw(thread_no)
        a, b = (C.c_double * max(n1, 1))(), (C.c_double * max(n2, 1))()
        _lib.check(self._lib.ttcr_fsm_get_changes(self._h, int(thread_no), a, n1, b, n2))
        return np.array(a[:n1]), np.array(b[:n2])

    def get_reference_changes(self, thread_no=0):
        n1, n2 = self.get_niter(thread_no), self.get_niterw(thread_no)
        a, b = (C.c_double * max(n1, 1))(), (C.c_double * max(n2, 1))()
        _lib.check(self._lib.ttcr_fsm_get_reference_changes(self._h, int(thread_no), a, n1, b, n2))
        return np.array(a[:n1]), np.array(b[:n2])

    def timing(self):
        t = _lib.Timing()
        _lib.check(self._lib.ttcr_fsm_last_timing(self._h, C.byref(t)))
        return {k: getattr(t, k) for k, _ in t._fields_}

    def stopping_stats(self):
        a, b, c = C.c_longlong(0), C.c_longlong(0), C.c_longlong(0)
        _lib.check(self._lib.ttcr_fsm_stopping_stats(self._h, C.byref(a), C.byref(b), C.byref(c)))
        return {"reference_sums": a.value, "reference_sums_missed": b.value, "rounds": c.value}

    def prefill_swaps(self):
        a = C.c_longlong(0)
        _lib.check(self._lib.ttcr_fsm_prefill_swaps(self._h, C.byref(a)))
        return a.value

    def prefill_inline_fills(self):
        a = C.c_longlong(0)
        _lib.check(self._lib.ttcr_fsm_prefill_inline_fills(self._h, C.byref(a)))
        return a.value

    def reference_change(self, times, field, parallel=True):
        dt = self._dtype
        a = np.ascontiguousarray(times, dtype=dt).ravel()
        b = np.ascontiguousarray(field, dtype=dt).ravel()
        n = self.get_number_of_nodes()
        if a.size != n or b.size != n:
            raise ValueError('reference_change: fields of get_number_of_nodes() values expected')
        out = np.zeros(1, dtype=dt)
        _lib.check(self._lib.ttcr_fsm_reference_change(self._h, a.ctypes.data, b.ctypes.data, 1 if parallel else 0, out.ctypes.data))
        return out[0]

    def last_kernel(self):
        buf = C.create_string_buffer(256)
        _lib.check(self._lib.ttcr_fsm_last_kernel(self._h, buf, 256))
        return buf.value.decode()

    def _flat_tt(self, thread_no):
        if thread_no >= self._n_threads:
            raise ValueError('Thread number is larger than number of threads')
        n = self.get_number_of_nodes()
        out = np.empty(n, dtype=self._dtype)
        _lib.check(self._lib.ttcr_fsm_get_tt(self._h, int(thread_no), _ptr(out), n))
        return out

    def get_s0(self, hypo, slowness=None):
        nd = self._ndim
        hypo = np.asarray(hypo)
        if hypo.ndim != 2 or hypo.shape[1] != nd + 2:
            raise ValueError('hypo should be npts x %d' % (nd + 2))
        src = hypo[:, 2:2 + nd]
        evID = hypo[:, 0]
        eid = np.sort(np.unique(evID))
        if slowness is not None:
            self.set_slowness(slowness)
        first = np.array([int(np.nonzero(evID == e)[0][0]) for e in eid], dtype=np.int64)
        pts = np.ascontiguousarray(src[first, :], dtype=self._dtype)
        out = np.empty(max(len(eid), 1), dtype=self._dtype)
        _lib.check(self._lib.ttcr_fsm_compute_slowness(self._h, len(eid), _ptr(pts), 0, _ptr(out)))
        s0 = np.zeros((src.shape[0],))
        for n, e in enumerate(eid):
            s0[evID == e] = out[n]
        return s0

    def tt_device_ptr(self, thread_no=0):
        p = C.c_void_p()
        _lib.check(self._lib.ttcr_fsm_get_tt_device(self._h, int(thread_no), C.byref(p)))
        return p.value

    def tt_device_view(self, thread_no=0):
        p, st = C.c_void_p(), C.c_size_t()
        _lib.check(self._lib.ttcr_fsm_get_tt_device_view(self._h, int(thread_no), C.byref(p), C.byref(st)))
        return p.value, st.value

    def to_vtk(self, fields, filename):
        from . import io as _io

        if self._ndim == 3:
            nodes, cells = (self._x.size, self._y.size, self._z.size), (self._x.size - 1, self._y.size - 1, self._z.size - 1)
            xyz = (self._x, self._y, self._z)
        else:
            nodes, cells = (self._x.size, self._z.size), (self._x.size - 1, self._z.size - 1)
            xyz = (self._x, np.array([0.0]), self._z)
        pd, cd = {}, {}
        for fn in fields:
            data = fields[fn]
            if isinstance(data, list):
                _io.write_vtp_lines(filename + '_' + fn + '.vtp', data)
                continue
            data = np.asarray(data)
            for shape, dest in ((nodes, pd), (cells, cd)):
                if data.size == int(np.prod(shape)):
                    if data.ndim == len(shape):
# ... 1591 lines not shown
```

Before: 96400.

## Add per-chunk dirty marks for precise skip decisions in 3D persistent sweeps

Adds a chunk-granular mark array. During each sweep, wavefront ballots of changed nodes record which downstream chunks of the next sweep direction depend on them, and those chunks are stamped with the current sweep id. The next sweep reads these marks into a shared bitmask and uses it instead of the coarser brick-slab test, so it can skip more unchanged chunks. This costs extra LDS, atomics, a per-source memset of the mark buffer, and a new kernel variant. It is enabled automatically only when the measured fraction of evaluated updates is low.

```diff
diff --git a/include/ttcr_amd.h b/include/ttcr_amd.h
--- a/include/ttcr_amd.h
+++ b/include/ttcr_amd.h
@@ -203,11 +203,16 @@
 int ttcr_fsm_last_timing(const ttcr_fsm_grid* g, ttcr_fsm_timing* out);
 int ttcr_fsm_stopping_stats(const ttcr_fsm_grid* g, long long* reference_sums, long long* reference_sums_missed, long long* rounds);
 int ttcr_fsm_prefill_swaps(const ttcr_fsm_grid* g, long long* swaps);
+int ttcr_fsm_mark_units(const ttcr_fsm_grid* g, long long* units);
 int ttcr_fsm_prefill_inline_fills(const ttcr_fsm_grid* g, long long* fills);
 int ttcr_fsm_reference_change(ttcr_fsm_grid* g, const void* times, const void* field, int parallel, void* out);
 int ttcr_fsm_last_kernel(const ttcr_fsm_grid* g, char* buf, size_t n);
 int ttcr_fsm_unit_order(int dim, int dtype, int stage, int by_time, uint32_t nnx, uint32_t nny, uint32_t nnz, uint32_t* out,
                         size_t capacity, size_t* n_units);
+int ttcr_fsm_chunk_marks(int NF, int NJ, int NK, int PJ, int PK, int C, int dir, int jc, int kc, int ia, int ib, int edges,
+                         int* out, size_t capacity, size_t* n);
+int ttcr_fsm_chunk_marks_row(int NF, int NJ, int NK, int PJ, int PK, int C, int dir, int jca, int jcb, int kc, int La, int Lb, int edges,
+                             int* out, size_t capacity, size_t* n);
 int ttcr_fsm_prefill_slice(int dtype, uint64_t n_el, uint32_t n_tickets, uint32_t ticket, uint64_t* slice_len, uint64_t* begin, uint64_t* end);
 const char* ttcr_fsm_build_id(void);
 
diff --git a/ttcr_amd/_lib.py b/ttcr_amd/_lib.py
--- a/ttcr_amd/_lib.py
+++ b/ttcr_amd/_lib.py
@@ -50,6 +50,9 @@
     "ttcr_fsm_last_kernel": (_I, [_P, C.c_char_p, C.c_size_t]),
     "ttcr_fsm_build_id": (C.c_char_p, []),
     "ttcr_fsm_unit_order": (_I, [_I, _I, _I, _I, _U32, _U32, _U32, C.POINTER(_U32), C.c_size_t, C.POINTER(C.c_size_t)]),
+    "ttcr_fsm_chunk_marks": (_I, [_I, _I, _I, _I, _I, _I, _I, _I, _I, _I, _I, _I, C.POINTER(_I), C.c_size_t, C.POINTER(C.c_size_t)]),
+    "ttcr_fsm_mark_units": (_I, [_P, C.POINTER(C.c_longlong)]),
+    "ttcr_fsm_chunk_marks_row": (_I, [_I, _I, _I, _I, _I, _I, _I, _I, _I, _I, _I, _I, _I, C.POINTER(_I), C.c_size_t, C.POINTER(C.c_size_t)]),
     "ttcr_fsm_stopping_stats": (_I, [_P, C.POINTER(C.c_longlong), C.POINTER(C.c_longlong), C.POINTER(C.c_longlong)]),
     "ttcr_fsm_prefill_swaps": (_I, [_P, C.POINTER(C.c_longlong)]),
     "ttcr_fsm_prefill_inline_fills": (_I, [_P, C.POINTER(C.c_longlong)]),
diff --git a/ttcr_amd/build.py b/ttcr_amd/build.py
--- a/ttcr_amd/build.py
+++ b/ttcr_amd/build.py
@@ -9,10 +9,10 @@
 INC = os.path.join("..", "..", "include", "ttcr_amd.h")
 UNITS = {
     "fsm_capi.hip": ([], ["fsm_capi.hip", "fsm_kernels.h", "fsm_fast_api.h", "fsm_march_levels.inc", "fsm_fast.hip", "fsm_tape_api.h",
-                          "fsm_tape.hip", "fsm_adjoint_api.h", "fsm_adjoint.hip", "fsm_normal.hip", "fsm_locate.hip", "fsm_unit_order.h", "fsm_prefill_slices.h", INC]),
-    "fsm_fast.hip": ([], ["fsm_fast.hip", "fsm_fast_api.h", "fsm_kernels.h", "fsm_march_levels.inc", "fsm_prefill_slices.h"]),
+                          "fsm_tape.hip", "fsm_adjoint_api.h", "fsm_adjoint.hip", "fsm_normal.hip", "fsm_locate.hip", "fsm_unit_order.h", "fsm_prefill_slices.h", "fsm_chunk_marks.h", INC]),
+    "fsm_fast.hip": ([], ["fsm_fast.hip", "fsm_fast_api.h", "fsm_kernels.h", "fsm_march_levels.inc", "fsm_prefill_slices.h", "fsm_chunk_marks.h"]),
     "fsm_tape.hip": ([], ["fsm_tape.hip", "fsm_tape_api.h"]),
-    "fsm_adjoint.hip": ([], ["fsm_adjoint.hip", "fsm_adjoint_api.h", "fsm_kernels.h", "fsm_march_levels.inc", "fsm_prefill_slices.h"]),
+    "fsm_adjoint.hip": ([], ["fsm_adjoint.hip", "fsm_adjoint_api.h", "fsm_kernels.h", "fsm_march_levels.inc", "fsm_prefill_slices.h", "fsm_chunk_marks.h"]),
     "fsm_normal.hip": ([], ["fsm_normal.hip", "fsm_adjoint_api.h"]),
     "fsm_locate.hip": ([], ["fsm_locate.hip", "fsm_adjoint_api.h"]),
 }
diff --git a/ttcr_amd/csrc/fsm_capi.hip b/ttcr_amd/csrc/fsm_capi.hip
--- a/ttcr_amd/csrc/fsm_capi.hip
+++ b/ttcr_amd/csrc/fsm_capi.hip
@@ -156,6 +156,7 @@
     int pair_by_distance = 1;
     virtual void set_pair_layout(int) {}
     virtual long long prefill_inline_count() const { return 0; }
+    virtual long long mark_unit_count() const { return 0; }
     virtual long long prefill_swap_count() const { return 0; }
     int lone_chunk = 16;
     int arith = 0;
@@ -182,6 +183,7 @@
     std::atomic<int> return_rays{0};
     int fixed_iters = 0, max_batch = 0, use_graph = 1;
     int skip = -1;
+    int skip_marks = -1;
     int mode = 2;
     Timing timing;
     std::string last_kernel;
@@ -196,6 +198,10 @@
         else if (k == "combine_window_us") combine_window_us = (int)value;
         else if (k == "mode") mode = (int)value;
         else if (k == "skip") skip = (int)value;
+        else if (k == "skip_marks") {
+            if (value != -1 && value != 0 && value != 1) throw ValueError("option 'skip_marks': -1 (default), 0 or 1");
+            skip_marks = (int)value;
+        }
         else if (k == "tt_from_rp") ttrp = value != 0;
         else if (k == "interp_vel") interp_vel = value != 0;
         else if (k == "return_rays") return_rays = value != 0;
@@ -305,6 +311,8 @@
     int n_patches = 0;
     int* h_abort = nullptr;
     DevBuf<int> d_stamp;
+    DevBuf<int> d_marks;
+    int mark_row = 0;
     DevBuf<unsigned long long> d_cmap;
     int cmap_words = 1;
     DevBuf<unsigned long long> d_sw;
@@ -404,7 +412,7 @@
         HIP_CHECK(hipHostMalloc((void**)&h_abort, sizeof(int)));
         *h_abort = 0;
         HIP_CHECK(hipHostMalloc((void**)&h_iter, 2 * sizeof(int)));
-        HIP_CHECK(hipHostMalloc((void**)&h_evals, sizeof(unsigned long long) * n_slots));
+        HIP_CHECK(hipHostMalloc((void**)&h_evals, sizeof(unsigned long long) * (n_slots + 1)));
         HIP_CHECK(hipMemsetAsync(d_tt.p, 0, n_nodes * tt_fields() * sizeof(T), stream));
 
         if (dim == 3) {
@@ -437,6 +445,9 @@
         nbk = (geom.NK + FSM_BRICK - 1) / FSM_BRICK;
         n_bricks = (size_t)nbf * nbj * nbk;
         d_stamp.reserve(n_bricks * n_slots);
+        if (dim == 3) {
+            mark_row = fsm_max_chunks(geom.NF, TileCfg<T, 3>::PJ, TileCfg<T, 3>::PK, 8);
+        }
         {
             const int PJ = dim == 3 ? TileCfg<T, 3>::PJ : TileCfg<T, 2>::PJ, PK = dim == 3 ? TileCfg<T, 3>::PK : 1;
             const int max_chunks = (geom.NF + 2 * (PJ + PK)) / 4 + 4;
@@ -447,7 +458,7 @@
             d_sw.reserve((size_t)sw_sweeps * n_slots);
         }
         d_iter.reserve(2);
-        d_evals.reserve(n_slots);
+        d_evals.reserve(n_slots + 1);
         if (dim == 2)
             HIP_CHECK(hipFuncSetAttribute(reinterpret_cast<const void*>(&fsm_sweep45_rows<T>),
                                           hipFuncAttributeMaxDynamicSharedMemorySize, 156 * 1024));
@@ -458,6 +469,7 @@
         if (const char* e = std::getenv("TTCR_FSM_TIME_ORDER_BELOW")) time_order_below = std::atoi(e);
         if (const char* e = std::getenv("TTCR_FSM_PRE_MIN")) pre_min = std::atoi(e);
         if (const char* e = std::getenv("TTCR_FSM_SKIP")) skip = std::atoi(e);
+        if (const char* e = std::getenv("TTCR_FSM_SKIP_MARKS")) skip_marks = std::atoi(e) < 0 ? -1 : std::atoi(e) != 0;
         if (const char* e = std::getenv("TTCR_FSM_SKIP_UNITS")) skip_units_min = std::atoi(e);
         if (const char* e = std::getenv("TTCR_FSM_SKIP_PROBE_UNITS")) skip_probe_min = std::atoi(e);
         if (const char* e = std::getenv("TTCR_FSM_RS_FIELDS")) rs_fields_max = (size_t)std::max(0, std::atoi(e));
@@ -549,6 +561,9 @@
         pa.sw = std::getenv("TTCR_FSM_NO_SW") ? nullptr : d_sw.p;
         pa.n_sw_groups = n_groups();
         pa.n_sw_sweeps = sw_sweeps;
+        pa.marks = nullptr;
+        pa.mcw = mark_row;
+        pa.mark_units = d_evals.p + n_slots;
         pa.fill_dst = nullptr;
         pa.fill_slice = 0;
         pa.fill_n = 0;
@@ -587,6 +602,21 @@
                     const hipError_t e = fsm_fast_launch(pa, fc, gridx.x, dyn_lds, stream);
                     if (e == hipErrorInvalidValue) throw std::logic_error("arith = 1: no such kernel (" + last_kernel + ")");
                     HIP_CHECK(e);
+                    return;
+                }
+            }
+            if constexpr (DIM == 3 && H == 1) {
+                const bool pre_k = NO_PRE ? false : pre;
+                if (marks_now(batch) && fsm_max_chunks(geom.NF, C::PJ, C::PK, CH) <= 32 * FSM_MARK_WORDS &&
+                    fsm_marks_kernel<T>(true, true, 1, NSV, true, pre_k, 0)) {
+                    pa.marks = d_marks.p;
+                    if constexpr (fsm_marks_kernel<T>(true, true, 1, NSV, true, false, 0)) {
+                        if (!pre_k) fsm_sweep_persistent<T, C::PJ, C::PK, CH, true, true, 1, NSV, true, false, 0, true><<<gridx, block, dyn_lds, stream>>>(pa);
+                    }
+                    if constexpr (!NO_PRE && fsm_marks_kernel<T>(true, true, 1, NSV, true, true, 0)) {
+                        if (pre_k) fsm_sweep_persistent<T, C::PJ, C::PK, CH, true, true, 1, NSV, true, true, 0, true><<<gridx, block, dyn_lds, stream>>>(pa);
+                    }
+                    HIP_CHECK(hipGetLastError());
                     return;
                 }
             }
@@ -953,6 +983,12 @@
         return (long long)n_patches * entries >= skip_units_min ? 1 : 0;
     }
     bool persistent_now() const { return mode >= 1 || stage == 1; }
+    bool marks_auto = true;
+    bool marks_now(int entries) const {
+        return dim == 3 && stage == 0 && mode == 2 && (skip_marks == 1 || (skip_marks < 0 && marks_auto)) && mark_row > 0 && arith == 0 && skip_now(entries);
+    }
+    long long mark_units_last = 0;
+    long long mark_unit_count() const override { return mark_units_last; }
     bool skip_now(int entries) const {
         const int on = skip < 0 ? skip_default(entries) : skip;
         const bool fits = (long long)geom.NF + geom.NJ + geom.NK < (1ll << 22) && nbf <= 32 * FSM_SLAB_WORDS;
@@ -1007,7 +1043,7 @@
         if (use_graph >= 2 || (use_graph == 1 && !persistent_now())) {
             hipGraph_t& graph = graphs[stage];
             hipGraphExec_t& graph_exec = graph_execs[stage];
-            const int key = mode * 2 + (skip_now(batch) ? 1 : 0);
+            const int key = mode * 4 + (skip_now(batch) ? 1 : 0) + (stage == 0 && marks_now(batch) ? 2 : 0);
             if (!graph_exec || graph_batches[stage] != batch || graph_modes[stage] != key) {
                 if (graph_exec) { (void)hipGraphExecDestroy(graph_exec); graph_exec = nullptr; }
                 if (graph) { (void)hipGraphDestroy(graph); graph = nullptr; }
@@ -1346,6 +1382,26 @@
         HIP_CHECK(hipMemcpyAsync(d_pts.p, pts.data(), pts.size() * sizeof(InitPoint<T>), hipMemcpyHostToDevice, stream));
         for (int b = 0; b < nb; ++b)
             HIP_CHECK(hipMemsetAsync(d_stamp.p + (size_t)(slot_ids[b] / NS) * n_bricks, 0xFF, n_bricks * sizeof(int), stream));
+        mark_units_last = 0;
+        std::vector<int> gs;
+        for (int b = 0; b < nb; ++b) gs.push_back(slot_ids[b] / NS);
+        std::sort(gs.begin(), gs.end());
+        gs.erase(std::unique(gs.begin(), gs.end()), gs.end());
+        stage = 0;
+        if (marks_now((int)gs.size())) {
+            const size_t per_group = (size_t)8 * n_patches * mark_row;
+            if (d_marks.n < per_group * n_groups()) {
+                HIP_CHECK(hipStreamSynchronize(stream));
+                d_marks.reserve(per_group * n_groups());
+                graph_batches[0] = graph_batches[1] = -1;
+            }
+            for (size_t q = 0; q < gs.size();) {
+                size_t r = q + 1;
+                while (r < gs.size() && gs[r] == gs[r - 1] + 1) ++r;
+                HIP_CHECK(hipMemsetAsync(d_marks.p + (size_t)gs[q] * per_group, 0, (r - q) * per_group * sizeof(int), stream));
+                q = r;
+            }
+        }
         std::vector<char> group_filled(n_groups(), 0);
         const bool all_slots = nb == n_slots && prefill_on();
         fill_arm = fill_in_flight = false;
@@ -1420,7 +1476,7 @@
         snap_always = false;
         if (persistent_now() || weno) HIP_CHECK(hipMemsetAsync(d_sync.p + 8, 0, (sync_words - 8) * sizeof(int), stream));
         if (persistent_now() || weno) HIP_CHECK(hipMemsetAsync(d_sync.p + 4, 0, sizeof(int), stream));
-        HIP_CHECK(hipMemsetAsync(d_evals.p, 0, sizeof(unsigned long long) * n_slots, stream));
+        HIP_CHECK(hipMemsetAsync(d_evals.p, 0, sizeof(unsigned long long) * (n_slots + 1), stream));
         HIP_CHECK(hipMemsetAsync(d_sw.p, 0, sizeof(unsigned long long) * (size_t)sw_sweeps * n_groups(), stream));
         HIP_CHECK(hipEventRecord(ev0, stream));
         int it_total = 0;
@@ -1565,12 +1621,15 @@
         timing.sweep_ms += ms;
         const long long evaluated_before = timing.evaluated_updates;
         if (was_persistent) {
-            HIP_CHECK(hipMemcpy(h_evals, d_evals.p, sizeof(unsigned long long) * n_slots, hipMemcpyDeviceToHost));
+            HIP_CHECK(hipMemcpy(h_evals, d_evals.p, sizeof(unsigned long long) * (n_slots + 1), hipMemcpyDeviceToHost));
+            mark_units_last = (long long)h_evals[n_slots];
             for (int s2 : slot_ids) timing.evaluated_updates += (long long)h_evals[s2];
         } else {
             timing.evaluated_updates += timing.node_updates - node_updates_before;
         }
         const bool skipped_now = skip_now(n_groups());
+        if (timing.node_updates > node_updates_before && skipped_now)
+            marks_auto = (double)(timing.evaluated_updates - evaluated_before) / (double)(timing.node_updates - node_updates_before) < 0.5;
         if (nb == n_slots && timing.node_updates > node_updates_before && skipped_now)
             last_eval_frac = (double)(timing.evaluated_updates - evaluated_before) / (double)(timing.node_updates - node_updates_before);
         if (skip < 0 && !weno && in_probe_window((nb + NS - 1) / NS) && timing.node_updates > node_updates_before) {
@@ -4294,6 +4353,9 @@
 int ttcr_fsm_stopping_stats(const ttcr_fsm_grid* g, long long* reference_sums, long long* reference_sums_missed, long long* rounds) {
     return guarded_on(g, [&] { g->impl->stopping_stats(reference_sums, reference_sums_missed, rounds); });
 }
+int ttcr_fsm_mark_units(const ttcr_fsm_grid* g, long long* units) {
+    return guarded_on(g, [&] { if (units) *units = g->impl->mark_unit_count(); });
+}
 int ttcr_fsm_prefill_swaps(const ttcr_fsm_grid* g, long long* swaps) {
     return guarded_on(g, [&] { if (swaps) *swaps = g->impl->prefill_swap_count(); });
 }
@@ -4346,6 +4408,57 @@
     });
 }
 
+int ttcr_fsm_chunk_marks(int NF, int NJ, int NK, int PJ, int PK, int C, int dir, int jc, int kc, int ia, int ib, int edges,
+                         int* out, size_t capacity, size_t* n) {
+    return guarded([&] {
+        if (NF < 1 || NJ < 1 || NK < 1 || PJ < 1 || PK < 1 || C < 1) throw ValueError("ttcr_fsm_chunk_marks: sizes must be positive");
+        if (dir < 0 || dir > 7) throw ValueError("ttcr_fsm_chunk_marks: dir must be 0 ... 7");
+        if (jc < 0 || jc >= NJ || kc < 0 || kc >= NK || ia < 0 || ib < ia || ib >= NF) throw ValueError("ttcr_fsm_chunk_marks: column or node range outside the grid");
+        if (!n) throw ValueError("ttcr_fsm_chunk_marks: null count");
+        size_t cnt = 0;
+        bool full = false;
+        auto emit = [&](int TJ, int TK, int c0, int c1) {
+            for (int c = c0; c <= c1; ++c) {
+                if (out) {
+                    if (cnt >= capacity) { full = true; return; }
+                    out[3 * cnt] = TJ; out[3 * cnt + 1] = TK; out[3 * cnt + 2] = c;
+                }
+                ++cnt;
+            }
+        };
+        if (edges) fsm_chunk_marks<true>(NF, NJ, NK, PJ, PK, C, dir, jc, kc, ia, ib, emit);
+        else fsm_chunk_marks<false>(NF, NJ, NK, PJ, PK, C, dir, jc, kc, ia, ib, emit);
+        if (full) throw ValueError("ttcr_fsm_chunk_marks: output buffer too small");
+        *n = cnt;
+    });
+}
+
+int ttcr_fsm_chunk_marks_row(int NF, int NJ, int NK, int PJ, int PK, int C, int dir, int jca, int jcb, int kc, int La, int Lb, int edges,
+                             int* out, size_t capacity, size_t* n) {
+    return guarded([&] {
+        if (NF < 1 || NJ < 1 || NK < 1 || PJ < 1 || PK < 1 || C < 1) throw ValueError("ttcr_fsm_chunk_marks_row: sizes must be positive");
+        if (dir < 0 || dir > 7) throw ValueError("ttcr_fsm_chunk_marks_row: dir must be 0 ... 7");
+        if (jca < 0 || jcb < jca || jcb >= NJ || kc < 0 || kc >= NK || Lb < La) throw ValueError("ttcr_fsm_chunk_marks_row: row or levels outside the grid");
+        if (Lb - jcb - kc < 0 || La - jca - kc > NF - 1) throw ValueError("ttcr_fsm_chunk_marks_row: an end column has no node on those levels");
+        if (!n) throw ValueError("ttcr_fsm_chunk_marks_row: null count");
+        size_t cnt = 0;
+        bool full = false;
+        auto emit = [&](int TJ, int TK, int c0, int c1) {
+            for (int c = c0; c <= c1; ++c) {
+                if (out) {
+                    if (cnt >= capacity) { full = true; return; }
+                    out[3 * cnt] = TJ; out[3 * cnt + 1] = TK; out[3 * cnt + 2] = c;
+                }
+                ++cnt;
+            }
+        };
+        if (edges) fsm_chunk_marks_row<true>(NF, NJ, NK, PJ, PK, C, dir, jca, jcb, kc, La, Lb, emit);
+        else fsm_chunk_marks_row<false>(NF, NJ, NK, PJ, PK, C, dir, jca, jcb, kc, La, Lb, emit);
+        if (full) throw ValueError("ttcr_fsm_chunk_marks_row: output buffer too small");
+        *n = cnt;
+    });
+}
+
 int ttcr_fsm_prefill_slice(int dtype, uint64_t n_el, uint32_t n_tickets, uint32_t ticket, uint64_t* slice_len, uint64_t* begin, uint64_t* end) {
     return guarded([&] {
         if (dtype != TTCR_F32 && dtype != TTCR_F64) throw ValueError("dtype must be TTCR_F32 or TTCR_F64");
diff --git a/ttcr_amd/csrc/fsm_chunk_marks.h b/ttcr_amd/csrc/fsm_chunk_marks.h
--- /dev/null
+++ b/ttcr_amd/csrc/fsm_chunk_marks.h
@@ -0,0 +1,87 @@
+#pragma once
+
+#if defined(__HIPCC__) || defined(__CUDACC__)
+#define FSM_MARKS_HD __host__ __device__ __forceinline__
+#else
+#define FSM_MARKS_HD inline
+#endif
+
+FSM_MARKS_HD int fsm_patch_lcf(int TJ, int TK, int PJ, int PK, int C) {
+    const int Ls = TJ * PJ + TK * PK;
+    return Ls - (Ls - TJ - TK) % C;
+}
+FSM_MARKS_HD int fsm_max_chunks(int NF, int PJ, int PK, int C) { return (PJ + PK + NF - 3 + C - 1) / C + 1; }
+
+template <bool EDGES = true, class Emit>
+FSM_MARKS_HD void fsm_chunk_marks(int NF, int NJ, int NK, int PJ, int PK, int C, int dir, int jc, int kc, int ia, int ib, Emit&& emit) {
+    const int nd = (dir + 1) & 7;
+    const bool ff = ((dir ^ nd) & 1) != 0, fj = ((dir ^ nd) & 2) != 0, fk = ((dir ^ nd) & 4) != 0;
+    const int j = fj ? NJ - 1 - jc : jc, k = fk ? NK - 1 - kc : kc;
+    const int a = ff ? NF - 1 - ib : ia, b = ff ? NF - 1 - ia : ib;
+    const int TJ = j / PJ, TK = k / PK;
+    const bool jf = j - TJ * PJ == 0, jl = j - TJ * PJ == PJ - 1 || j == NJ - 1;
+    const bool kf = k - TK * PK == 0, kl = k - TK * PK == PK - 1 || k == NK - 1;
+    const int la = a + j + k, lb = b + j + k;
+    for (int q = 0; q < (EDGES ? 5 : 1); ++q) {
+        const int dj = q == 1 ? -1 : q == 2 ? 1 : 0, dk = q == 3 ? -1 : q == 4 ? 1 : 0;
+        bool on = true;
+        int lo, hi;
+        if (q == 0) {
+            lo = (a > 0 || !jf || !kf) ? la - 1 : la;
+            hi = (b < NF - 1 || !jl || !kl) ? lb + 1 : lb;
+        } else {
+            on = q == 1 ? (jf && j > 0) : q == 2 ? (jl && j < NJ - 1) : q == 3 ? (kf && k > 0) : (kl && k < NK - 1);
+            lo = la + dj + dk;
+            hi = lb + dj + dk;
+        }
+        if (on) {
+            const int lcf = fsm_patch_lcf(TJ + dj, TK + dk, PJ, PK, C);
+            emit(TJ + dj, TK + dk, (lo - lcf) / C, (hi - lcf) / C);
+        }
+    }
+}
+
+template <bool EDGES = true, class Emit>
+FSM_MARKS_HD void fsm_chunk_marks_row(int NF, int NJ, int NK, int PJ, int PK, int C, int dir, int jca, int jcb, int kc, int La, int Lb,
+                                      Emit&& emit) {
+    const int nd = (dir + 1) & 7;
+    const bool ff = ((dir ^ nd) & 1) != 0, fj = ((dir ^ nd) & 2) != 0, fk = ((dir ^ nd) & 4) != 0;
+    const int k = fk ? NK - 1 - kc : kc;
+    const int ja = fj ? NJ - 1 - jcb : jca, jb = fj ? NJ - 1 - jca : jcb;
+    const int TK = k / PK;
+    const int k0 = TK * PK, km = (k0 + PK < NK ? k0 + PK : NK) - 1;
+    auto levels = [&](int j, int& la, int& lb) {
+        const int jc = fj ? NJ - 1 - j : j;
+        int ia = La - jc - kc, ib = Lb - jc - kc;
+        ia = ia < 0 ? 0 : ia;
+        ib = ib > NF - 1 ? NF - 1 : ib;
+        la = (ff ? NF - 1 - ib : ia) + j + k;
+        lb = (ff ? NF - 1 - ia : ib) + j + k;
+    };
+    auto put = [&](int TJ2, int TK2, int lo, int hi) {
+        const int j0 = TJ2 * PJ, kk0 = TK2 * PK;
+        const int ls = j0 + kk0, le = (j0 + PJ < NJ ? j0 + PJ : NJ) - 1 + (kk0 + PK < NK ? kk0 + PK : NK) - 1 + NF - 1;
+        lo = lo < ls ? ls : lo;
+        hi = hi > le ? le : hi;
+        if (lo > hi) return;
+        const int lcf = fsm_patch_lcf(TJ2, TK2, PJ, PK, C);
+        emit(TJ2, TK2, (lo - lcf) / C, (hi - lcf) / C);
+    };
+#if defined(__HIP_DEVICE_COMPILE__)
+#pragma unroll 1
+#endif
+    for (int TJ = ja / PJ; TJ <= jb / PJ; ++TJ) {
+        const int j0 = TJ * PJ, jm = (j0 + PJ < NJ ? j0 + PJ : NJ) - 1;
+        const int pa = ja > j0 ? ja : j0, pb = jb < jm ? jb : jm;
+        int la0, lb0, la1, lb1;
+        levels(pa, la0, lb0);
+        levels(pb, la1, lb1);
+        const int lo = la0 < la1 ? la0 : la1, hi = lb0 > lb1 ? lb0 : lb1;
+        put(TJ, TK, lo - 1, hi + 1);
+        if (!EDGES) continue;
+        if (pa == j0 && TJ > 0) put(TJ - 1, TK, la0 - 1, lb0 - 1);
+        if (pb == jm && jm < NJ - 1) put(TJ + 1, TK, la1 + 1, lb1 + 1);
+        if (k == k0 && TK > 0) put(TJ, TK - 1, lo - 1, hi - 1);
+        if (k == km && km < NK - 1) put(TJ, TK + 1, lo + 1, hi + 1);
+    }
+}
diff --git a/ttcr_amd/csrc/fsm_kernels.h b/ttcr_amd/csrc/fsm_kernels.h
--- a/ttcr_amd/csrc/fsm_kernels.h
+++ b/ttcr_amd/csrc/fsm_kernels.h
@@ -4,6 +4,7 @@
 #include <type_traits>
 
 #include "fsm_prefill_slices.h"
+#include "fsm_chunk_marks.h"
 
 namespace ttcr_amd {
 
@@ -448,6 +449,9 @@
     T* fill_dst;
     size_t fill_slice;
     size_t fill_n;
+    int* marks;
+    int mcw;
+    unsigned long long* mark_units;
 };
 
 
@@ -710,6 +714,9 @@
 #ifndef FSM_SLAB_WORDS
 #define FSM_SLAB_WORDS 32
 #endif
+#ifndef FSM_MARK_WORDS
+#define FSM_MARK_WORDS 4
+#endif
 #define FSM_FIN 0x3ffffff0
 #ifndef FSM_SKIP_ABL
 #define FSM_SKIP_ABL 0
@@ -775,8 +782,13 @@
 
 __host__ __device__ constexpr bool fsm_looped(bool is3d, int h) { return is3d && h == 1; }
 
+template <typename T>
+__host__ __device__ constexpr bool fsm_marks_kernel(bool is3d, bool skip, int h, int ns, bool xs, bool pre, int ar) {
+    return is3d && skip && h == 1 && xs && ar == 0 && !(sizeof(T) == 8 && ns == 2 && pre);
+}
+
 __device__ __forceinline__ int kmaxp_of(int k0, int NK, int PK) { return (k0 + PK < NK ? k0 + PK : NK) - 1; }
-template <typename T, int PJ, int PK, int C, bool IS3D, bool SKIP, int H, int NS, bool XS, bool PRE, int AR = 0>
+template <typename T, int PJ, int PK, int C, bool IS3D, bool SKIP, int H, int NS, bool XS, bool PRE, int AR = 0, bool MK = false>
 __device__ __forceinline__ bool fsm_sweep_unit(const PersistArgs<T>& pa) {
     static_assert(AR == 0 || std::is_same<T, float>::value, "tolerance-grade arithmetic: fp32 kernels");
     constexpr bool LOOPED = fsm_looped(IS3D, H);
@@ -825,6 +837,15 @@
     __shared__ unsigned s_mywv[2];
     enum { U_THR, U_RSJLO, U_RSKLO, U_RSNJ, U_RSNK, U_LCF, U_UPLCF0, U_UPLCF1, U_HIST, U_EVER, U_UCHG, U_PENDV, U_LCHG, U_N };
     __shared__ int s_u[U_N];
+    constexpr bool MARKS = MK;
+    static_assert(!MK || fsm_marks_kernel<T>(IS3D, SKIP, H, NS, XS, PRE, AR), "chunk marks: no such instantiation");
+    constexpr int MARKW = MARKS ? FSM_MARK_WORDS : 1;
+    __shared__ unsigned s_mark[MARKS ? 9 : 1][MARKW];
+    __shared__ unsigned s_cmask[MARKW];
+    constexpr int MARKNW = NT / 64;
+    __shared__ unsigned long long s_mlog[MARKS ? 32 * MARKW * MARKNW : 1];
+    enum { U_MKJ, U_MKK, U_MKR, U_MKN };
+    __shared__ int s_mk[MARKS ? U_MKN : 1];
 
     int tid = threadIdx.x;
     if constexpr (LOOPED) asm volatile("" : "+v"(tid));
@@ -1226,6 +1247,14 @@
         const int nsw = (pa.nbf + 31) >> 5;
         for (int w = tid; w < nsw; w += NT) s_slab[w] = 0u;
         for (int w = tid; w < 9 * SLABW; w += NT) s_stamped[w / SLABW][w % SLABW] = 0u;
+        if constexpr (MARKS) {
+            for (int w = tid; w < 9 * MARKW; w += NT) s_mark[w / MARKW][w % MARKW] = 0u;
+            if (tid < MARKW) s_cmask[tid] = 0u;
+            if (pa.marks) {
+                const int nlog = ((Le - Lc) / C + 1) * MARKNW;
+                for (int w = tid; w < nlog; w += NT) s_mlog[w] = 0ull;
+            }
+        }
         if (tid == 0) {
             s_cwi[0] = -1; s_cwi[1] = -1; s_mywi = -1;
             const int ja = j0 - H < 0 ? 0 : j0 - H, jb = jmaxp + H > NJ - 1 ? NJ - 1 : jmaxp + H;
@@ -1241,9 +1270,23 @@
             s_u[U_UPLCF0] = lsj - (((lsj - mu) % C + C) % C);
             s_u[U_UPLCF1] = lsk - (((lsk - mu) % C + C) % C);
             s_u[U_HIST] = 0; s_u[U_EVER] = 0; s_u[U_UCHG] = 0; s_u[U_PENDV] = 0; s_u[U_LCHG] = 0;
+            if constexpr (MARKS) {
+                const int nd = (dir + 1) & 7;
+                const int ja1 = j0 - 1 < 0 ? 0 : j0 - 1, jb1 = jmaxp + 1 > NJ - 1 ? NJ - 1 : jmaxp + 1;
+                const int ka1 = k0 - 1 < 0 ? 0 : k0 - 1, kb1 = kmaxp + 1 > NK - 1 ? NK - 1 : kmaxp + 1;
+                s_mk[U_MKJ] = (((dir ^ nd) & 2) ? NJ - 1 - jb1 : ja1) / PJ;
+                s_mk[U_MKK] = (((dir ^ nd) & 4) ? NK - 1 - kb1 : ka1) / PK;
+                s_mk[U_MKR] = (pa.marks && sg >= 2 && pa.skip != 2) ? 1 : 0;
+                if (s_mk[U_MKR] && pa.evals) atomicAdd(pa.mark_units, 1ull);
+            }
         }
         __syncthreads();
-        {
+        if (MARKS && s_mk[U_MKR]) {
+            const int* __restrict__ mrow = pa.marks + (((size_t)grp * 8 + dir) * pa.n_patches + (size_t)(TK * npj + TJ)) * pa.mcw;
+            const int nch = (Le - Lc) / C + 1, sg0 = pa.ndir * pa.iter_ptr[0] + dir;
+            for (int c = tid; c < nch; c += NT)
+                if (__hip_atomic_load(mrow + c, __ATOMIC_RELAXED, __HIP_MEMORY_SCOPE_AGENT) == sg0) atomicOr(&s_cmask[c >> 5], 1u << (c & 31));
+        } else {
             const int jlo = s_u[U_RSJLO], nj = s_u[U_RSNJ], klo = s_u[U_RSKLO], nk = s_u[U_RSNK], thr = s_u[U_THR];
             const int* __restrict__ stamp = pa.stamp + (size_t)grp * pa.nbf * pa.nbj * pa.nbk;
             const int total = pa.nbf * nj * nk;
@@ -1354,7 +1397,11 @@
                     if (!ok) { act = 0; break; }
                     if (L == lcf && vj >= FSM_FIN && !(vj & 1) && vk >= FSM_FIN && !(vk & 2)) {
                         bool any = false;
-                        for (int w = 0; w < ((pa.nbf + 31) >> 5); ++w) any |= s_slab[w] != 0u;
+                        if (MARKS && s_mk[U_MKR]) {
+                            for (int w = 0; w < MARKW; ++w) any |= s_cmask[w] != 0u;
+                        } else {
+                            for (int w = 0; w < ((pa.nbf + 31) >> 5); ++w) any |= s_slab[w] != 0u;
+                        }
                         if (!any) {
                             st_prog(my_prog, FSM_FIN);
                             L = Le + 1;
@@ -1362,9 +1409,15 @@
                             break;
                         }
                     }
-                    int flo, fhi;
-                    chunk_frange(L, H, flo, fhi);
-                    bool dirty = slab_any(flo, fhi);
+                    bool dirty;
+                    if (MARKS && s_mk[U_MKR]) {
+                        const int ci = (L - lcf) / C;
+                        dirty = (s_cmask[ci >> 5] >> (ci & 31)) & 1u;
+                    } else {
+                        int flo, fhi;
+                        chunk_frange(L, H, flo, fhi);
+                        dirty = slab_any(flo, fhi);
+                    }
                     if (!dirty && up_j) dirty = up_dirty(vj, need, 0);
                     if (!dirty && up_k) dirty = up_dirty(vk, need, 1);
                     if (dirty) break;
@@ -1572,6 +1625,11 @@
                 atomicOr(&s_stamped[jk][ba >> 5], 1u << (ba & 31));
                 if (bb2 != ba) atomicOr(&s_stamped[jk][bb2 >> 5], 1u << (bb2 & 31));
             }
+            if constexpr (MARKS) {
+                static_assert(!MARKS || (PJ == 16 && NT % 64 == 0), "chunk marks: a wavefront is four rows of a patch");
+                const unsigned long long cm = __builtin_amdgcn_ballot_w64(changed);
+                if (cm != 0ull && pa.marks && (tid & 63) == 0) s_mlog[((L0 - s_u[U_LCF]) / C) * MARKNW + (tid >> 6)] = cm;
+            }
         } else {
             if (wave_any(changed) && (tid & 63) == 0) s_anychg = 1;
         }
@@ -1594,9 +1652,11 @@
         if constexpr (SKIP) {
             if (!(FSM_SKIP_ABL & 4) && tid == 0) {
                 if (any_changed) {
-                    int flo, fhi;
-                    chunk_frange(L0, 0, flo, fhi);
-                    for (int b = flo / FSM_BRICK; b <= fhi / FSM_BRICK; ++b) s_slab[b >> 5] |= 1u << (b & 31);
+                    if (!(MARKS && s_mk[U_MKR])) {
+                        int flo, fhi;
+                        chunk_frange(L0, 0, flo, fhi);
+                        for (int b = flo / FSM_BRICK; b <= fhi / FSM_BRICK; ++b) s_slab[b >> 5] |= 1u << (b & 31);
+                    }
                     const int ci = (L0 - s_u[U_LCF]) / C, w = ci >> 5;
                     if ((chg_flags & 6) && w < pa.cw) {
                         if (s_mywi != w) { s_mywi = w; s_mywv[0] = 0u; s_mywv[1] = 0u; }
@@ -1638,6 +1698,41 @@
                 if (bf < pa.nbf && ((s_stamped[jk][bf >> 5] >> (bf & 31)) & 1u))
                     atomicMax(stamp + ((size_t)(rs_klo + jk / rs_nj) * pa.nbj + rs_jlo + jk % rs_nj) * pa.nbf + bf, sigma);
             }
+            if constexpr (MARKS) {
+                if (pa.marks) {
+                    {
+                        const int lcf = s_u[U_LCF], mkj = s_mk[U_MKJ], mkk = s_mk[U_MKK];
+                        const int nlog = ((Le - lcf) / C + 1) * MARKNW;
+                        for (int q = tid; q < nlog; q += NT) {
+                            const unsigned long long cm = s_mlog[q];
+                            if (cm == 0ull) continue;
+                            const int Lq = lcf + (q / MARKNW) * C, krow = k0 + 4 * (q % MARKNW);
+                            for (int r = 0; r < 4; ++r) {
+                                const unsigned m16 = (unsigned)(cm >> (16 * r)) & 0xffffu;
+                                if (!m16) continue;
+                                fsm_chunk_marks_row(NF, NJ, NK, PJ, PK, C, dir, j0 + __builtin_ctz(m16), j0 + 31 - __builtin_clz(m16), krow + r, Lq, Lq + C - 1,
+                                                    [&](int tj2, int tk2, int c0, int c1) {
+                                                        unsigned* mw = s_mark[(tk2 - mkk) * 3 + (tj2 - mkj)];
+                                                        for (int c = c0; c <= c1; ++c)
+                                                            if (c < 32 * MARKW) atomicOr(&mw[c >> 5], 1u << (c & 31));
+                                                    });
+                            }
+                        }
+                    }
+                    __syncthreads();
+                    int* __restrict__ mk = pa.marks + ((size_t)grp * 8 + ((dir + 1) & 7)) * pa.n_patches * pa.mcw;
+                    for (int w = tid; w < 9 * MARKW; w += NT) {
+                        const int sl = w / MARKW;
+                        unsigned bits = s_mark[sl][w % MARKW];
+                        int* row = mk + (size_t)((s_mk[U_MKK] + sl / 3) * npj + s_mk[U_MKJ] + sl % 3) * pa.mcw + (w % MARKW) * 32;
+                        while (bits) {
+                            const int b = __builtin_ctz(bits);
+                            bits &= bits - 1u;
+                            __hip_atomic_store(row + b, sigma, __ATOMIC_RELAXED, __HIP_MEMORY_SCOPE_AGENT);
+                        }
+                    }
+                }
+            }
             pending = 1;
         }
     }
@@ -1685,7 +1780,7 @@
     return true;
 }
 
-template <typename T, int PJ, int PK, int C, bool IS3D, bool SKIP, int H, int NS, bool XS, bool PRE = false, int AR = 0>
+template <typename T, int PJ, int PK, int C, bool IS3D, bool SKIP, int H, int NS, bool XS, bool PRE = false, int AR = 0, bool MK = false>
 #ifndef FSM_WENO_MINW
 #define FSM_WENO_MINW FSM_MINW
 #endif
@@ -1696,10 +1791,10 @@
         for (;;) {
             auto kp = __builtin_amdgcn_kernarg_segment_ptr();
             asm volatile("" : "+s"(kp));
-            if (!fsm_sweep_unit<T, PJ, PK, C, IS3D, SKIP, H, NS, XS, PRE, AR>(*(const PersistArgs<T>*)kp)) break;
+            if (!fsm_sweep_unit<T, PJ, PK, C, IS3D, SKIP, H, NS, XS, PRE, AR, MK>(*(const PersistArgs<T>*)kp)) break;
         }
     } else {
-        fsm_sweep_unit<T, PJ, PK, C, IS3D, SKIP, H, NS, XS, PRE, AR>(pa);
+        fsm_sweep_unit<T, PJ, PK, C, IS3D, SKIP, H, NS, XS, PRE, AR, MK>(pa);
     }
 }
 
diff --git a/ttcr_amd/rgrid.py b/ttcr_amd/rgrid.py
--- a/ttcr_amd/rgrid.py
+++ b/ttcr_amd/rgrid.py
@@ -121,6 +121,11 @@
         a, b, c = C.c_longlong(0), C.c_longlong(0), C.c_longlong(0)
         _lib.check(self._lib.ttcr_fsm_stopping_stats(self._h, C.byref(a), C.byref(b), C.byref(c)))
         return {"reference_sums": a.value, "reference_sums_missed": b.value, "rounds": c.value}
+
+    def mark_units(self):
+        a = C.c_longlong(0)
+        _lib.check(self._lib.ttcr_fsm_mark_units(self._h, C.byref(a)))
+        return a.value
 
     def prefill_swaps(self):
         a = C.c_longlong(0)
```

New measurement: 100,400 (median of 6 runs). 1.04x the previous value.
